# Negai-98/LDT

Hardware: AMD Instinct MI355X
Metric: shapes/sec (2048-pt, 1000-step SDE sample) (higher is better)
Workload: dtype bf16; 1 GPU; BASELINE configs[1]: ShapeNet-airplane sampling, batch 64/GPU, 256 latent tokens x 120, 1000 ancestral SDE steps (24-block d=1024 Score) + decode to 2048 points; global_batch=64, batch_per_gpu=64, sde_steps=1000, points=2048, parallelism=dp1 batch slices, one all-gather, collective=none (single process), rccl_ranks_seen=0

## Files before the change

include/ldt_hip.h:

```cpp
#ifndef LDT_HIP_H
#define LDT_HIP_H
#include <stdint.h>
#ifdef __cplusplus
extern "C" {
#endif

#define LDT_ABI_VERSION 25
#define LDT_OK 0
#define LDT_EARG (-1)
#define LDT_ESHAPE (-2)
#define LDT_EALIGN (-3)
#define LDT_MAX_BLOCKS 64

int ldt_abi_version(void);
const char* ldt_last_error(void);

int ldt_cast_pad_bf16(const float* src, int64_t ld_src, uint16_t* dst, int64_t ld_dst,
                      int64_t rows, int32_t cols, int32_t cols_pad, void* stream);

enum ldt_epilogue {
    LDT_EPI_F32 = 0,
    LDT_EPI_BF16 = 1,
    LDT_EPI_GELU_BF16 = 2,
    LDT_EPI_RELU_BF16 = 3,
// ... 91 lines not shown
                   int64_t mod_sample_stride, int32_t rows_per_sample, void* stream);

int ldt_fold_mean_ratio(const float* stats, int32_t parts, int64_t M, int32_t K, float* out, void* stream);

int ldt_fps(const float* xyz, int32_t B, int32_t n, int32_t m, int32_t skip_near_origin, int32_t* idx_out, void* stream);
int ldt_norm_points(const float* xyz, int32_t B, int32_t n, float* out, void* stream);
int ldt_mixture_seed(const float* eps, const float* sig, const float* mu, const float* logits, int32_t n_mix, int32_t D, int64_t rows,
                     float* out, void* stream);
int ldt_knn(const float* xyz, const float* centers, int32_t B, int32_t n, int32_t S, int32_t k,
            int32_t* idx_out, float* dist_out, void* stream);
int ldt_group_normalize(const float* feat, const float* xyz, const int32_t* fps_idx, const int32_t* knn_idx,
                        const float* alpha, const float* beta, double* stats, int32_t B, int32_t n, int32_t S,
                        int32_t k, int32_t D, uint16_t* U, int32_t ldu, int32_t center_mode, float* group_mean,
                        void* stream);
int ldt_gather_rows(const float* src, const int32_t* idx, int32_t B, int32_t n, int32_t S, int32_t C, float* out, void* stream);
int ldt_grouper_mlp(const float* feat, const float* xyz, const int32_t* fps_idx, const int32_t* knn_idx, const float* alpha,
                    const float* beta, double* stats, int32_t B, int32_t n, int32_t S, int32_t k, int32_t D,
                    const uint16_t* wimg, const float* b1, const float* b2, const float* b3, float* out, void* stream);
int ldt_maxpool(const void* in, int32_t in_bf16, int64_t ld, int64_t G, int32_t n, int32_t C, float* out, void* stream);
int ldt_actnorm(float* x, const float* shift, const float* log_scale, int64_t B, int64_t per_sample, void* stream);
int ldt_reparam(const float* post, const float* noise, float* out, int64_t ldo, float* mu_out, float* logvar_out,
                int64_t rows, int32_t z, float lo, float hi, void* stream);
int ldt_chamfer(const float* a, const float* b, int32_t B, int32_t na, int32_t nb, float* dl, float* dr, void* stream);

int ldt_reparam_kl(const float* post, const float* noise, float* out, int64_t ldo, float* mu_out, float* logvar_out,
                   float* kl_out, float* logqz_out, float* kl_sample_sum, int64_t rows, int64_t rows_per_sample, int32_t z,
                   float lo, float hi, void* stream);
int ldt_diffuse_q(const float* x0, const float* eta_in, const float* m, const float* var, float* xt, float* eta_out,
                  int64_t B, int64_t per_sample, uint64_t seed, int32_t step, void* stream);
int ldt_dsm_loss(const float* eta, const float* params, const float* weight, int64_t B, int64_t per_sample, int32_t l1,
                 float* sample_loss, float* mean_loss, void* stream);

int ldt_nelbo_terms(const float* eta, const float* params, const float* logqz, const float* weight, int64_t B, int64_t per_sample,
                    float* sample_sums, float* batch_sums, void* stream);
int ldt_occupancy_grid(const float* pts, int32_t S, int32_t n, const float* cells, int32_t G, uint32_t* counters, uint32_t* bernoulli,
                       void* stream);

int ldt_transpose_cast_bf16(const void* src, int32_t src_bf16, int64_t ld_src, uint16_t* dst, int64_t ld_dst, int64_t R, int32_t C,
                            int64_t R_pad, void* stream);
int ldt_colsum(const void* dy, int32_t dy_bf16, int64_t ld, int64_t M, int32_t C, float* out, void* stream);
int ldt_layernorm_modulate_bwd(const float* x, int64_t ldx, const float* dy, int64_t lddy, const float* scale, int64_t mod_sample_stride,
                               int32_t rows_per_sample, float* dx, int64_t lddx, float* dshift, float* dscale,
                               int64_t dmod_sample_stride, float* stats, int64_t M, int32_t C, void* stream);
int ldt_gelu_bwd(const uint16_t* u, int64_t ldu, const void* dh, int32_t dh_bf16, int64_t lddh, uint16_t* du, int64_t lddu, int64_t M,
                 int32_t C, void* stream);
int ldt_gate_residual_bwd(const float* dy, int64_t lddy, const void* a, int32_t a_bf16, int64_t lda, const float* gate,
                          int64_t gate_sample_stride, int32_t rows_per_sample, uint16_t* da, int64_t ldda, float* dgate,
                          int64_t dgate_sample_stride, int64_t M, int32_t C, void* stream);
int ldt_silu_bwd(const float* c, const float* dy, float* dc, float* act, int64_t n, void* stream);
int ldt_dsm_loss_bwd(const float* eta, const float* params, const float* weight, int64_t B, int64_t per_sample, int32_t l1, float* dparams,
                     void* stream);
int ldt_embedding_grad(const float* dc, int64_t ld, const int32_t* label, int32_t B, int32_t D, int32_t n_classes, float* dE, void* stream);
int ldt_attention_bwd(const uint16_t* Q, int64_t ldq, int64_t q_batch_stride, const uint16_t* K, int64_t ldk, const uint16_t* V,
                      int64_t ldv, int64_t kv_batch_stride, const uint16_t* O, const uint16_t* dO, float* stats, uint16_t* dQ,
                      int64_t lddq, int64_t dq_batch_stride, uint16_t* dK, int64_t lddk, uint16_t* dV, int64_t lddv,
                      int64_t dkv_batch_stride, int32_t B, int32_t H, int32_t N, int32_t head_dim, void* stream);
int ldt_attention_bwd_narrow(const uint16_t* Q, int64_t ldq, int64_t q_batch_stride, const uint16_t* K, int64_t ldk, const uint16_t* V,
                             int64_t ldv, int64_t kv_batch_stride, const uint16_t* O, const uint16_t* dO, float* stats, uint16_t* dQ,
                             int64_t lddq, int64_t dq_batch_stride, uint16_t* dK, int64_t lddk, uint16_t* dV, int64_t lddv,
                             int64_t dkv_batch_stride, int32_t B, int32_t H, int32_t N, int32_t head_dim, void* stream);
int ldt_attention_bwd_cross(const uint16_t* Q, int64_t ldq, int64_t q_batch_stride, const uint16_t* K, int64_t ldk, const uint16_t* V,
                            int64_t ldv, int64_t kv_batch_stride, const uint16_t* O, const uint16_t* dO, float* stats, uint16_t* dQ,
                            int64_t lddq, int64_t dq_batch_stride, uint16_t* dK, int64_t lddk, uint16_t* dV, int64_t lddv,
                            int64_t dkv_batch_stride, int32_t B, int32_t H, int32_t Nq, int32_t Nk, int32_t head_dim, void* stream);
int ldt_sumsq(const float* x, int64_t n, double* scratch, int32_t scratch_len, float max_norm, float* out, void* stream);
int ldt_adam_ema_step(float* param, float* grad, float* exp_avg, float* exp_avg_sq, float* ema, int64_t n, double lr, double beta1,
                      double beta2, double eps, double weight_decay, int32_t step, double ema_decay, int32_t ema_init,
                      const float* clip_factor, void* stream);

int ldt_ln_mlp_resid(float* x, int64_t ldx, int64_t M, int32_t C, const float* ln_w, const float* ln_b,
                     const float* shift, const float* scale, const float* gate, int64_t mod_sample_stride,
                     int32_t rows_per_sample, const uint16_t* w_up, const float* b_up, const uint16_t* w_dn,
                     const float* b_dn, uint16_t* x_bf16, int64_t ldxb, void* stream);

int ldt_ln_mlp_resid_next(float* x, int64_t ldx, int64_t M, int32_t C, const float* ln_w, const float* ln_b,
                          const float* shift, const float* scale, const float* gate, int64_t mod_sample_stride,
                          int32_t rows_per_sample, const uint16_t* w_up, const float* b_up, const uint16_t* w_dn,
                          const float* b_dn, uint16_t* x_bf16, int64_t ldxb,
                          const float* nx_ln_w, const float* nx_ln_b, const float* nx_shift, const float* nx_scale,
                          int64_t nx_mod_sample_stride, int32_t nx_rows_per_sample, const uint16_t* nx_w, const float* nx_bias,
                          int32_t nx_N, uint16_t* nx_out, int64_t nx_ldo, void* stream);

int ldt_ln_linear(const float* x, int64_t ldx, int64_t M, int32_t C, const float* ln_w, const float* ln_b,
                  const float* shift, const float* scale, int64_t mod_sample_stride, int32_t rows_per_sample,
                  const uint16_t* w, const float* bias, int32_t N, uint16_t* out, int64_t ldo, void* stream);

int ldt_chamfer_pairwise(const float* x, const float* y, int32_t S, int32_t R, int32_t n, int32_t m, float* cd, void* stream);
int ldt_emd_approx(const float* x, const float* y, int32_t S, int32_t R, int32_t n, int32_t m, int32_t pairwise,
                   float* out, void* stream);

typedef struct ldt_score_plan {
    int32_t hidden, heads, blocks, z_dim, z_pad, mlp_hidden, tokens, batch;
    const uint16_t* w_in;  const float* b_in;
    const uint16_t* w_qkv[LDT_MAX_BLOCKS]; const float* b_qkv[LDT_MAX_BLOCKS];
    const uint16_t* w_o[LDT_MAX_BLOCKS];   const float* b_o[LDT_MAX_BLOCKS];
    const uint16_t* w_up[LDT_MAX_BLOCKS];  const float* b_up[LDT_MAX_BLOCKS];
    const uint16_t* w_dn[LDT_MAX_BLOCKS];  const float* b_dn[LDT_MAX_BLOCKS];
    const uint16_t* w_out; const float* b_out;
    const uint16_t* w_q[LDT_MAX_BLOCKS];   const float* b_q[LDT_MAX_BLOCKS];
    const uint16_t* kv_cond[LDT_MAX_BLOCKS];
    int32_t cond_tokens; int32_t _pad0;
    const float* mod; int64_t mod_step_stride; int64_t mod_sample_stride;
    uint16_t* xin;
    float*    X;
    uint16_t* Hb;
    uint16_t* QKV;
    uint16_t* Ob;
    uint16_t* U;
    const float* fold; int64_t fold_step_stride; float* stats;
    int32_t gemm_wgs;
    int32_t fold_monitor_every;
    float* fold_monitor;
} ldt_score_plan;

int ldt_score_lnfold_route(int32_t M, int32_t D, int32_t F, int32_t gemm_wgs);

int ldt_score_forward(const ldt_score_plan* plan, const float* x, float* eps_out,
                      const int32_t* step_ptr, void* stream);

enum ldt_prof_class {
    LDT_PROF_OTHER = 0,
    LDT_PROF_GEMM_IO = 1,
    LDT_PROF_LN = 2,
    LDT_PROF_GEMM_QKV = 3,
    LDT_PROF_ATTN = 4,
    LDT_PROF_GEMM_O = 5,
    LDT_PROF_GEMM_GELU = 6,
    LDT_PROF_GEMM_DN = 7,
    LDT_PROF_NCLASS = 8
};
int ldt_score_forward_profile(const ldt_score_plan* plan, const float* x, float* eps_out, const int32_t* step_ptr,
                              float* ms_by_class, int32_t* launches_by_class, void* stream);

typedef struct ldt_cond_args {
    const float* temb;
    const float* extra;
    const float* w_ada;
    const float* b_ada;
    float* c_buf;
    float* mod_buf;
    int32_t t_dim, n_mod;
    const void* w_ada_bf16;
    void* c_buf_bf16;
} ldt_cond_args;

int ldt_sample_loop(const ldt_score_plan* plan, float* x, float* x_mean, float* eps_tmp,
                    const float* coef, int32_t mode, const float* noise, int64_t noise_step_stride,
                    int64_t elem_offset, uint64_t seed, int32_t* step_counter, int32_t n_steps,
                    const ldt_cond_args* cond, float* x_traj, int32_t use_graph, void* stream);

int ldt_dbg_gemm_group_m(int32_t rows_per_group);
int ldt_dbg_gemm_epi(int32_t bits);
int ldt_dbg_gemm_wreg(int32_t on);

#ifdef __cplusplus
}
#endif
#endif
```

ldt_amd/_lib.py:

```python
import ctypes as C
import os

_HERE = os.path.dirname(os.path.abspath(__file__))
LIB_PATH = os.environ.get("LDT_HIP_LIB", os.path.join(_HERE, "libldt_hip.so"))
ABI_VERSION = 25
MAX_BLOCKS = 64
ODE_SUMSQ_SCRATCH = 1024

EPI_F32, EPI_BF16, EPI_GELU_BF16, EPI_RELU_BF16, EPI_RESID_F32 = range(5)
ACT_NONE, ACT_SILU, ACT_RELU, ACT_GELU = range(4)
BLOCK_ACTS = {"gelu": 1, "silu": 2, "swish": 2, "relu": 3, "leakyrelu": 4, "leakyrelu0.2": 5, "rrelu": 6, "hardswish": 7, "selu": 8}


def block_act_id(name):
    return 0 if name is None else BLOCK_ACTS.get(str(name).lower(), 3)
PROF_CLASSES = ("other", "gemm_io", "ln_modulate", "gemm_qkv", "attention", "gemm_o", "gemm_gelu", "gemm_dn")

_vp, _i32, _i64, _u64 = C.c_void_p, C.c_int32, C.c_int64, C.c_uint64


class ScorePlan(C.Structure):
    _fields_ = (
        [(n, _i32) for n in ("hidden", "heads", "blocks", "z_dim", "z_pad", "mlp_hidden", "tokens", "batch")]
        + [("w_in", _vp), ("b_in", _vp)]
        + [("w_qkv", _vp * MAX_BLOCKS), ("b_qkv", _vp * MAX_BLOCKS),
           ("w_o", _vp * MAX_BLOCKS), ("b_o", _vp * MAX_BLOCKS),
           ("w_up", _vp * MAX_BLOCKS), ("b_up", _vp * MAX_BLOCKS),
           ("w_dn", _vp * MAX_BLOCKS), ("b_dn", _vp * MAX_BLOCKS)]
        + [("w_out", _vp), ("b_out", _vp)]
        + [("w_q", _vp * MAX_BLOCKS), ("b_q", _vp * MAX_BLOCKS), ("kv_cond", _vp * MAX_BLOCKS), ("cond_tokens", _i32), ("_pad0", _i32)]
        + [("mod", _vp), ("mod_step_stride", _i64), ("mod_sample_stride", _i64)]
        + [(n, _vp) for n in ("xin", "X", "Hb", "QKV", "Ob", "U")]
        + [("fold", _vp), ("fold_step_stride", _i64), ("stats", _vp), ("gemm_wgs", _i32), ("fold_monitor_every", _i32), ("fold_monitor", _vp)]
    )


class CondArgs(C.Structure):
    _fields_ = ([(n, _vp) for n in ("temb", "extra", "w_ada", "b_ada", "c_buf", "mod_buf")] + [("t_dim", _i32), ("n_mod", _i32)] +
                [("w_ada_bf16", _vp), ("c_buf_bf16", _vp)])


SIGNATURES = {
    "ldt_abi_version": [],
    "ldt_last_error": [],
    "ldt_cast_pad_bf16": [_vp, _i64, _vp, _i64, _i64, _i32, _i32, _vp],
    "ldt_gemm_bf16": [_i32, _vp, _i64, _vp, _i64, _vp, _vp, _i64, _vp, _i64, _vp, _i64, _vp, _i64, _i32, _vp, _i64,
                      _i32, _i32, _i32, _vp],
    "ldt_gemm_resid_lnstats": [_vp, _i64, _vp, _i64, _vp, _vp, _i64, _vp, _i64, _i32, _vp, _vp, _i64, _vp, _vp, _i64, _i64,
                               _i32, _i32, _i32, _i32, _vp],
    "ldt_gemm_lnfold": [_i32, _vp, _i64, _vp, _i64, _vp, _vp, _vp, _vp, _i64, _vp, _i64, _i32, _i32, _i32, _i32, _vp],
    "ldt_score_lnfold_route": [_i32, _i32, _i32, _i32],
    "ldt_layernorm_modulate": [_vp, _i64, _vp, _i64, _vp, _vp, _vp, _vp, _i64, _i32, _vp, _i64, _i64, _i32, _vp],
    "ldt_attention_fwd": [_vp, _i64, _i64, _vp, _i64, _vp, _i64, _i64, _vp, _i32, _i32, _i32, _i32, _i32, _vp],
    "ldt_attention_route": [_i32, _i32, _i32, _i32, _i32],
    "ldt_gemm_route": [_i32, _i32, _i32, _i32, _i64, _i32, _i32],
    "ldt_qkv_attention": [_vp, _i64, _vp, _i64, _vp, _vp, _i32, _vp, _vp, _i64, _vp, _i64, _i64, _vp, _vp,
                          _i32, _i32, _i32, _i32, _i32, _i32, _i32, _vp, _vp],
    "ldt_qkv_attention_route": [_i32, _i32, _i32, _i32, _i32, _i32, _i32, _i32],
    "ldt_attention_oproj_resid": [_vp, _i64, _i64, _vp, _i64, _vp, _i64, _i64, _i32, _i32, _i32, _i32, _i32, _vp, _vp, _vp, _i64, _vp, _i64, _vp],
    "ldt_sgemm": [_vp, _i64, _vp, _i64, _vp, _vp, _i64, _i32, _i32, _i32, _i32, _i32, _i32, _vp],
    "ldt_sinusoid": [_vp, _vp, _vp, _i32, _i32, _vp],
    "ldt_sampler_step": [_vp, _vp, _vp, _i64, _vp, _vp, _vp, _vp, _i32, _i32, _i64, _i64, _u64, _i32, _i32, _vp],
    "ldt_sampler_step_traj": [_vp, _vp, _vp, _i64, _vp, _vp, _vp, _vp, _vp, _i32, _i32, _i64, _i64, _u64, _i32, _i32, _vp],
    "ldt_philox_normal": [_vp, _i64, _i64, _i32, _u64, _vp],
    "ldt_batch_norm_sum": [_vp, _i32, _i64, _vp, _vp, _vp],
    "ldt_langevin_coef": [_vp, _i32, C.c_float, C.c_float, _vp, _vp],
    "ldt_pndm_transfer": [_vp, _vp, C.c_float, C.c_float, C.c_float, _vp, _i64, _vp],
    "ldt_lincomb4": [_vp, _vp, _vp, _vp, C.c_float, C.c_float, C.c_float, C.c_float, C.c_float, _vp, _i64, _vp],
    "ldt_vpsde_score": [_vp, _vp, C.c_float, C.c_float, C.c_float, _vp, _i32, _i64, _vp],
    "ldt_sde_score": [_vp, _vp, _i32, C.c_float, C.c_float, C.c_float, _vp, _i32, _i64, _vp],
    "ldt_add_f32": [_vp, _vp, _vp, _i64, _vp],
    "ldt_ode_stage": [_vp] * 7 + [C.c_double] * 6 + [_i32, C.c_double, _vp, _vp, _i64, _vp],
    "ldt_ode_rhs": [_vp, _vp, _i32, C.c_float, C.c_float, C.c_float, _vp, _i64, _vp],
    "ldt_ode_scaled_sumsq": [_vp] * 7 + [C.c_double] * 7 + [_i32, _vp, _vp, C.c_double, C.c_double, _vp, _i32, _vp, _i64, _vp],
    "ldt_block_activation": [_vp, _i64, _i64, _i32, _i32, _vp],
    "ldt_group_stats": [_vp, _i64, _i32, _i32, _i32, _i32, C.c_float, _vp, _vp],
    "ldt_norm_apply": [_vp, _i64, _vp, _i64, _i64, _i32, _vp, _i32, _i32, _vp, _vp, _vp, _vp, _i64, _i32, _vp],
    "ldt_widen_bf16": [_vp, _vp, _i64, _vp],
    "ldt_fold_mean_ratio": [_vp, _i32, _i64, _i32, _vp, _vp],
    "ldt_fps": [_vp, _i32, _i32, _i32, _i32, _vp, _vp],
    "ldt_norm_points": [_vp, _i32, _i32, _vp, _vp],
    "ldt_mixture_seed": [_vp, _vp, _vp, _vp, _i32, _i32, _i64, _vp, _vp],
    "ldt_knn": [_vp, _vp, _i32, _i32, _i32, _i32, _vp, _vp, _vp],
    "ldt_group_normalize": [_vp, _vp, _vp, _vp, _vp, _vp, _vp, _i32, _i32, _i32, _i32, _i32, _vp, _i32, _i32, _vp, _vp],
    "ldt_gather_rows": [_vp, _vp, _i32, _i32, _i32, _i32, _vp, _vp],
    "ldt_maxpool": [_vp, _i32, _i64, _i64, _i32, _i32, _vp, _vp],
    "ldt_actnorm": [_vp, _vp, _vp, _i64, _i64, _vp],
    "ldt_reparam": [_vp, _vp, _vp, _i64, _vp, _vp, _i64, _i32, C.c_float, C.c_float, _vp],
    "ldt_chamfer": [_vp, _vp, _i32, _i32, _i32, _vp, _vp, _vp],
    "ldt_reparam_kl": [_vp, _vp, _vp, _i64, _vp, _vp, _vp, _vp, _vp, _i64, _i64, _i32, C.c_float, C.c_float, _vp],
    "ldt_diffuse_q": [_vp, _vp, _vp, _vp, _vp, _vp, _i64, _i64, _u64, _i32, _vp],
    "ldt_dsm_loss": [_vp, _vp, _vp, _i64, _i64, _i32, _vp, _vp, _vp],
    "ldt_nelbo_terms": [_vp, _vp, _vp, _vp, _i64, _i64, _vp, _vp, _vp],
    "ldt_occupancy_grid": [_vp, _i32, _i32, _vp, _i32, _vp, _vp, _vp],
    "ldt_transpose_cast_bf16": [_vp, _i32, _i64, _vp, _i64, _i64, _i32, _i64, _vp],
    "ldt_colsum": [_vp, _i32, _i64, _i64, _i32, _vp, _vp],
    "ldt_layernorm_modulate_bwd": [_vp, _i64, _vp, _i64, _vp, _i64, _i32, _vp, _i64, _vp, _vp, _i64, _vp, _i64, _i32, _vp],
    "ldt_gelu_bwd": [_vp, _i64, _vp, _i32, _i64, _vp, _i64, _i64, _i32, _vp],
    "ldt_gate_residual_bwd": [_vp, _i64, _vp, _i32, _i64, _vp, _i64, _i32, _vp, _i64, _vp, _i64, _i64, _i32, _vp],
    "ldt_silu_bwd": [_vp, _vp, _vp, _vp, _i64, _vp],
    "ldt_dsm_loss_bwd": [_vp, _vp, _vp, _i64, _i64, _i32, _vp, _vp],
    "ldt_embedding_grad": [_vp, _i64, _vp, _i32, _i32, _i32, _vp, _vp],
    "ldt_attention_bwd": [_vp, _i64, _i64, _vp, _i64, _vp, _i64, _i64, _vp, _vp, _vp, _vp, _i64, _i64, _vp, _i64, _vp, _i64, _i64,
                          _i32, _i32, _i32, _i32, _vp],
    "ldt_attention_bwd_narrow": [_vp, _i64, _i64, _vp, _i64, _vp, _i64, _i64, _vp, _vp, _vp, _vp, _i64, _i64, _vp, _i64, _vp, _i64, _i64,
                                 _i32, _i32, _i32, _i32, _vp],
    "ldt_attention_bwd_cross": [_vp, _i64, _i64, _vp, _i64, _vp, _i64, _i64, _vp, _vp, _vp, _vp, _i64, _i64, _vp, _i64, _vp, _i64, _i64,
                                _i32, _i32, _i32, _i32, _i32, _vp],
    "ldt_sumsq": [_vp, _i64, _vp, _i32, C.c_float, _vp, _vp],
    "ldt_adam_ema_step": [_vp, _vp, _vp, _vp, _vp, _i64, C.c_double, C.c_double, C.c_double, C.c_double, C.c_double, _i32, C.c_double, _i32,
                          _vp, _vp],
    "ldt_grouper_mlp": [_vp, _vp, _vp, _vp, _vp, _vp, _vp, _i32, _i32, _i32, _i32, _i32, _vp, _vp, _vp, _vp, _vp, _vp],
    "ldt_ln_mlp_resid": [_vp, _i64, _i64, _i32, _vp, _vp, _vp, _vp, _vp, _i64, _i32, _vp, _vp, _vp, _vp, _vp, _i64, _vp],
    "ldt_ln_mlp_resid_next": [_vp, _i64, _i64, _i32, _vp, _vp, _vp, _vp, _vp, _i64, _i32, _vp, _vp, _vp, _vp, _vp, _i64,
                              _vp, _vp, _vp, _vp, _i64, _i32, _vp, _vp, _i32, _vp, _i64, _vp],
    "ldt_ln_linear": [_vp, _i64, _i64, _i32, _vp, _vp, _vp, _vp, _i64, _i32, _vp, _vp, _i32, _vp, _i64, _vp],
    "ldt_chamfer_pairwise": [_vp, _vp, _i32, _i32, _i32, _i32, _vp, _vp],
    "ldt_emd_approx": [_vp, _vp, _i32, _i32, _i32, _i32, _i32, _vp, _vp],
    "ldt_score_forward": [C.POINTER(ScorePlan), _vp, _vp, _vp, _vp],
    "ldt_score_forward_profile": [C.POINTER(ScorePlan), _vp, _vp, _vp, C.POINTER(C.c_float), C.POINTER(C.c_int32), _vp],
    "ldt_dbg_gemm_group_m": [_i32],
    "ldt_dbg_gemm_epi": [_i32],
    "ldt_dbg_gemm_wreg": [_i32],
    "ldt_sample_loop": [C.POINTER(ScorePlan), _vp, _vp, _vp, _vp, _i32, _vp, _i64, _i64, _u64, _vp, _i32, C.POINTER(CondArgs), _vp, _i32, _vp],
}

_lib = None


class LdtHipError(RuntimeError):
    pass


def lib():
    global _lib
    if _lib is not None:
        return _lib
    if not os.path.exists(LIB_PATH):
        raise LdtHipError(
            "HIP extension %s not found: run `python -c 'import __graft_entry__ as g; g.build()'` "
            "(or ldt_amd/csrc/build.sh).  There is no CPU fallback." % LIB_PATH)
    h = C.CDLL(LIB_PATH)
    for name, argtypes in SIGNATURES.items():
        fn = getattr(h, name)
        fn.argtypes = argtypes
        fn.restype = C.c_char_p if name == "ldt_last_error" else C.c_int
    if h.ldt_abi_version() != ABI_VERSION:
        raise LdtHipError("libldt_hip.so ABI %d != binding ABI %d: rebuild" % (h.ldt_abi_version(), ABI_VERSION))
    _lib = h
    return h


def check(rc, what=""):
    if rc != 0:
        msg = lib().ldt_last_error()
        raise LdtHipError("%s failed (status %d): %s" % (what or "libldt_hip", rc, (msg or b"").decode()))
```

ldt_amd/csrc/api.hip:

```cpp
#include <stdarg.h>
#include <stdio.h>
#include <stdlib.h>
#include <string.h>

#include <vector>

#include "../../include/ldt_hip.h"
#include "kernels.h"

static thread_local char g_err[512] = "";

void ldt_set_error(const char* fmt, ...) {
    va_list ap;
    va_start(ap, fmt);
    vsnprintf(g_err, sizeof(g_err), fmt, ap);
    va_end(ap);
}
int ldt_check_launch(const char* what) {
    const hipError_t e = hipGetLastError();
    if (e != hipSuccess) {
        ldt_set_error("%s: %s", what, hipGetErrorString(e));
        return (int)e;
    }
    return LDT_OK;
}
extern "C" const char* ldt_last_error(void) { return g_err; }
extern "C" int ldt_abi_version(void) { return LDT_ABI_VERSION; }

#define BF(p) reinterpret_cast<const bf16_t*>(p)
#define BFM(p) reinterpret_cast<bf16_t*>(p)
#define ST(s) reinterpret_cast<hipStream_t>(s)
#define TRY(expr)                   \
    do {                            \
        const int _rc = (expr);     \
        if (_rc != LDT_OK) return _rc; \
    } while (0)

extern "C" int ldt_cast_pad_bf16(const float* src, int64_t ld_src, uint16_t* dst, int64_t ld_dst, int64_t rows,
                                 int32_t cols, int32_t cols_pad, void* stream) {
    LDT_REQUIRE(src && dst, LDT_EARG, "cast_pad: null pointer");
    return ldt_cast_pad_launch(src, ld_src, BFM(dst), ld_dst, rows, cols, cols_pad, ST(stream));
}

extern "C" int ldt_gemm_bf16(int32_t epilogue, const uint16_t* X, int64_t ldx, const uint16_t* W, int64_t ldw,
                             const float* bias, void* out, int64_t ldo, const float* resid, int64_t ldr,
                             const uint16_t* skip, int64_t ldskip, const float* gate, int64_t gate_sample_stride,
                             int32_t rows_per_sample, const int32_t* step_ptr, int64_t gate_step_stride,
                             int32_t M, int32_t N, int32_t K, void* stream) {
    LDT_REQUIRE(X && W && out, LDT_EARG, "gemm: null pointer");
    GemmArgs a{BF(X), ldx, BF(W), ldw, bias, out, ldo, resid, ldr, BF(skip), ldskip, gate, gate_sample_stride,
               rows_per_sample, step_ptr, gate_step_stride, M, N, K};
    return ldt_gemm_launch(epilogue, &a, ST(stream));
}

extern "C" int ldt_gemm_resid_lnstats(const uint16_t* X, int64_t ldx, const uint16_t* W, int64_t ldw, const float* bias,
                                      float* out, int64_t ldo, const float* gate, int64_t gate_sample_stride,
                                      int32_t rows_per_sample, const float* ln_scale, uint16_t* xs, int64_t ldxs,
                                      float* stats_out, const int32_t* step_ptr, int64_t gate_step_stride,
                                      int64_t ln_step_stride, int32_t M, int32_t N, int32_t K, int32_t stats_parts, void* stream) {
    LDT_REQUIRE(X && W && out && xs && ln_scale && stats_out, LDT_EARG, "gemm_resid_lnstats: null pointer");
    LDT_REQUIRE(stats_parts == N / 256 || stats_parts == N / 32, LDT_EARG, "gemm_resid_lnstats: stats_parts=%d is neither N/256 nor N/32 (N=%d)", stats_parts, N);
    GemmArgs a{BF(X), ldx, BF(W), ldw, bias, out, ldo, out, ldo, nullptr, 0, gate, gate_sample_stride, rows_per_sample, step_ptr,
               gate_step_stride, M, N, K, BFM(xs), ldxs, ln_scale, ln_step_stride, stats_out};
    a.stats_parts = stats_parts;
    return ldt_gemm_lnfold_launch(EPI_RESID_F32, &a, ST(stream));
}

extern "C" int ldt_gemm_lnfold(int32_t epilogue, const uint16_t* Xs, int64_t ldx, const uint16_t* W, int64_t ldw,
                               const float* stats_in, const float* fold_S, const float* fold_C, uint16_t* out, int64_t ldo,
                               const int32_t* step_ptr, int64_t fold_step_stride, int32_t M, int32_t N, int32_t K, int32_t stats_parts,
                               void* stream) {
    LDT_REQUIRE(Xs && W && out && stats_in && fold_S && fold_C, LDT_EARG, "gemm_lnfold: null pointer");
    LDT_REQUIRE(stats_parts == K / 256 || stats_parts == K / 32, LDT_EARG, "gemm_lnfold: stats_parts=%d is neither K/256 nor K/32 (K=%d)", stats_parts, K);
    GemmArgs a{BF(Xs), ldx, BF(W), ldw, nullptr, out, ldo, nullptr, 0, nullptr, 0, nullptr, 0, 0, step_ptr, 0, M, N, K,
               nullptr, 0, nullptr, 0, nullptr, stats_in, stats_parts, fold_S, fold_C, fold_step_stride};
    return ldt_gemm_lnfold_launch(epilogue, &a, ST(stream));
}

extern "C" int ldt_layernorm_modulate(const float* x, int64_t ldx, uint16_t* y, int64_t ldy, const float* w,
                                      const float* b, const float* shift, const float* scale,
                                      int64_t mod_sample_stride, int32_t rows_per_sample, const int32_t* step_ptr,
                                      int64_t mod_step_stride, int64_t M, int32_t C, void* stream) {
    LDT_REQUIRE(x && y, LDT_EARG, "ln: null pointer");
    LnArgs a{x, ldx, BFM(y), ldy, w, b, shift, scale, mod_sample_stride, rows_per_sample, step_ptr, mod_step_stride, M, C};
    return ldt_ln_launch(&a, ST(stream));
}

extern "C" int ldt_attention_fwd(const uint16_t* Q, int64_t ldq, int64_t q_batch_stride, const uint16_t* K,
                                 int64_t ldk, const uint16_t* V, int64_t ldv, int64_t kv_batch_stride, uint16_t* O,
                                 int32_t B, int32_t H, int32_t Nq, int32_t Nk, int32_t head_dim, void* stream) {
    LDT_REQUIRE(Q && K && V && O, LDT_EARG, "attention: null pointer");
    AttnArgs a{BF(Q), ldq, q_batch_stride, BF(K), ldk, kv_batch_stride, BF(V), ldv, BFM(O), B, H, Nq, Nk,
               1.4426950408889634f / sqrtf((float)head_dim), nullptr, nullptr, nullptr, 0, nullptr, 0};
    return ldt_attn_launch(&a, head_dim, ST(stream));
}
extern "C" int ldt_attention_route(int32_t B, int32_t H, int32_t Nq, int32_t Nk, int32_t head_dim) { return ldt_attn_route(B, H, Nq, Nk, head_dim); }
extern "C" int ldt_gemm_route(int32_t epilogue, int32_t M, int32_t N, int32_t K, int64_t ldo, int32_t fold, int32_t max_wgs) {
    GemmArgs a{};
    a.M = M; a.N = N; a.K = K; a.ldo = ldo; a.ldr = ldo; a.max_wgs = max_wgs;
    if (fold != 0 && fold != 32 && fold != 256) return 0;
    const GemmRoute r = ldt_gemm_decide(epilogue, &a, fold);
    return (r.family << 28) | ((r.tiles_per_wg < 255 ? r.tiles_per_wg : 255) << 20) | (r.bm << 10) | r.bn;
}
extern "C" int ldt_attention_oproj_resid(const uint16_t* Q, int64_t ldq, int64_t q_batch_stride, const uint16_t* K,
                                         int64_t ldk, const uint16_t* V, int64_t ldv, int64_t kv_batch_stride,
                                         int32_t B, int32_t H, int32_t Nq, int32_t Nk, int32_t head_dim,
                                         const uint16_t* Wo, const float* bo, float* X, int64_t ldx, const float* gate,
                                         int64_t gate_sample_stride, void* stream) {
    LDT_REQUIRE(Q && K && V && Wo && bo && X, LDT_EARG, "attention_oproj: null pointer");
    AttnArgs a{BF(Q), ldq, q_batch_stride, BF(K), ldk, kv_batch_stride, BF(V), ldv, nullptr, B, H, Nq, Nk,
               1.4426950408889634f / sqrtf((float)head_dim), BF(Wo), bo, X, ldx, gate, gate_sample_stride};
    return ldt_attn_oproj_launch(&a, head_dim, ST(stream));
}

extern "C" int ldt_sgemm(const float* A, int64_t lda, const float* Bw, int64_t ldb, const float* bias, void* C,
                         int64_t ldc, int32_t out_bf16, int32_t act_in, int32_t act_out, int32_t M, int32_t N,
                         int32_t K, void* stream) {
    SgemmArgs a{A, lda, Bw, ldb, bias, C, ldc, out_bf16, act_in, act_out, M, N, K};
    return ldt_sgemm_launch(&a, ST(stream));
}

extern "C" int ldt_sinusoid(const float* t, const float* freq, float* e, int32_t n, int32_t half, void* stream) {
    LDT_REQUIRE(t && freq && e, LDT_EARG, "sinusoid: null pointer");
    return ldt_sinusoid_launch(t, freq, e, n, half, ST(stream));
}

extern "C" int ldt_sampler_step(const float* x, const float* params, const float* noise, int64_t noise_step_stride,
                                float* x_out, float* x_mean_out, const float* coef, const int32_t* step_ptr,
                                int32_t step_host, int32_t mode, int64_t n, int64_t elem_offset, uint64_t seed,
                                int32_t philox_mul, int32_t philox_add, void* stream) {
    StepArgs a{x, params, noise, x_out, x_mean_out, coef, step_ptr, step_host, mode, n, elem_offset, noise_step_stride,
               (uint32_t)seed, (uint32_t)(seed >> 32), philox_mul, philox_add};
    return ldt_sampler_step_launch(&a, ST(stream));
}
extern "C" int ldt_sampler_step_traj(const float* x, const float* params, const float* noise, int64_t noise_step_stride,
                                     float* x_out, float* x_mean_out, float* traj, const float* coef, const int32_t* step_ptr,
                                     int32_t step_host, int32_t mode, int64_t n, int64_t elem_offset, uint64_t seed,
                                     int32_t philox_mul, int32_t philox_add, void* stream) {
    LDT_REQUIRE(!traj || ldt_aligned16(traj), LDT_EALIGN, "sampler_step_traj: traj must be 16-byte aligned");
    StepArgs a{x, params, noise, x_out, x_mean_out, coef, step_ptr, step_host, mode, n, elem_offset, noise_step_stride,
               (uint32_t)seed, (uint32_t)(seed >> 32), philox_mul, philox_add, traj};
    return ldt_sampler_step_launch(&a, ST(stream));
}

extern "C" int ldt_philox_normal(float* out, int64_t n, int64_t elem_offset, int32_t step, uint64_t seed, void* stream) {
    LDT_REQUIRE(out, LDT_EARG, "philox_normal: null pointer");
    return ldt_philox_normal_launch(out, n, elem_offset, step, (uint32_t)seed, (uint32_t)(seed >> 32), ST(stream));
}

extern "C" int ldt_fps(const float* xyz, int32_t B, int32_t n, int32_t m, int32_t skip_near_origin, int32_t* idx_out, void* stream) {
    LDT_REQUIRE(xyz && idx_out, LDT_EARG, "fps: null pointer");
    return ldt_fps_launch(xyz, B, n, m, skip_near_origin, idx_out, ST(stream));
}
extern "C" int ldt_knn(const float* xyz, const float* centers, int32_t B, int32_t n, int32_t S, int32_t k,
                       int32_t* idx_out, float* dist_out, void* stream) {
    LDT_REQUIRE(xyz && centers && idx_out, LDT_EARG, "knn: null pointer");
    return ldt_knn_launch(xyz, centers, B, n, S, k, idx_out, dist_out, ST(stream));
// ... 50 lines not shown
extern "C" int ldt_ln_mlp_resid(float* x, int64_t ldx, int64_t M, int32_t C, const float* ln_w, const float* ln_b,
                                const float* shift, const float* scale, const float* gate, int64_t mod_sample_stride,
                                int32_t rows_per_sample, const uint16_t* w_up, const float* b_up, const uint16_t* w_dn,
                                const float* b_dn, uint16_t* x_bf16, int64_t ldxb, void* stream) {
    LDT_REQUIRE(x && w_up && b_up && w_dn && b_dn, LDT_EARG, "ln_mlp: null pointer");
    MlpArgs a{x, ldx, M, ln_w, ln_b, shift, scale, gate, mod_sample_stride, rows_per_sample, BF(w_up), b_up, BF(w_dn), b_dn,
              BFM(x_bf16), ldxb};
    return ldt_ln_mlp_launch(&a, C, ST(stream));
}
extern "C" int ldt_ln_mlp_resid_next(float* x, int64_t ldx, int64_t M, int32_t C, const float* ln_w, const float* ln_b,
                                     const float* shift, const float* scale, const float* gate, int64_t mod_sample_stride,
                                     int32_t rows_per_sample, const uint16_t* w_up, const float* b_up, const uint16_t* w_dn,
                                     const float* b_dn, uint16_t* x_bf16, int64_t ldxb,
                                     const float* nx_ln_w, const float* nx_ln_b, const float* nx_shift, const float* nx_scale,
                                     int64_t nx_mod_sample_stride, int32_t nx_rows_per_sample, const uint16_t* nx_w, const float* nx_bias,
                                     int32_t nx_N, uint16_t* nx_out, int64_t nx_ldo, void* stream) {
    LDT_REQUIRE(x && w_up && b_up && w_dn && b_dn && nx_w && nx_out, LDT_EARG, "ln_mlp_next: null pointer");
    MlpArgs a{x, ldx, M, ln_w, ln_b, shift, scale, gate, mod_sample_stride, rows_per_sample, BF(w_up), b_up, BF(w_dn), b_dn,
              BFM(x_bf16), ldxb,
              LnLinArgs{nullptr, 0, M, nx_ln_w, nx_ln_b, nx_shift, nx_scale, nx_mod_sample_stride, nx_rows_per_sample, BF(nx_w), nx_bias,
                        nx_N, BFM(nx_out), nx_ldo}};
    return ldt_ln_mlp_launch(&a, C, ST(stream));
}
extern "C" int ldt_ln_linear(const float* x, int64_t ldx, int64_t M, int32_t C, const float* ln_w, const float* ln_b,
                             const float* shift, const float* scale, int64_t mod_sample_stride, int32_t rows_per_sample,
                             const uint16_t* w, const float* bias, int32_t N, uint16_t* out, int64_t ldo, void* stream) {
    LDT_REQUIRE(x && w && out, LDT_EARG, "ln_linear: null pointer");
    LnLinArgs a{x, ldx, M, ln_w, ln_b, shift, scale, mod_sample_stride, rows_per_sample, BF(w), bias, N, BFM(out), ldo};
    return ldt_ln_linear_launch(&a, C, ST(stream));
}
extern "C" int ldt_chamfer_pairwise(const float* x, const float* y, int32_t S, int32_t R, int32_t n, int32_t m, float* cd, void* stream) {
    LDT_REQUIRE(x && y && cd, LDT_EARG, "chamfer_pairwise: null pointer");
    return ldt_chamfer_pairwise_launch(x, y, S, R, n, m, cd, ST(stream));
}
extern "C" int ldt_emd_approx(const float* x, const float* y, int32_t S, int32_t R, int32_t n, int32_t m, int32_t pairwise,
                              float* out, void* stream) {
    LDT_REQUIRE(x && y && out, LDT_EARG, "emd_approx: null pointer");
    return ldt_emd_approx_launch(x, y, S, R, n, m, pairwise, out, ST(stream));
}

extern "C" int ldt_score_lnfold_route(int32_t M, int32_t D, int32_t F, int32_t gemm_wgs) {
    if (M <= 0 || D <= 0 || F <= 0 || D % 256 != 0 || D > 1024 || F % 256 != 0) return 0;
    if (ldt_gemm_lnfold_v1_route(M, D, F, gemm_wgs)) return 2;
    const int lim = ldt_wg_limit(gemm_wgs);
    return (M % 256 == 0 && (long)(M / 256) * (D / 256) * 8 >= (long)lim * 5) ? 1 : 0;
}

static int check_plan(const ldt_score_plan* p) {
    LDT_REQUIRE(p, LDT_EARG, "score: null plan");
    LDT_REQUIRE(p->blocks > 0 && p->blocks <= LDT_MAX_BLOCKS, LDT_ESHAPE, "score: blocks=%d out of range", p->blocks);
    LDT_REQUIRE(p->hidden > 0 && p->heads > 0 && p->hidden % p->heads == 0, LDT_ESHAPE, "score: hidden %% heads");
    const int dh = p->hidden / p->heads;
    LDT_REQUIRE(dh == 8 || dh == 16 || dh == 32 || dh == 64, LDT_ESHAPE, "score: head dim %d not built (8, 16, 32, 64)", dh);
    LDT_REQUIRE(p->hidden % 64 == 0 && p->mlp_hidden % 64 == 0 && p->z_pad % 64 == 0 && p->z_pad >= p->z_dim, LDT_ESHAPE,
                "score: hidden/mlp_hidden/z_pad must be multiples of 64");
    LDT_REQUIRE(p->z_dim % 4 == 0, LDT_ESHAPE, "score: z_dim %% 4");
    LDT_REQUIRE(p->tokens > 0 && p->batch > 0, LDT_ESHAPE, "score: empty batch");
    LDT_REQUIRE(p->w_in && p->w_out && p->mod && p->xin && p->X && p->Hb && p->QKV && p->Ob && p->U, LDT_EARG, "score: null buffer in plan");
    for (int l = 0; l < p->blocks; ++l) {
        LDT_REQUIRE(p->w_qkv[l] && p->w_o[l] && p->w_up[l] && p->w_dn[l], LDT_EARG, "score: block %d weights missing", l);
        LDT_REQUIRE(!p->kv_cond[l] || (p->w_q[l] && p->cond_tokens > 0), LDT_EARG, "score: block %d cross-attention needs w_q and cond_tokens", l);
    }
    return LDT_OK;
}

struct Prof {
    hipStream_t s;
    std::vector<hipEvent_t> ev;
    std::vector<int> cls;
    void begin(int c) { hipEvent_t a, b; (void)hipEventCreate(&a); (void)hipEventCreate(&b); ev.push_back(a); ev.push_back(b); cls.push_back(c); (void)hipEventRecord(a, s); }
    void end() { (void)hipEventRecord(ev.back(), s); }
    void cancel() { (void)hipEventDestroy(ev.back()); ev.pop_back(); (void)hipEventDestroy(ev.back()); ev.pop_back(); cls.pop_back(); }
};
#define LAUNCH_TRY(cls_, took_, try_expr, st_)      \
    do {                                            \
        if (prof) prof->begin(cls_);                \
        took_ = (try_expr);                         \
        if (prof) { if (took_) prof->end(); else prof->cancel(); } \
        if (took_ && (st_) != LDT_OK) return (st_); \
    } while (0)
#define LAUNCH(cls_, expr)                \
    do {                                  \
        if (prof) prof->begin(cls_);      \
        const int _rc = (expr);           \
        if (prof) prof->end();            \
        if (_rc != LDT_OK) return _rc;    \
    } while (0)

struct QkvAttnStep {
    const bf16_t* X; long ldx; const bf16_t* W; long ldw; const float* bias;
    const float* stats; int stats_parts; const float* fold_S; const float* fold_C; long fold_step_stride;
    const bf16_t* kv; long ldkv; long kv_batch_stride;
    bf16_t* attn_o; bf16_t* QKV;
    int B, tokens, cond_tokens, hidden, heads, K, max_wgs;
    const int* step_ptr;
};
static int qkv_attention_route(const GemmArgs* g, int tokens, int cond_tokens, int head_dim, bool cross, bool folded) {
    if (cross) return ldt_gemm_mid_q_xattn_takes(g, tokens, cond_tokens, head_dim) ? 3 : 0;
    if (ldt_gemm_mid_qkv_attn_takes(g, tokens, head_dim, folded)) return 1;
    return ldt_gemm_qkv_attn256_takes(g, tokens, head_dim, folded) ? 2 : 0;
}
static int qkv_attention_step(const QkvAttnStep& q, hipStream_t s, Prof* prof) {
    const int D = q.hidden, T = q.tokens, dh = D / q.heads;
    const bool cross = q.kv != nullptr, folded = q.stats != nullptr;
    const float scale_log2e = 1.4426950408889634f / sqrtf((float)dh);
    GemmArgs gq{q.X, q.ldx, q.W, q.ldw, q.bias, q.QKV, 3L * D, nullptr, 0, nullptr, 0, nullptr, 0, 0, folded ? q.step_ptr : nullptr, 0,
                q.B * T, cross ? D : 3 * D, q.K};
    if (folded) { gq.stats_in = q.stats; gq.stats_parts = q.stats_parts; gq.fold_S = q.fold_S; gq.fold_C = q.fold_C; gq.fold_step_stride = q.fold_step_stride; }
    gq.max_wgs = q.max_wgs;
    gq.attn_o = q.attn_o; gq.attn_scale_log2e = scale_log2e;
    if (cross) { gq.attn_k = q.kv; gq.attn_v = q.kv + D; gq.attn_ldkv = q.ldkv; gq.attn_kv_batch_stride = q.kv_batch_stride; }
    int fst = LDT_OK;
    bool took = false;
    if (cross) LAUNCH_TRY(LDT_PROF_GEMM_QKV, took, ldt_gemm_mid_q_xattn_try(&gq, T, q.cond_tokens, dh, s, &fst), fst);
    else {
        LAUNCH_TRY(LDT_PROF_GEMM_QKV, took, ldt_gemm_mid_qkv_attn_try(&gq, T, dh, folded, s, &fst), fst);
        if (!took) LAUNCH_TRY(LDT_PROF_GEMM_QKV, took, ldt_gemm_qkv_attn256_try(&gq, T, dh, folded, s, &fst), fst);
    }
    if (took) return LDT_OK;
    if (folded) LAUNCH(LDT_PROF_GEMM_QKV, ldt_gemm_lnfold_launch(LDT_EPI_BF16, &gq, s));
    else LAUNCH(LDT_PROF_GEMM_QKV, ldt_gemm_launch(LDT_EPI_BF16, &gq, s));
    const int S = cross ? q.cond_tokens : T;
    AttnArgs at{q.QKV, 3L * D, (long)T * 3 * D, cross ? q.kv : q.QKV + D, cross ? q.ldkv : 3L * D, cross ? q.kv_batch_stride : (long)T * 3 * D,
                cross ? q.kv + D : q.QKV + 2 * D, cross ? q.ldkv : 3L * D, q.attn_o, q.B, q.heads, T, S, scale_log2e};
    LAUNCH(LDT_PROF_ATTN, ldt_attn_launch(&at, dh, s));
    return LDT_OK;
}

extern "C" int ldt_qkv_attention_route(int32_t B, int32_t tokens, int32_t cond_tokens, int32_t hidden, int32_t heads, int32_t K, int32_t fold,
                                       int32_t max_wgs) {
    if (B <= 0 || tokens <= 0 || hidden <= 0 || heads <= 0 || hidden % heads != 0 || (fold != 0 && fold != 32 && fold != 256) || (fold && cond_tokens > 0)) return 0;
    GemmArgs g{};
    g.M = B * tokens; g.N = cond_tokens > 0 ? hidden : 3 * hidden; g.K = K; g.max_wgs = max_wgs;
    g.stats_parts = fold ? K / fold : 0;
    return qkv_attention_route(&g, tokens, cond_tokens, hidden / heads, cond_tokens > 0, fold != 0);
}
extern "C" int ldt_qkv_attention(const uint16_t* X, int64_t ldx, const uint16_t* W, int64_t ldw, const float* bias,
                                 const float* stats, int32_t stats_parts, const float* fold_S, const float* fold_C, int64_t fold_step_stride,
                                 const uint16_t* kv_cond, int64_t ldkv, int64_t kv_batch_stride, uint16_t* O, uint16_t* QKV,
                                 int32_t B, int32_t tokens, int32_t cond_tokens, int32_t hidden, int32_t heads, int32_t K, int32_t max_wgs,
                                 const int32_t* step_ptr, void* stream) {
    LDT_REQUIRE(X && W && O && QKV, LDT_EARG, "qkv_attention: null pointer");
    LDT_REQUIRE(B > 0 && tokens > 0 && hidden > 0 && heads > 0 && hidden % heads == 0 && hidden % 64 == 0 && K > 0, LDT_ESHAPE,
                "qkv_attention: B=%d tokens=%d hidden=%d heads=%d K=%d", B, tokens, hidden, heads, K);
    const int dh = hidden / heads;
    LDT_REQUIRE(dh == 8 || dh == 16 || dh == 32 || dh == 64, LDT_ESHAPE, "qkv_attention: head dim %d not built (8, 16, 32, 64)", dh);
    LDT_REQUIRE(!kv_cond || (cond_tokens > 0 && !stats), LDT_EARG, "qkv_attention: cross-attention needs cond_tokens and has no folded form");
    LDT_REQUIRE(!stats || (fold_S && fold_C && stats_parts > 0 && !bias), LDT_EARG, "qkv_attention: the folded form needs fold_S, fold_C, stats_parts and takes no bias (it is part of fold_C)");
    QkvAttnStep q{BF(X), ldx, BF(W), ldw, bias, stats, stats_parts, fold_S, fold_C, fold_step_stride, BF(kv_cond), ldkv, kv_batch_stride,
                  BFM(O), BFM(QKV), B, tokens, cond_tokens, hidden, heads, K, max_wgs, step_ptr};
    return qkv_attention_step(q, ST(stream), nullptr);
}

static int score_forward_impl(const ldt_score_plan* p, const float* x, float* eps_out, const int32_t* step_ptr,
                              hipStream_t s, Prof* prof) {
    TRY(check_plan(p));
    LDT_REQUIRE(x && eps_out, LDT_EARG, "score: null x/out");
    const int D = p->hidden, T = p->tokens, M = p->batch * p->tokens, F = p->mlp_hidden;
    const long sstr = p->mod_sample_stride, tstr = p->mod_step_stride;
    const bool fold_v1 = ldt_gemm_lnfold_v1_route(M, D, F, p->gemm_wgs);
    bool fold = p->fold && p->stats && sstr == 0 && (M % 256 == 0 || fold_v1) && D % 256 == 0 && D <= 1024 && F % 256 == 0;
    for (int l = 0; l < p->blocks && fold; ++l) fold = !p->kv_cond[l];
    const int sparts = fold_v1 ? D / 32 : D / 256;
    const long fstep = p->fold_step_stride, fblk = 6L * D + 2L * F;
    LAUNCH(LDT_PROF_OTHER, ldt_cast_pad_launch(x, p->z_dim, BFM(p->xin), p->z_pad, M, p->z_dim, p->z_pad, s));
    {
        GemmArgs g{BF(p->xin), p->z_pad, BF(p->w_in), p->z_pad, p->b_in, p->X, D, nullptr, 0, nullptr, 0, nullptr, 0, 0, nullptr, 0, M, D, p->z_pad};
        g.max_wgs = p->gemm_wgs; LAUNCH(LDT_PROF_GEMM_IO, ldt_gemm_launch(LDT_EPI_F32, &g, s));
    }
    for (int l = 0; l < p->blocks; ++l) {
        const float* m = p->mod + (long)l * 6 * D;
        const float* fl = fold ? p->fold + (long)l * fblk : nullptr;
        QkvAttnStep qa{BF(p->Hb), D, nullptr, D, nullptr, nullptr, 0, nullptr, nullptr, 0, nullptr, 0, 0, BFM(p->Ob), BFM(p->QKV),
                       p->batch, T, p->cond_tokens, D, p->heads, D, p->gemm_wgs, step_ptr};
        if (fold && l > 0) {
            qa.W = BF(p->w_qkv[l]);
            qa.stats = p->stats; qa.stats_parts = sparts; qa.fold_S = fl; qa.fold_C = fl + 3L * D; qa.fold_step_stride = fstep;
        } else {
            LnArgs n1{p->X, D, BFM(p->Hb), D, nullptr, nullptr, m, m + D, sstr, T, step_ptr, tstr, M, D};
            LAUNCH(LDT_PROF_LN, ldt_ln_launch(&n1, s));
            if (p->kv_cond[l]) {
                qa.W = BF(p->w_q[l]); qa.bias = p->b_q[l];
                qa.kv = BF(p->kv_cond[l]); qa.ldkv = 2L * D; qa.kv_batch_stride = (long)p->cond_tokens * 2 * D;
            } else {
                qa.W = BF(p->w_qkv[l]); qa.bias = p->b_qkv[l];
            }
        }
        TRY(qkv_attention_step(qa, s, prof));
        if (fold) {
            GemmArgs go{BF(p->Ob), D, BF(p->w_o[l]), D, p->b_o[l], p->X, D, p->X, D, nullptr, 0, m + 2 * D, sstr, T, step_ptr, tstr, M, D, D,
                        BFM(p->Hb), D, m + 4 * D, tstr, p->stats};
            go.max_wgs = p->gemm_wgs; go.stats_parts = sparts; LAUNCH(LDT_PROF_GEMM_O, ldt_gemm_lnfold_launch(LDT_EPI_RESID_F32, &go, s));
            if (p->fold_monitor) TRY(ldt_fold_monitor_launch(p->stats, sparts, M, D, p->fold_monitor, s));
            GemmArgs gu{BF(p->Hb), D, BF(p->w_up[l]), D, nullptr, p->U, F, nullptr, 0, nullptr, 0, nullptr, 0, 0, step_ptr, 0, M, F, D,
                        nullptr, 0, nullptr, 0, nullptr, p->stats, sparts, fl + 6L * D, fl + 6L * D + F, fstep};
            gu.max_wgs = p->gemm_wgs; LAUNCH(LDT_PROF_GEMM_GELU, ldt_gemm_lnfold_launch(LDT_EPI_GELU_BF16, &gu, s));
            GemmArgs gd{BF(p->U), F, BF(p->w_dn[l]), F, p->b_dn[l], p->X, D, p->X, D, nullptr, 0, m + 5 * D, sstr, T, step_ptr, tstr, M, D, F,
                        BFM(p->Hb), D, m + 6 * D + D, tstr, p->stats};
            gd.max_wgs = p->gemm_wgs; gd.stats_parts = sparts;
            if (l + 1 < p->blocks) {
                LAUNCH(LDT_PROF_GEMM_DN, ldt_gemm_lnfold_launch(LDT_EPI_RESID_F32, &gd, s));
                if (p->fold_monitor) TRY(ldt_fold_monitor_launch(p->stats, sparts, M, D, p->fold_monitor, s));
            }
            else LAUNCH(LDT_PROF_GEMM_DN, ldt_gemm_launch(LDT_EPI_RESID_F32, &gd, s));
            continue;
        }
        LnArgs n2{p->X, D, BFM(p->Hb), D, nullptr, nullptr, m + 3 * D, m + 4 * D, sstr, T, step_ptr, tstr, M, D};
        {
            GemmArgs go{BF(p->Ob), D, BF(p->w_o[l]), D, p->b_o[l], p->X, D, p->X, D, nullptr, 0, m + 2 * D, sstr, T, step_ptr, tstr, M, D, D};
            go.max_wgs = p->gemm_wgs; LAUNCH(LDT_PROF_GEMM_O, ldt_gemm_launch(LDT_EPI_RESID_F32, &go, s));
        }
        LAUNCH(LDT_PROF_LN, ldt_ln_launch(&n2, s));
        GemmArgs gu{BF(p->Hb), D, BF(p->w_up[l]), D, p->b_up[l], p->U, F, nullptr, 0, nullptr, 0, nullptr, 0, 0, nullptr, 0, M, F, D};
        gu.max_wgs = p->gemm_wgs; LAUNCH(LDT_PROF_GEMM_GELU, ldt_gemm_launch(LDT_EPI_GELU_BF16, &gu, s));
        {
            GemmArgs gd{BF(p->U), F, BF(p->w_dn[l]), F, p->b_dn[l], p->X, D, p->X, D, nullptr, 0, m + 5 * D, sstr, T, step_ptr, tstr, M, D, F};
            gd.max_wgs = p->gemm_wgs; LAUNCH(LDT_PROF_GEMM_DN, ldt_gemm_launch(LDT_EPI_RESID_F32, &gd, s));
        }
    }
    {
        const float* m = p->mod + (long)p->blocks * 6 * D;
        LnArgs nf{p->X, D, BFM(p->Hb), D, nullptr, nullptr, m, m + D, sstr, T, step_ptr, tstr, M, D};
        LAUNCH(LDT_PROF_LN, ldt_ln_launch(&nf, s));
        GemmArgs gf{BF(p->Hb), D, BF(p->w_out), D, p->b_out, eps_out, p->z_dim, nullptr, 0, nullptr, 0, nullptr, 0, 0, nullptr, 0, M, p->z_dim, D};
        gf.max_wgs = p->gemm_wgs; LAUNCH(LDT_PROF_GEMM_IO, ldt_gemm_launch(LDT_EPI_F32, &gf, s));
    }
    return LDT_OK;
}

extern "C" int ldt_score_forward(const ldt_score_plan* p, const float* x, float* eps_out, const int32_t* step_ptr, void* stream) {
    return score_forward_impl(p, x, eps_out, step_ptr, ST(stream), nullptr);
}

extern "C" int ldt_score_forward_profile(const ldt_score_plan* p, const float* x, float* eps_out, const int32_t* step_ptr,
                                         float* ms_by_class, int32_t* launches_by_class, void* stream) {
    LDT_REQUIRE(ms_by_class && launches_by_class, LDT_EARG, "score_profile: null output");
    Prof prof{ST(stream), {}, {}};
    const int rc = score_forward_impl(p, x, eps_out, step_ptr, ST(stream), &prof);
    (void)hipStreamSynchronize(ST(stream));
    for (int c = 0; c < LDT_PROF_NCLASS; ++c) { ms_by_class[c] = 0.f; launches_by_class[c] = 0; }
    for (size_t i = 0; i < prof.cls.size(); ++i) {
        float ms = 0.f;
        if (rc == LDT_OK && hipEventElapsedTime(&ms, prof.ev[2 * i], prof.ev[2 * i + 1]) == hipSuccess) {
            ms_by_class[prof.cls[i]] += ms;
            launches_by_class[prof.cls[i]] += 1;
        }
        (void)hipEventDestroy(prof.ev[2 * i]);
        (void)hipEventDestroy(prof.ev[2 * i + 1]);
    }
    return rc;
}

static int enqueue_step(const ldt_score_plan* p, float* x, float* x_mean, float* eps_tmp, const float* coef, int mode,
                        const float* noise, long noise_step_stride, long elem_offset, uint64_t seed, int* step_counter,
                        const ldt_cond_args* cond, float* x_traj, hipStream_t s) {
    if (cond) {
        TRY(ldt_cond_rows_launch(cond->temb, cond->extra, cond->c_buf, cond->c_buf_bf16, step_counter, p->batch, cond->t_dim, 1, s));
        if (cond->w_ada_bf16 && (cond->t_dim % 64 == 0 || !cond->w_ada)) {
            GemmArgs g{};
            g.X = BF(cond->c_buf_bf16); g.ldx = cond->t_dim;
            g.W = BF(cond->w_ada_bf16); g.ldw = cond->t_dim;
            g.bias = cond->b_ada; g.out = cond->mod_buf; g.ldo = cond->n_mod;
            g.M = p->batch; g.N = cond->n_mod; g.K = cond->t_dim;
            g.max_wgs = p->gemm_wgs;
            TRY(ldt_gemm_launch(EPI_F32, &g, s));
        } else {
            SgemmArgs g{cond->c_buf, cond->t_dim, cond->w_ada, cond->t_dim, cond->b_ada, cond->mod_buf, cond->n_mod, 0, LDT_ACT_NONE,
                        LDT_ACT_NONE, p->batch, cond->n_mod, cond->t_dim};
            TRY(ldt_sgemm_launch(&g, s));
        }
    }
    TRY(score_forward_impl(p, x, eps_tmp, cond ? nullptr : step_counter, s, nullptr));
    const long n = (long)p->batch * p->tokens * p->z_dim;
    StepArgs st{x, eps_tmp, noise, x, x_mean, coef, step_counter, 0, mode, n, elem_offset, noise_step_stride,
                (uint32_t)seed, (uint32_t)(seed >> 32), 1, 0, x_traj};
    TRY(ldt_sampler_step_launch(&st, s));
    return ldt_advance_step_launch(step_counter, s);
}

extern "C" int ldt_sample_loop(const ldt_score_plan* p, float* x, float* x_mean, float* eps_tmp, const float* coef,
                               int32_t mode, const float* noise, int64_t noise_step_stride, int64_t elem_offset,
                               uint64_t seed, int32_t* step_counter, int32_t n_steps, const ldt_cond_args* cond,
                               float* x_traj, int32_t use_graph, void* stream) {
    TRY(check_plan(p));
    LDT_REQUIRE(x && x_mean && eps_tmp && coef && step_counter && n_steps > 0, LDT_EARG, "sample_loop: null pointer / n_steps");
    LDT_REQUIRE(!cond || !cond->w_ada_bf16 == !cond->c_buf_bf16, LDT_EARG, "sample_loop: w_ada_bf16 and c_buf_bf16 go together");
    LDT_REQUIRE(!cond || (cond->temb && (cond->w_ada || cond->w_ada_bf16) && cond->b_ada && cond->c_buf && cond->mod_buf && cond->mod_buf == p->mod &&
                          p->mod_sample_stride == cond->n_mod && cond->t_dim > 0), LDT_EARG,
                "sample_loop: inconsistent conditioning block (plan->mod must be cond->mod_buf with sample stride n_mod)");
    hipStream_t s = ST(stream);
    hipError_t e = hipMemsetAsync(step_counter, 0, sizeof(int), s);
    if (e != hipSuccess) { ldt_set_error("sample_loop: memset: %s", hipGetErrorString(e)); return (int)e; }
    ldt_score_plan plain = *p;
    plain.fold_monitor = nullptr;
    const bool mon = p->fold_monitor != nullptr;
    const int every = p->fold_monitor_every > 0 ? p->fold_monitor_every : 1;
    auto monitored = [&](int i) { return mon && (i % every == 0 || i == n_steps - 1); };
    if (!use_graph) {
        for (int i = 0; i < n_steps; ++i)
            TRY(enqueue_step(monitored(i) ? p : &plain, x, x_mean, eps_tmp, coef, mode, noise, noise_step_stride, elem_offset, seed, step_counter, cond, x_traj, s));
        return LDT_OK;
    }
    hipStream_t gs = nullptr;
    hipEvent_t ev_in = nullptr, ev_out = nullptr;
    hipGraph_t graph = nullptr, graph_m = nullptr;
    hipGraphExec_t exec = nullptr, exec_m = nullptr;
    int status = LDT_OK;
#define HIPTRY(call, what)                                                                   \
    do {                                                                                     \
        const hipError_t _e = (call);                                                        \
        if (_e != hipSuccess && status == LDT_OK) {                                          \
            ldt_set_error("sample_loop: %s: %s", what, hipGetErrorString(_e));               \
            status = (int)_e;                                                                \
        }                                                                                    \
    } while (0)
    HIPTRY(hipStreamCreateWithFlags(&gs, hipStreamNonBlocking), "stream create");
    HIPTRY(hipEventCreateWithFlags(&ev_in, hipEventDisableTiming), "event create");
    HIPTRY(hipEventCreateWithFlags(&ev_out, hipEventDisableTiming), "event create");
    if (status == LDT_OK) {
        HIPTRY(hipEventRecord(ev_in, s), "event record");
        HIPTRY(hipStreamWaitEvent(gs, ev_in, 0), "stream wait");
    }
    if (status == LDT_OK) {
        for (int pass = 0; pass < (mon ? 2 : 1) && status == LDT_OK; ++pass) {
            HIPTRY(hipStreamBeginCapture(gs, hipStreamCaptureModeThreadLocal), "begin capture");
            if (status == LDT_OK) {
                const int rc = enqueue_step(pass ? p : &plain, x, x_mean, eps_tmp, coef, mode, noise, noise_step_stride, elem_offset, seed, step_counter, cond, x_traj, gs);
                const hipError_t ee = hipStreamEndCapture(gs, pass ? &graph_m : &graph);
                if (rc != LDT_OK) status = rc;
                else if (ee != hipSuccess) { ldt_set_error("sample_loop: end capture: %s", hipGetErrorString(ee)); status = (int)ee; }
            }
        }
    }
    if (status == LDT_OK) HIPTRY(hipGraphInstantiate(&exec, graph, nullptr, nullptr, 0), "graph instantiate");
    if (status == LDT_OK && mon) HIPTRY(hipGraphInstantiate(&exec_m, graph_m, nullptr, nullptr, 0), "graph instantiate");
    for (int i = 0; i < n_steps && status == LDT_OK; ++i) HIPTRY(hipGraphLaunch(monitored(i) ? exec_m : exec, gs), "graph launch");
    if (gs) {
        if (status == LDT_OK) {
            HIPTRY(hipEventRecord(ev_out, gs), "event record");
            HIPTRY(hipStreamWaitEvent(s, ev_out, 0), "stream wait");
        }
        (void)hipStreamSynchronize(gs);
    }
    if (exec) (void)hipGraphExecDestroy(exec);
    if (exec_m) (void)hipGraphExecDestroy(exec_m);
    if (graph) (void)hipGraphDestroy(graph);
    if (graph_m) (void)hipGraphDestroy(graph_m);
    if (ev_in) (void)hipEventDestroy(ev_in);
    if (ev_out) (void)hipEventDestroy(ev_out);
    if (gs) (void)hipStreamDestroy(gs);
#undef HIPTRY
    return status;
}
```

ldt_amd/csrc/elementwise.hip:

```cpp
#include <stdlib.h>

#include "kernels.h"

__global__ void cast_pad_kernel(const float* __restrict__ src, long lds, bf16_t* __restrict__ dst, long ldd,
                                long rows, int cols, int cols_pad) {
    const long total = rows * (long)(cols_pad / 4);
    for (long i = blockIdx.x * (long)blockDim.x + threadIdx.x; i < total; i += (long)gridDim.x * blockDim.x) {
        const long r = i / (cols_pad / 4);
        const int c = (int)(i % (cols_pad / 4)) * 4;
        float v[4];
#pragma unroll
        for (int j = 0; j < 4; ++j) v[j] = (c + j < cols) ? src[r * lds + c + j] : 0.f;
        bf16x4 pk = {(bf16_t)v[0], (bf16_t)v[1], (bf16_t)v[2], (bf16_t)v[3]};
        *reinterpret_cast<bf16x4*>(dst + r * ldd + c) = pk;
    }
}

int ldt_cast_pad_launch(const float* src, long lds, bf16_t* dst, long ldd, long rows, int cols,
                                   int cols_pad, hipStream_t s) {
    LDT_REQUIRE(rows > 0 && cols > 0 && cols_pad >= cols && cols_pad % 4 == 0 && ldd % 4 == 0, LDT_ESHAPE,
                "cast_pad: bad shape rows=%ld cols=%d cols_pad=%d ldd=%ld", rows, cols, cols_pad, ldd);
    LDT_REQUIRE((reinterpret_cast<uintptr_t>(dst) & 7) == 0, LDT_EALIGN, "cast_pad: dst must be 8-byte aligned");
    const long total = rows * (long)(cols_pad / 4);
    int blocks = (int)((total + 255) / 256);
    if (blocks > 2048) blocks = 2048;
    hipLaunchKernelGGL(cast_pad_kernel, dim3(blocks), dim3(256), 0, s, src, lds, dst, ldd, rows, cols, cols_pad);
    return ldt_check_launch("cast_pad");
}

template <int NV>
__global__ __launch_bounds__(256) void ln_mod_vec_kernel(const LnArgs a) {
    const int lane = threadIdx.x & 63;
    const long row = blockIdx.x * 4L + (threadIdx.x >> 6);
    if (row >= a.M) return;
    const float* xr = a.x + row * a.ldx;
    const long modoff = a.shift ? (a.step_ptr ? (long)(*a.step_ptr) * a.mod_step_stride : 0) + (row / a.rows_per_sample) * a.mod_sample_stride : 0;
    f32x4 v[NV];
    float s = 0.f;
#pragma unroll
    for (int i = 0; i < NV; ++i) {
        const int c = i * 256 + lane * 4;
        v[i] = *reinterpret_cast<const f32x4*>(xr + c);
        s += (v[i][0] + v[i][1]) + (v[i][2] + v[i][3]);
    }
    const float mean = wave_sum(s) / (float)a.C;
    float q = 0.f;
#pragma unroll
    for (int i = 0; i < NV; ++i)
#pragma unroll
        for (int j = 0; j < 4; ++j) { const float d = v[i][j] - mean; q += d * d; }
    const float rstd = rsqrtf(wave_sum(q) / (float)a.C + 1e-6f);
    const float* sh = a.shift; const float* sc = a.scale;
    if (sh) { sh += modoff; sc += modoff; }
    bf16_t* yr = a.y + row * a.ldy;
#pragma unroll
    for (int i = 0; i < NV; ++i) {
        const int c = i * 256 + lane * 4;
        f32x4 o;
#pragma unroll
        for (int j = 0; j < 4; ++j) o[j] = (v[i][j] - mean) * rstd;
        if (a.w) { const f32x4 w = *reinterpret_cast<const f32x4*>(a.w + c); const f32x4 b = *reinterpret_cast<const f32x4*>(a.b + c);
#pragma unroll
            for (int j = 0; j < 4; ++j) o[j] = o[j] * w[j] + b[j]; }
        if (sh) { const f32x4 h = *reinterpret_cast<const f32x4*>(sh + c); const f32x4 g = *reinterpret_cast<const f32x4*>(sc + c);
#pragma unroll
            for (int j = 0; j < 4; ++j) o[j] = o[j] * (1.f + g[j]) + h[j]; }
        bf16x4 pk = {(bf16_t)o[0], (bf16_t)o[1], (bf16_t)o[2], (bf16_t)o[3]};
        *reinterpret_cast<bf16x4*>(yr + c) = pk;
    }
}

__global__ __launch_bounds__(256) void ln_mod_generic_kernel(const LnArgs a) {
    const int lane = threadIdx.x & 63;
    const long row = blockIdx.x * 4L + (threadIdx.x >> 6);
    if (row >= a.M) return;
    const float* xr = a.x + row * a.ldx;
    float s = 0.f;
    for (int c = lane; c < a.C; c += 64) s += xr[c];
    const float mean = wave_sum(s) / (float)a.C;
    float q = 0.f;
    for (int c = lane; c < a.C; c += 64) { const float d = xr[c] - mean; q += d * d; }
    const float rstd = rsqrtf(wave_sum(q) / (float)a.C + 1e-6f);
    const float* sh = a.shift; const float* sc = a.scale;
    if (sh) {
        const long off = (a.step_ptr ? (long)(*a.step_ptr) * a.mod_step_stride : 0) +
                         (row / a.rows_per_sample) * a.mod_sample_stride;
        sh += off; sc += off;
    }
    bf16_t* yr = a.y + row * a.ldy;
    for (int c = lane; c < a.C; c += 64) {
        float o = (xr[c] - mean) * rstd;
        if (a.w) o = o * a.w[c] + a.b[c];
        if (sh) o = o * (1.f + sc[c]) + sh[c];
        yr[c] = (bf16_t)o;
    }
}

int ldt_ln_launch(const LnArgs* a, hipStream_t s) {
    LDT_REQUIRE(a->M > 0 && a->C > 0, LDT_ESHAPE, "ln: empty problem");
    LDT_REQUIRE((a->shift == nullptr) == (a->scale == nullptr), LDT_EARG, "ln: shift and scale go together");
    LDT_REQUIRE((a->w == nullptr) == (a->b == nullptr), LDT_EARG, "ln: affine weight and bias go together");
    LDT_REQUIRE(!a->shift || a->rows_per_sample > 0, LDT_EARG, "ln: rows_per_sample must be > 0 with modulation");
    dim3 grid((unsigned)((a->M + 3) / 4)), block(256);
    const bool vec = (a->C % 256 == 0) && a->C <= 1024 && a->ldx % 4 == 0 && a->ldy % 4 == 0 && ldt_aligned16(a->x) &&
                     (reinterpret_cast<uintptr_t>(a->y) & 7) == 0 && (!a->shift || (ldt_aligned16(a->shift) && ldt_aligned16(a->scale) &&
                     a->mod_sample_stride % 4 == 0 && a->mod_step_stride % 4 == 0)) && (!a->w || (ldt_aligned16(a->w) && ldt_aligned16(a->b)));
    if (vec) {
        switch (a->C / 256) {
            case 1: hipLaunchKernelGGL(ln_mod_vec_kernel<1>, grid, block, 0, s, *a); break;
            case 2: hipLaunchKernelGGL(ln_mod_vec_kernel<2>, grid, block, 0, s, *a); break;
            case 3: hipLaunchKernelGGL(ln_mod_vec_kernel<3>, grid, block, 0, s, *a); break;
            default: hipLaunchKernelGGL(ln_mod_vec_kernel<4>, grid, block, 0, s, *a); break;
        }
    } else {
        hipLaunchKernelGGL(ln_mod_generic_kernel, grid, block, 0, s, *a);
    }
    return ldt_check_launch("ln_modulate");
}


__global__ __launch_bounds__(256) void sampler_step_kernel(const StepArgs a) {
    const int step = a.step_ptr ? *a.step_ptr : a.step_host;
    const f32x4 cf = *reinterpret_cast<const f32x4*>(a.coef + 4L * step);
    const float* nz = a.noise ? a.noise + (long)step * a.noise_step_stride : nullptr;
    const long nvec = a.n / 4;
    for (long i = blockIdx.x * (long)blockDim.x + threadIdx.x; i < nvec; i += (long)gridDim.x * blockDim.x) {
        const f32x4 x = *reinterpret_cast<const f32x4*>(a.x + 4 * i);
        const f32x4 p = *reinterpret_cast<const f32x4*>(a.params + 4 * i);
        f32x4 z;
        if (nz) {
            z = *reinterpret_cast<const f32x4*>(nz + 4 * i);
        } else {
            const uint64_t e = (uint64_t)(a.elem_offset / 4 + i);
            uint32_t c[4] = {(uint32_t)e, (uint32_t)(e >> 32), (uint32_t)(step * a.philox_mul + a.philox_add), 0x4C445421u};
            philox4x32_10(c, a.seed_lo, a.seed_hi);
            float z0, z1, z2, z3;
            box_muller(c[0], c[1], z0, z1);
            box_muller(c[2], c[3], z2, z3);
            z = (f32x4){z0, z1, z2, z3};
        }
        f32x4 xm, xn;
        {
#pragma clang fp contract(off)
#pragma unroll
            for (int j = 0; j < 4; ++j) {
                if (a.mode == 0) {
                    const float score = -p[j] / cf[1];
                    const float bs = cf[0] * score;
                    const float num = x[j] + bs;
                    xm[j] = num / cf[2];
                } else {
                    const float ax = cf[0] * x[j];
                    const float bp = cf[1] * p[j];
                    xm[j] = ax + bp;
                }
                const float cz = (a.mode == 0) ? cf[3] : cf[2];
                const float nz_ = cz * z[j];
                xn[j] = xm[j] + nz_;
            }
        }
        *reinterpret_cast<f32x4*>(a.x_out + 4 * i) = xn;
        if (a.traj) *reinterpret_cast<f32x4*>(a.traj + (long)step * a.n + 4 * i) = xn;
        if (a.x_mean_out) *reinterpret_cast<f32x4*>(a.x_mean_out + 4 * i) = xm;
    }
}

__global__ void advance_step_kernel(int* step_ptr) { if (threadIdx.x == 0 && blockIdx.x == 0) *step_ptr += 1; }

int ldt_sampler_step_launch(const StepArgs* a, hipStream_t s) {
    LDT_REQUIRE(a->n > 0 && a->n % 4 == 0 && a->elem_offset % 4 == 0, LDT_ESHAPE, "sampler_step: n and elem_offset must be multiples of 4 (n=%ld)", a->n);
    LDT_REQUIRE(a->x && a->params && a->x_out && a->coef, LDT_EARG, "sampler_step: null pointer");
    LDT_REQUIRE(ldt_aligned16(a->x) && ldt_aligned16(a->params) && ldt_aligned16(a->x_out) && ldt_aligned16(a->coef) &&
                (!a->noise || ldt_aligned16(a->noise)) && (!a->x_mean_out || ldt_aligned16(a->x_mean_out)) && a->noise_step_stride % 4 == 0,
                LDT_EALIGN, "sampler_step: buffers must be 16-byte aligned");
    LDT_REQUIRE(a->mode == 0 || a->mode == 1, LDT_EARG, "sampler_step: mode %d", a->mode);
    long blocks = (a->n / 4 + 255) / 256;
    if (blocks > 2048) blocks = 2048;
    hipLaunchKernelGGL(sampler_step_kernel, dim3((unsigned)blocks), dim3(256), 0, s, *a);
    return ldt_check_launch("sampler_step");
}
int ldt_advance_step_launch(int* step_ptr, hipStream_t s) {
    hipLaunchKernelGGL(advance_step_kernel, dim3(1), dim3(64), 0, s, step_ptr);
    return ldt_check_launch("advance_step");
}

__global__ void philox_normal_kernel(float* out, long n, long elem_offset, int step, uint32_t k0, uint32_t k1) {
    const long nvec = n / 4;
    for (long i = blockIdx.x * (long)blockDim.x + threadIdx.x; i < nvec; i += (long)gridDim.x * blockDim.x) {
        const uint64_t e = (uint64_t)(elem_offset / 4 + i);
        uint32_t c[4] = {(uint32_t)e, (uint32_t)(e >> 32), (uint32_t)step, 0x4C445421u};
        philox4x32_10(c, k0, k1);
        float z0, z1, z2, z3;
        box_muller(c[0], c[1], z0, z1);
        box_muller(c[2], c[3], z2, z3);
        *reinterpret_cast<f32x4*>(out + 4 * i) = (f32x4){z0, z1, z2, z3};
    }
}
int ldt_philox_normal_launch(float* out, long n, long elem_offset, int step, uint32_t k0, uint32_t k1, hipStream_t s) {
    LDT_REQUIRE(n > 0 && n % 4 == 0 && elem_offset % 4 == 0 && ldt_aligned16(out), LDT_ESHAPE, "philox_normal: n/offset %% 4, 16-byte aligned");
    long blocks = (n / 4 + 255) / 256;
    if (blocks > 2048) blocks = 2048;
    hipLaunchKernelGGL(philox_normal_kernel, dim3((unsigned)blocks), dim3(256), 0, s, out, n, elem_offset, step, k0, k1);
    return ldt_check_launch("philox_normal");
}

__global__ void sinusoid_kernel(const float* __restrict__ t, const float* __restrict__ freq, float* __restrict__ e, int n, int half) {
    const int i = blockIdx.x;
    for (int k = threadIdx.x; k < half; k += blockDim.x) {
        const float a = __fmul_rn(t[i], freq[k]);
        e[(long)i * 2 * half + k] = sinf(a);
        e[(long)i * 2 * half + half + k] = cosf(a);
    }
}
int ldt_sinusoid_launch(const float* t, const float* freq, float* e, int n, int half, hipStream_t s) {
    LDT_REQUIRE(n > 0 && half > 0, LDT_ESHAPE, "sinusoid: empty");
    hipLaunchKernelGGL(sinusoid_kernel, dim3(n), dim3(128), 0, s, t, freq, e, n, half);
    return ldt_check_launch("sinusoid");
}

__device__ __forceinline__ float apply_act(float v, int act) {
    switch (act) {
        case ACT_SILU: return v / (1.0f + expf(-v));
        case ACT_RELU: return fmaxf(v, 0.f);
        case ACT_GELU: return gelu_erf(v);
        default: return v;
    }
}
__global__ __launch_bounds__(256) void sgemm_nt_kernel(const SgemmArgs a) {
    __shared__ float As[16][68];
    __shared__ float Bs[16][68];
    const int tid = threadIdx.x;
    const int tx = tid & 15, ty = tid >> 4;
    const int m0 = blockIdx.y * 64, n0 = blockIdx.x * 64;
    float acc[4][4] = {};
    const int lr = tid >> 2, lk = (tid & 3) * 4;
    const bool vec = (a.lda % 4 == 0) && (a.ldb % 4 == 0) && (a.K % 4 == 0) && ldt_aligned16(a.A) && ldt_aligned16(a.B);
    for (int k0 = 0; k0 < a.K; k0 += 16) {
        const int m = m0 + lr, n = n0 + lr, kk = k0 + lk;
        f32x4 va4 = {0.f, 0.f, 0.f, 0.f}, vb4 = {0.f, 0.f, 0.f, 0.f};
        if (vec) {
            if (m < a.M && kk < a.K) va4 = *reinterpret_cast<const f32x4*>(a.A + (long)m * a.lda + kk);
            if (n < a.N && kk < a.K) vb4 = *reinterpret_cast<const f32x4*>(a.B + (long)n * a.ldb + kk);
        } else {
#pragma unroll
            for (int j = 0; j < 4; ++j) {
                if (m < a.M && kk + j < a.K) va4[j] = a.A[(long)m * a.lda + kk + j];
                if (n < a.N && kk + j < a.K) vb4[j] = a.B[(long)n * a.ldb + kk + j];
            }
        }
#pragma unroll
        for (int j = 0; j < 4; ++j) {
            As[lk + j][lr] = a.act_in ? apply_act(va4[j], a.act_in) : va4[j];
            Bs[lk + j][lr] = vb4[j];
        }
        __syncthreads();
#pragma unroll
        for (int k = 0; k < 16; ++k) {
            const f32x4 av = *reinterpret_cast<const f32x4*>(&As[k][ty * 4]);
            const f32x4 bv = *reinterpret_cast<const f32x4*>(&Bs[k][tx * 4]);
#pragma unroll
            for (int i = 0; i < 4; ++i)
#pragma unroll
                for (int j = 0; j < 4; ++j) acc[i][j] = fmaf(av[i], bv[j], acc[i][j]);
        }
        __syncthreads();
    }
#pragma unroll
    for (int i = 0; i < 4; ++i) {
        const int m = m0 + ty * 4 + i;
        if (m >= a.M) continue;
#pragma unroll
        for (int j = 0; j < 4; ++j) {
            const int n = n0 + tx * 4 + j;
            if (n >= a.N) continue;
            float v = acc[i][j] + (a.bias ? a.bias[n] : 0.f);
            v = apply_act(v, a.act_out);
            if (a.out_bf16) reinterpret_cast<bf16_t*>(a.C)[(long)m * a.ldc + n] = (bf16_t)v;
            else reinterpret_cast<float*>(a.C)[(long)m * a.ldc + n] = v;
        }
    }
}
int ldt_sgemm_launch(const SgemmArgs* a, hipStream_t s) {
    LDT_REQUIRE(a->M > 0 && a->N > 0 && a->K > 0, LDT_ESHAPE, "sgemm: empty problem");
    LDT_REQUIRE(a->A && a->B && a->C, LDT_EARG, "sgemm: null pointer");
    static const bool no_mfma = getenv("LDT_SGEMM_VALU") != nullptr;
    static const bool no_skinny = getenv("LDT_SGEMM_SKINNY") && atoi(getenv("LDT_SGEMM_SKINNY")) == 0;
    int st = LDT_OK;
    if (!no_skinny && ldt_skinny_linear_try(a, s, &st)) return st;
    if (!no_mfma && ldt_sgemm_mfma_try(a, s, &st)) return st;
    dim3 grid((a->N + 63) / 64, (a->M + 63) / 64), block(256);
    LDT_REQUIRE(grid.y < 65536, LDT_ESHAPE, "sgemm: M too large for this kernel (M=%d)", a->M);
    hipLaunchKernelGGL(sgemm_nt_kernel, grid, block, 0, s, *a);
    return ldt_check_launch("sgemm_nt");
}

__global__ void cond_rows_kernel(const float* __restrict__ temb, const float* __restrict__ extra, float* __restrict__ c, bf16_t* __restrict__ cb,
                                 const int* __restrict__ step_ptr, int batch, int t_dim, int silu_out) {
    const int step = step_ptr ? *step_ptr : 0;
    for (int i = blockIdx.x * blockDim.x + threadIdx.x; i < batch * t_dim; i += gridDim.x * blockDim.x) {
        const int k = i % t_dim;
        const float v = temb[(long)step * t_dim + k] + (extra ? extra[i] : 0.f);
        const float o = silu_out ? silu(v) : v;
        c[i] = o;
        if (cb) cb[i] = (bf16_t)o;
    }
}
int ldt_cond_rows_launch(const float* temb, const float* extra, float* c, void* c_bf16, const int* step_ptr, int batch, int t_dim, int silu_out, hipStream_t s) {
    LDT_REQUIRE(temb && c && batch > 0 && t_dim > 0, LDT_EARG, "cond_rows: bad arguments");
    int blocks = (batch * t_dim + 255) / 256; if (blocks > 1024) blocks = 1024;
    hipLaunchKernelGGL(cond_rows_kernel, dim3(blocks), dim3(256), 0, s, temb, extra, c, reinterpret_cast<bf16_t*>(c_bf16), step_ptr, batch, t_dim, silu_out);
    return ldt_check_launch("cond_rows");
}
```

ldt_amd/csrc/gemm256_tile.h:

```cpp
#pragma once
#include <type_traits>

#include "kernels.h"

enum { FOLD_NONE = 0, FOLD_PRODUCER = 1, FOLD_CONSUMER = 2 };

#define G256_BUF_BYTES 65536
#define G256_W_OFF 32768
#define G256_RING_BYTES (2 * G256_BUF_BYTES)
#define G256_LDS_BYTES (G256_RING_BYTES + 8 * 4096)
#define G256_STATS_OFF 2304
#define G256_SC_OFF (G256_STATS_OFF + 1024)

#define G256_BARRIER()                        \
    do {                                      \
        __builtin_amdgcn_sched_barrier(0);    \
        __builtin_amdgcn_s_barrier();         \
        __builtin_amdgcn_sched_barrier(0);    \
    } while (0)

struct Tile256List {
    int tiles_m, tiles_n, gm;
    int c_lo, j, stride, count;
    __host__ __device__ Tile256List(int tiles_m_, int tiles_n_, int group_m, int G, int bid) : tiles_m(tiles_m_), tiles_n(tiles_n_), gm(group_m) {
        const int tiles = tiles_m * tiles_n;
        const int nx = G < 8 ? G : 8;
        const int xcd = bid % nx;
        j = bid / nx;
        stride = (G - xcd + nx - 1) / nx;
        const int c_hi = (int)((long)tiles * (xcd + 1) / nx);
        c_lo = (int)((long)tiles * xcd / nx);
        count = (c_hi - c_lo - j + stride - 1) / stride > 0 ? (c_hi - c_lo - j + stride - 1) / stride : 0;
    }
    __host__ __device__ void tile(int i, int& tm, int& tn) const {
        const int id = c_lo + j + i * stride;
        if (gm <= 1) { tm = id / tiles_n; tn = id % tiles_n; return; }
        const int per = gm * tiles_n, g = id / per, r = id - g * per;
        const int rows = gm < tiles_m - g * gm ? gm : tiles_m - g * gm;
        tm = g * gm + r % rows; tn = r / rows;
    }
    static int max_count(int tiles_m, int tiles_n, int G) {
        int mx = 0;
        for (int b = 0; b < G && b < 8; ++b) { const int c = Tile256List(tiles_m, tiles_n, 1, G, b).count; mx = c > mx ? c : mx; }
        return mx;
    }
};

static inline int gemm256_default_group_m(int tiles_m, int tiles_n) { return (tiles_n >= 8 && tiles_m >= 8) ? 4 : 1; }
bool ldt_gemm256_takes(int epi, const GemmArgs* a);
int ldt_gemm256_launch(int epi, int fold, const GemmArgs* a, const GemmRoute& route, hipStream_t stream);
int ldt_gemm_variant_env();

__device__ __forceinline__ float row16_sum(float v) {
    v += __builtin_bit_cast(float, __builtin_amdgcn_update_dpp(0, __builtin_bit_cast(int, v), 0xB1, 0xF, 0xF, true));
    v += __builtin_bit_cast(float, __builtin_amdgcn_update_dpp(0, __builtin_bit_cast(int, v), 0x4E, 0xF, 0xF, true));
    v += __builtin_bit_cast(float, __builtin_amdgcn_update_dpp(0, __builtin_bit_cast(int, v), 0x141, 0xF, 0xF, true));
    v += __builtin_bit_cast(float, __builtin_amdgcn_update_dpp(0, __builtin_bit_cast(int, v), 0x140, 0xF, 0xF, true));
    return v;
}


__device__ __forceinline__ void g256_fold_finalize(char* stage_base, int R, int parts, int K) {
    char* slot = stage_base + (R >> 7) * 4096 + G256_STATS_OFF + (R & 127) * 8;
    float s1 = 0.f, s2 = 0.f;
    for (int pp = 0; pp < parts; ++pp) {
        const f32x2 t = *reinterpret_cast<const f32x2*>(slot + pp * 2 * 4096);
        s1 += t[0]; s2 += t[1];
    }
    const float invk = 1.0f / (float)K;
    const float mean = s1 * invk;
    const float var = fmaxf(s2 * invk - mean * mean, 0.f);
    const float r = rsqrtf(var + 1e-6f);
    *reinterpret_cast<f32x2*>(slot) = (f32x2){r, -mean * r};
}

template <int EPI, int FOLD, int XRING = 0>
__device__ __forceinline__ void g256_epilogue_staged(const GemmArgs& a, f32x4 (&acc)[4][8], int m0, int n0, int grp, int wn,
                                                   int lane, int lrow, int lchk, const float* gate, char* reg, char* stage_base,
                                                   const float* ln_scale, bool have_pre, f32x4 g4_pre, f32x4 sc4_pre,
                                                   char* xring = nullptr) {
    const int mb = m0 + grp * 128, nb = n0 + wn * 64;
    f32x4 bias4[4];
#pragma unroll
    for (int ni = 0; ni < 4; ++ni)
        bias4[ni] = (a.bias && FOLD != FOLD_CONSUMER) ? *reinterpret_cast<const f32x4*>(a.bias + nb + ni * 16 + lchk * 4) : (f32x4){0.f, 0.f, 0.f, 0.f};
    if (EPI == EPI_BF16 || EPI == EPI_GELU_BF16 || EPI == EPI_RELU_BF16) {
        constexpr int RS = 128 + 16;
        f32x4 s4[4];
        float rr[8], nm[8];
        if (FOLD == FOLD_CONSUMER) {
#pragma unroll
            for (int mi = 0; mi < 8; ++mi) {
                const int R = grp * 128 + mi * 16 + lrow;
                const f32x2 t = *reinterpret_cast<const f32x2*>(stage_base + (R >> 7) * 4096 + G256_STATS_OFF + (R & 127) * 8);
                rr[mi] = t[0]; nm[mi] = t[1];
            }
#pragma unroll
            for (int ni = 0; ni < 4; ++ni) {
                const int c = wn * 64 + ni * 16 + lchk * 4;
                s4[ni] = *reinterpret_cast<const f32x4*>(stage_base + (c >> 7) * 4096 + G256_SC_OFF + (c & 127) * 4);
                bias4[ni] = *reinterpret_cast<const f32x4*>(stage_base + (2 + (c >> 7)) * 4096 + G256_SC_OFF + (c & 127) * 4);
            }
        }
#pragma unroll
        for (int mi = 0; mi < 8; ++mi) {
#pragma unroll
            for (int ni = 0; ni < 4; ++ni) {
                f32x4 v = acc[ni][mi];
                if (FOLD == FOLD_CONSUMER) {
#pragma unroll
                    for (int r = 0; r < 4; ++r) v[r] = v[r] * rr[mi] + (nm[mi] * s4[ni][r] + bias4[ni][r]);
                } else {
#pragma unroll
                    for (int r = 0; r < 4; ++r) v[r] += bias4[ni][r];
                }
                if (EPI == EPI_GELU_BF16) {
#pragma unroll
                    for (int r = 0; r < 4; r += 2) {
                        const f32x2 gg = gelu_erf_fast2((f32x2){v[r], v[r + 1]});
                        v[r] = gg[0]; v[r + 1] = gg[1];
                    }
                }
                if (EPI == EPI_RELU_BF16) {
                    if (a.skip) {
                        const bf16x4 sk = *reinterpret_cast<const bf16x4*>(a.skip + (long)(mb + mi * 16 + lrow) * a.lds_ + nb + ni * 16 + lchk * 4);
#pragma unroll
                        for (int r = 0; r < 4; ++r) v[r] += (float)sk[r];
                    }
#pragma unroll
                    for (int r = 0; r < 4; ++r) v[r] = fmaxf(v[r], 0.f);
                }
                const bf16x4 pk = {(bf16_t)v[0], (bf16_t)v[1], (bf16_t)v[2], (bf16_t)v[3]};
                *reinterpret_cast<bf16x4*>(reg + lrow * RS + (ni * 16 + lchk * 4) * 2) = pk;
            }
            bf16_t* o = reinterpret_cast<bf16_t*>(a.out) + (long)(mb + mi * 16) * a.ldo + nb;
#pragma unroll
            for (int it = 0; it < 2; ++it) {
                const int row = it * 8 + (lane >> 3), ch = lane & 7;
                const bf16x8 d = *reinterpret_cast<const bf16x8*>(reg + row * RS + ch * 16);
                *reinterpret_cast<bf16x8*>(o + (long)row * a.ldo + ch * 8) = d;
            }
        }
    } else {
        const int ch = lane & 15;
        f32x4 g4 = {1.f, 1.f, 1.f, 1.f};
        const bool has_gate = (EPI == EPI_RESID_F32) && gate;
        const bool shared_gate = has_gate && a.gate_sample_stride == 0;
        if (shared_gate) g4 = have_pre ? g4_pre : *reinterpret_cast<const f32x4*>(gate + nb + ch * 4);
        f32x4 sc4 = {1.f, 1.f, 1.f, 1.f};
        constexpr int SP = (FOLD == FOLD_PRODUCER) ? 8 : 4;
        const float* xsrc = XRING ? a.resid + ((long)mb + (lane >> 4)) * a.ldr + nb + ch * 4 : nullptr;
        const long xstep = (long)4 * a.ldr;
        auto request_pass = [&](int p) {
#pragma unroll
            for (int it = 0; it < 4; ++it) {
                __builtin_amdgcn_global_load_lds((const __attribute__((address_space(1))) void*)xsrc,
                                                 (__attribute__((address_space(3))) void*)(xring + (p & 3) * 4096 + it * 1024), 16, 0, 0);
                xsrc += xstep;
                asm volatile("" : "+v"(xsrc));
            }
        };
        if (XRING) { request_pass(0); request_pass(1); request_pass(2); request_pass(3); }
        float rs1[8], rs2[8];
        if (FOLD == FOLD_PRODUCER) {
            const f32x4 t = have_pre ? sc4_pre : *reinterpret_cast<const f32x4*>(ln_scale + nb + ch * 4);
#pragma unroll
            for (int r = 0; r < 4; ++r) sc4[r] = 1.0f + t[r];
        }
#pragma unroll
        for (int mi = 0; mi < 8; ++mi) {
#pragma unroll
            for (int ni = 0; ni < 4; ++ni) {
                f32x4 v = acc[ni][mi];
#pragma unroll
                for (int r = 0; r < 4; ++r) v[r] += bias4[ni][r];
                *reinterpret_cast<f32x4*>(reg + lrow * 256 + (((ni * 4 + lchk) ^ lrow) << 4)) = v;
            }
            const long mrow0 = mb + mi * 16;
            float k1 = 0.f, k2 = 0.f;
            if (XRING) {
                constexpr int NW[8] = {12, 12 + SP, 12 + 2 * SP, 12 + 3 * SP, 12 + 3 * SP, 8 + 3 * SP, 4 + 3 * SP, 3 * SP};
                switch (mi) {
                    case 0: asm volatile("s_waitcnt vmcnt(%0)" ::"n"(NW[0]) : "memory"); break;
                    case 1: asm volatile("s_waitcnt vmcnt(%0)" ::"n"(NW[1]) : "memory"); break;
                    case 2: asm volatile("s_waitcnt vmcnt(%0)" ::"n"(NW[2]) : "memory"); break;
                    case 3: asm volatile("s_waitcnt vmcnt(%0)" ::"n"(NW[3]) : "memory"); break;
                    case 4: asm volatile("s_waitcnt vmcnt(%0)" ::"n"(NW[4]) : "memory"); break;
                    case 5: asm volatile("s_waitcnt vmcnt(%0)" ::"n"(NW[5]) : "memory"); break;
                    case 6: asm volatile("s_waitcnt vmcnt(%0)" ::"n"(NW[6]) : "memory"); break;
                    default: asm volatile("s_waitcnt vmcnt(%0)" ::"n"(NW[7]) : "memory"); break;
                }
            }
#pragma unroll
            for (int it = 0; it < 4; ++it) {
                const int row = it * 4 + (lane >> 4);
                f32x4 v = *reinterpret_cast<const f32x4*>(reg + row * 256 + ((ch ^ row) << 4));
                float* o = reinterpret_cast<float*>(a.out) + (mrow0 + row) * a.ldo + nb + ch * 4;
                if (EPI == EPI_RESID_F32 && XRING) {
                    const f32x4 x = *reinterpret_cast<const f32x4*>(xring + (mi & 3) * 4096 + it * 1024 + lane * 16);
#pragma unroll
                    for (int r = 0; r < 4; ++r) v[r] = x[r] + g4[r] * v[r];
                } else if (EPI == EPI_RESID_F32) {
                    f32x4 x = {0.f, 0.f, 0.f, 0.f};
                    if (!(a.dbg & 1)) x = *reinterpret_cast<const f32x4*>(a.resid + (mrow0 + row) * a.ldr + nb + ch * 4);
                    if (has_gate && !shared_gate)
                        g4 = *reinterpret_cast<const f32x4*>(gate + ((mrow0 + row) / a.rows_per_sample) * a.gate_sample_stride + nb + ch * 4);
#pragma unroll
                    for (int r = 0; r < 4; ++r) v[r] = x[r] + g4[r] * v[r];
                }
                if (XRING || !(a.dbg & 2)) *reinterpret_cast<f32x4*>(o) = v;
                if (FOLD == FOLD_PRODUCER) {
                    const bf16x4 pk = {(bf16_t)(v[0] * sc4[0]), (bf16_t)(v[1] * sc4[1]), (bf16_t)(v[2] * sc4[2]), (bf16_t)(v[3] * sc4[3])};
                    if (XRING || !(a.dbg & 4)) *reinterpret_cast<bf16x4*>(a.xs + (mrow0 + row) * a.ldxs + nb + ch * 4) = pk;
                    const float s1 = row16_sum((v[0] + v[1]) + (v[2] + v[3]));
                    const float s2 = row16_sum((v[0] * v[0] + v[1] * v[1]) + (v[2] * v[2] + v[3] * v[3]));
                    const bool keep = (lane & 15) == it;
                    k1 = keep ? s1 : k1; k2 = keep ? s2 : k2;
                }
            }
            rs1[mi] = k1; rs2[mi] = k2;
            if (XRING && mi < 4) request_pass(mi + 4);
        }
        if (FOLD == FOLD_PRODUCER && !(a.dbg & 8)) {
            if ((lane & 15) < 4) {
#pragma unroll
                for (int mi = 0; mi < 8; ++mi)
                    *reinterpret_cast<f32x2*>(reg + (mi * 16 + (lane & 15) * 4 + (lane >> 4)) * 8) = (f32x2){rs1[mi], rs2[mi]};
            }
            asm volatile("s_waitcnt lgkmcnt(0)" ::: "memory");
            G256_BARRIER();
            const int tid = threadIdx.x;
            if (tid < 256) {
                const char* src = stage_base + (tid >> 7) * 4 * 4096 + (tid & 127) * 8;
                f32x2 t = *reinterpret_cast<const f32x2*>(src);
#pragma unroll
                for (int w = 1; w < 4; ++w) { const f32x2 u = *reinterpret_cast<const f32x2*>(src + w * 4096); t[0] += u[0]; t[1] += u[1]; }
                *reinterpret_cast<f32x2*>(a.stats_out + ((long)(n0 >> 8) * a.M + m0 + tid) * 2) = t;
            }
        }
    }
}

template <int NWP, int W_TILE_ROWS>
struct Stream256 {
    int wvo[NWP], xavo[2], xbvo[2];
    int wds[NWP], xads[2], xbds[2];
    const char* sxb = nullptr;
    const char* swb = nullptr;
    int s_it = 0, s_kt = 0, s_inc = 128;

    __device__ __forceinline__ Stream256(const GemmArgs& a, int wave, int lane) {
#pragma unroll
        for (int q = 0; q < 2; ++q) {
            const int pj = wave * 2 + q;
            const int r0 = pj < 8 ? pj * 8 : 128 + (pj - 8) * 8;
            const int ra = r0 + (lane >> 3), rb = ra + 64;
            xavo[q] = ra * (int)a.ldx * 2 + (((lane & 7) ^ ((ra >> 1) & 7)) << 4);
            xbvo[q] = rb * (int)a.ldx * 2 + (((lane & 7) ^ ((rb >> 1) & 7)) << 4);
            xads[q] = r0 * 128;
            xbds[q] = (r0 + 64) * 128;
        }
    }
    __device__ __forceinline__ void seek(const GemmArgs& a, const Tile256List& tl, int it) {
        int tm, tn;
        tl.tile(it, tm, tn);
        sxb = reinterpret_cast<const char*>(a.X + (long)(tm * 256) * a.ldx);
        swb = reinterpret_cast<const char*>(a.W + (long)tn * W_TILE_ROWS * a.ldw);
    }
    __device__ __forceinline__ void advance(const GemmArgs& a, const Tile256List& tl) {
        sxb += s_inc; swb += s_inc;
        if (++s_kt == (a.K >> 6)) {
            s_kt = 0;
            if (++s_it < tl.count) seek(a, tl, s_it);
            else { sxb -= s_inc; swb -= s_inc; s_inc = 0; s_kt = -0x40000000; }
        }
    }
    static __device__ __forceinline__ void piece(const char* src, char* dst) {
        __builtin_amdgcn_global_load_lds((const __attribute__((address_space(1))) void*)src, (__attribute__((address_space(3))) void*)dst, 16, 0, 0);
    }
    __device__ __forceinline__ void issue_w(char* buf) const {
#pragma unroll
        for (int q = 0; q < NWP; ++q) piece(swb + wvo[q], buf + wds[q]);
    }
    __device__ __forceinline__ void issue_xa(char* buf) const {
#pragma unroll
        for (int q = 0; q < 2; ++q) piece(sxb + xavo[q], buf + xads[q]);
    }
    __device__ __forceinline__ void issue_xb(char* buf) const {
#pragma unroll
        for (int q = 0; q < 2; ++q) piece(sxb + xbvo[q], buf + xbds[q]);
    }
};

struct KTileLanes {
    int xb[2], wb[2];
    __device__ __forceinline__ KTileLanes(int grp, int wcol0, int lrow, int lchk) {
        const int sw = (lrow >> 1) & 7;
        const int xrb = (grp * 128 + lrow) * 128, wrb = G256_W_OFF + (wcol0 + lrow) * 128;
        xb[0] = xrb + ((lchk ^ sw) << 4); xb[1] = xrb + (((4 + lchk) ^ sw) << 4);
        wb[0] = wrb + ((lchk ^ sw) << 4); wb[1] = wrb + (((4 + lchk) ^ sw) << 4);
    }
};

template <int PH> using Phase = std::integral_constant<int, PH>;
template <int NF, bool W_LDS, class Req, class WRegs>
__device__ __forceinline__ void ktile256(const char* st, const KTileLanes& ln, f32x4 (&acc)[NF][8], Req&& request, WRegs&& wregs) {
    bf16x8 wf[NF], xf[4];
    auto phase = [&](auto ph) {
        constexpr int PH = decltype(ph)::value, KH = PH >> 1, MH = PH & 1;
        if constexpr (W_LDS && MH == 0) {
#pragma unroll
            for (int i = 0; i < NF; ++i) wf[i] = *reinterpret_cast<const bf16x8*>(st + ln.wb[KH] + i * 2048);
        }
#pragma unroll
        for (int i = 0; i < 4; ++i) xf[i] = *reinterpret_cast<const bf16x8*>(st + ln.xb[KH] + (MH * 4 + i) * 2048);
        request(ph);
        G256_BARRIER();
        if constexpr (!W_LDS && MH == 0) wregs(ph, wf);
        __builtin_amdgcn_s_setprio(1);
#pragma unroll
        for (int ni = 0; ni < NF; ++ni)
#pragma unroll
            for (int mi = 0; mi < 4; ++mi)
                acc[ni][MH * 4 + mi] = __builtin_amdgcn_mfma_f32_16x16x32_bf16(wf[ni], xf[mi], acc[ni][MH * 4 + mi], 0, 0, 0);
        __builtin_amdgcn_s_setprio(0);
        G256_BARRIER();
    };
    phase(Phase<0>{}); phase(Phase<1>{}); phase(Phase<2>{}); phase(Phase<3>{});
}

__device__ __forceinline__ void g256_fold_stats_dma(const GemmArgs& a, int m0, int wave, int lane, char* stage_reg) {
    if (wave < 2 * a.stats_parts) {
        const float* src = a.stats_in + ((long)(wave >> 1) * a.M + m0 + (wave & 1) * 128) * 2 + lane * 4;
        __builtin_amdgcn_global_load_lds((const __attribute__((address_space(1))) void*)src,
                                         (__attribute__((address_space(3))) void*)(stage_reg + G256_STATS_OFF), 16, 0, 0);
    }
}
```

ldt_amd/csrc/gemm_256.hip:

```cpp
#include <stdlib.h>

#include <map>
#include <mutex>
#include <tuple>

#include "gemm256_tile.h"
#include "attn_tile.h"

template <int EPI, int FOLD = FOLD_NONE, int XRING = 0, int WREG = 0, int KLONG = 0>
__global__ __launch_bounds__(512) void gemm_bf16_nt_256f_kernel(const GemmArgs a) {
    static_assert(!WREG || XRING == 1, "WREG: one tile per workgroup");
    extern __shared__ __attribute__((aligned(16))) char smem2[];
    const int tid = threadIdx.x;
    const int lane = tid & 63;
    const int wave = __builtin_amdgcn_readfirstlane(tid >> 6);
    const int grp = wave >> 2, wn = wave & 3;
    const int lrow = lane & 15, lchk = lane >> 4;
    const int nkt = a.K >> 6;

    const Tile256List tl(a.M / 256, a.N / 256, a.group_m, gridDim.x, blockIdx.x);
    if (tl.count == 0) return;
    auto tile_of = [&](int it, int& m0, int& n0) {
        int tm, tn;
        tl.tile(it, tm, tn);
        m0 = tm * 256; n0 = tn * 256;
    };

    Stream256<4, 256> S(a, wave, lane);
#pragma unroll
    for (int q = 0; q < 4; ++q) {
        const int r = (wave * 4 + q) * 8 + (lane >> 3);
        S.wvo[q] = r * (int)a.ldw * 2 + (((lane & 7) ^ ((r >> 1) & 7)) << 4);
        S.wds[q] = G256_W_OFF + (wave * 4 + q) * 1024;
    }
    int gk = 0;
    S.seek(a, tl, 0);
    const char* wrp = nullptr;
    const char* wnext = nullptr;
    int w_kt = 0;
    const int wlane = lane * 16, wlane2 = lane * 16 + 4096;
    typedef int i32x4 __attribute__((ext_vector_type(4)));
    i32x4 w0[4], w1[4];
    auto wbase = [&](int it) {
        int m0, n0;
        tile_of(it, m0, n0);
        return reinterpret_cast<const char*>(a.Wp) + (long)((n0 >> 6) + wn) * nkt * 8192;
    };
    auto wload_h0 = [&]() {
        const unsigned long wb = ((unsigned long)(unsigned)__builtin_amdgcn_readfirstlane((int)((unsigned long)wrp >> 32)) << 32) |
                                 (unsigned long)(unsigned)__builtin_amdgcn_readfirstlane((int)(unsigned long)wrp);
#define WLD(dst, voff, imm) asm volatile("global_load_dwordx4 %0, %1, %2 offset:" #imm : "=v"(dst) : "v"(voff), "s"(wb) : "memory")
        WLD(w0[0], wlane, 0); WLD(w0[1], wlane, 1024); WLD(w0[2], wlane, 2048); WLD(w0[3], wlane, 3072);
    };
    auto wload_h1 = [&]() {
        const unsigned long wb = ((unsigned long)(unsigned)__builtin_amdgcn_readfirstlane((int)((unsigned long)wrp >> 32)) << 32) |
                                 (unsigned long)(unsigned)__builtin_amdgcn_readfirstlane((int)(unsigned long)wrp);
        WLD(w1[0], wlane2, 0); WLD(w1[1], wlane2, 1024); WLD(w1[2], wlane2, 2048); WLD(w1[3], wlane2, 3072);
#undef WLD
        wrp += 8192;
        if (++w_kt == nkt) { w_kt = 0; wrp = wnext; }
    };
    if (WREG) wrp = wbase(0);

    const float* gate = a.gate;
    if (EPI == EPI_RESID_F32 && gate && a.step_ptr) gate += (long)(*a.step_ptr) * a.gate_step_stride;
    const int step = ((FOLD != FOLD_NONE) && a.step_ptr) ? *a.step_ptr : 0;
    const float* ln_scale = (FOLD == FOLD_PRODUCER) ? a.ln_scale + (long)step * a.ln_step_stride : nullptr;
    const float* fold_S = (FOLD == FOLD_CONSUMER) ? a.fold_S + (long)step * a.fold_step_stride : nullptr;
    const float* fold_C = (FOLD == FOLD_CONSUMER) ? a.fold_C + (long)step * a.fold_step_stride : nullptr;
    f32x4 g4_pre = {1.f, 1.f, 1.f, 1.f}, sc4_pre = {0.f, 0.f, 0.f, 0.f};
    const bool pre_ok = (EPI == EPI_RESID_F32) && gate && a.gate_sample_stride == 0;
    if (EPI == EPI_RESID_F32) {
        int m0, n0;
        tile_of(0, m0, n0);
        if (pre_ok) g4_pre = *reinterpret_cast<const f32x4*>(gate + n0 + wn * 64 + (lane & 15) * 4);
        if (FOLD == FOLD_PRODUCER) sc4_pre = *reinterpret_cast<const f32x4*>(ln_scale + n0 + wn * 64 + (lane & 15) * 4);
    }

    if (WREG) {
        wload_h0();
        __builtin_amdgcn_sched_barrier(0);
        S.issue_xa(smem2); S.issue_xb(smem2); S.advance(a, tl);
        S.issue_xa(smem2 + G256_BUF_BYTES); S.issue_xb(smem2 + G256_BUF_BYTES); S.advance(a, tl);
        asm volatile("s_waitcnt vmcnt(6)" ::: "memory");
    } else {
        S.issue_w(smem2); S.issue_xa(smem2); S.issue_xb(smem2); S.advance(a, tl);
        S.issue_w(smem2 + G256_BUF_BYTES); S.issue_xa(smem2 + G256_BUF_BYTES); S.issue_xb(smem2 + G256_BUF_BYTES); S.advance(a, tl);
        asm volatile("s_waitcnt vmcnt(10)" ::: "memory");
    }
    G256_BARRIER();
    if (EPI == EPI_RESID_F32) asm volatile("" : "+v"(g4_pre), "+v"(sc4_pre));

    const KTileLanes ln(grp, wn * 64, lrow, lchk);
    constexpr int EPI_VMEM = (EPI == EPI_BF16 || EPI == EPI_GELU_BF16 || EPI == EPI_RELU_BF16) ? 16
                             : (FOLD == FOLD_PRODUCER) ? 57 : 32;
    char* stage_reg = smem2 + G256_RING_BYTES + wave * 4096;
    bool prev_staged = false;

    for (int it = 0; it < tl.count; ++it) {
        int m0, n0;
        tile_of(it, m0, n0);
        f32x4 acc[4][8];
#pragma unroll
        for (int i = 0; i < 4; ++i)
#pragma unroll
            for (int jj = 0; jj < 8; ++jj) acc[i][jj] = (f32x4){0.f, 0.f, 0.f, 0.f};
        if (WREG) wnext = wbase(it);
        if (grp == 1) G256_BARRIER();

        enum { KT_PLAIN = 0, KT_FIRST = 1 , KT_SECOND = 2, KT_FOLD_DMA = 4, KT_FOLD_FINAL = 8 };
        auto ktile = [&](auto flags_c) {
            constexpr int FL = decltype(flags_c)::value;
            constexpr bool SKIP = (FL & KT_FIRST) != 0;
            char* nb = smem2 + ((gk + 1) & 1) * G256_BUF_BYTES;
            auto request = [&](auto ph) {
                constexpr int PH = decltype(ph)::value;
                if constexpr (PH == 0) {
                    if (WREG) wload_h1();
                    else if (!SKIP) S.issue_w(nb);
                    if (FL & KT_FOLD_DMA) {
                        g256_fold_stats_dma(a, m0, wave, lane, stage_reg);
                        if (wave < 4 && lane < 32) {
                            const float* src = (wave < 2 ? fold_S : fold_C) + n0 + (wave & 1) * 128 + lane * 4;
                            __builtin_amdgcn_global_load_lds((const __attribute__((address_space(1))) void*)src,
                                                             (__attribute__((address_space(3))) void*)(stage_reg + G256_SC_OFF), 16, 0, 0);
                        }
                    }
                    if ((FL & KT_FOLD_FINAL) && wave < 4) g256_fold_finalize(smem2 + G256_RING_BYTES, tid, a.stats_parts, a.K);
                    constexpr int P0W = SKIP ? 8 : 4;
                    constexpr bool AFTER_EPI = (FL & KT_FIRST) || (!WREG && (FL & KT_SECOND));
                    if (AFTER_EPI && prev_staged) asm volatile("s_waitcnt vmcnt(%0)" ::"n"(P0W + EPI_VMEM > 63 ? 63 : P0W + EPI_VMEM) : "memory");
                    else asm volatile("s_waitcnt vmcnt(%0)" ::"n"(P0W) : "memory");
                } else if constexpr (PH == 1) {
                    if (!SKIP) S.issue_xa(nb);
                } else if constexpr (PH == 2) {
                    if (!SKIP) { S.issue_xb(nb); S.advance(a, tl); }
                    if (WREG) {
                        wload_h0();
                        if (SKIP) asm volatile("s_waitcnt vmcnt(4)" ::: "memory");
                        else asm volatile("s_waitcnt vmcnt(8)" ::: "memory");
                    }
                } else {
                    constexpr int P3W = WREG ? (SKIP ? 4 : 6) : 2;
                    if (!WREG && SKIP && prev_staged) asm volatile("s_waitcnt vmcnt(%0)" ::"n"(2 + EPI_VMEM > 63 ? 63 : 2 + EPI_VMEM) : "memory");
                    else asm volatile("s_waitcnt vmcnt(%0)" ::"n"(P3W) : "memory");
                }
            };
            auto wregs = [&](auto ph, bf16x8 (&wf)[4]) {
                if constexpr (decltype(ph)::value == 0) {
                    asm volatile("" : "+v"(w0[0]), "+v"(w0[1]), "+v"(w0[2]), "+v"(w0[3]));
#pragma unroll
                    for (int i = 0; i < 4; ++i) wf[i] = __builtin_bit_cast(bf16x8, w0[i]);
                } else {
                    asm volatile("" : "+v"(w1[0]), "+v"(w1[1]), "+v"(w1[2]), "+v"(w1[3]));
#pragma unroll
                    for (int i = 0; i < 4; ++i) wf[i] = __builtin_bit_cast(bf16x8, w1[i]);
                }
            };
            ktile256<4, !WREG>(smem2 + (gk & 1) * G256_BUF_BYTES, ln, acc, request, wregs);
            ++gk;
        };
#define KTL(f) std::integral_constant<int, (f)>{}
        if (FOLD == FOLD_CONSUMER) {
            ktile(KTL(KT_FIRST)); ktile(KTL(KT_FOLD_DMA | KT_SECOND)); ktile(KTL(KT_PLAIN)); ktile(KTL(KT_FOLD_FINAL));
            for (int kt = 4; kt < nkt; ++kt) ktile(KTL(KT_PLAIN));
        } else {
            ktile(KTL(KT_FIRST)); ktile(KTL(KT_SECOND));
            for (int kt = 2; kt < nkt; ++kt) ktile(KTL(KT_PLAIN));
        }
#undef KTL
        if (grp == 0) G256_BARRIER();

        prev_staged = true;
        if (!XRING) {
            char* pb = smem2 + ((gk + 1) & 1) * G256_BUF_BYTES;
            if (!WREG) S.issue_w(pb);
            S.issue_xa(pb); S.issue_xb(pb); S.advance(a, tl);
        }
        if (XRING) {
            asm volatile("s_waitcnt vmcnt(0)" ::: "memory");
            G256_BARRIER();
            g256_epilogue_staged<EPI, FOLD, 1>(a, acc, m0, n0, grp, wn, lane, lrow, lchk, gate, stage_reg, smem2 + G256_RING_BYTES, ln_scale,
                                               true, g4_pre, sc4_pre, smem2 + wave * 16384);
            break;
        } else
            g256_epilogue_staged<EPI, FOLD>(a, acc, m0, n0, grp, wn, lane, lrow, lchk, gate, stage_reg, smem2 + G256_RING_BYTES, ln_scale,
                                            it == 0 && (pre_ok || FOLD == FOLD_PRODUCER), g4_pre, sc4_pre);
    }
    asm volatile("s_waitcnt vmcnt(0)" ::: "memory");
}

template <int FOLD>
__global__ __launch_bounds__(512) void gemm_qkv_attn256_kernel(const GemmArgs a) {
    static_assert(FOLD == FOLD_NONE || FOLD == FOLD_CONSUMER, "qkv+attention: plain or LN-folded consumer");
    extern __shared__ __attribute__((aligned(16))) char smem2[];
    const int tid = threadIdx.x;
    const int lane = tid & 63;
    const int wave = __builtin_amdgcn_readfirstlane(tid >> 6);
    const int grp = wave >> 2, wn = wave & 3;
    const int lrow = lane & 15, lchk = lane >> 4;
    const int nkt = a.K >> 6;
    const int hidden = a.N / 3, heads = hidden / 64;

    const Tile256List tl(a.M / 256, heads, a.group_m, gridDim.x, blockIdx.x);
    if (tl.count == 0) return;
    auto tile_of = [&](int it, int& m0, int& hd) {
        int tm;
        tl.tile(it, tm, hd);
        m0 = tm * 256;
    };

    Stream256<3, 64> S(a, wave, lane);
#pragma unroll
    for (int q = 0; q < 3; ++q) {
        const int pj = wave * 3 + q;
        const int r = pj * 8 + (lane >> 3);
        const int gr = (pj >> 3) * hidden + (r & 63);
        S.wvo[q] = gr * (int)a.ldw * 2 + (((lane & 7) ^ ((r >> 1) & 7)) << 4);
        S.wds[q] = G256_W_OFF + pj * 1024;
    }
    int gk = 0;
    S.seek(a, tl, 0);
    const int step = ((FOLD != FOLD_NONE) && a.step_ptr) ? *a.step_ptr : 0;
    const float* fold_S = (FOLD == FOLD_CONSUMER) ? a.fold_S + (long)step * a.fold_step_stride : nullptr;
    const float* fold_C = (FOLD == FOLD_CONSUMER) ? a.fold_C + (long)step * a.fold_step_stride : nullptr;

    S.issue_w(smem2); S.issue_xa(smem2); S.issue_xb(smem2); S.advance(a, tl);
    asm volatile("s_waitcnt vmcnt(2)" ::: "memory");
    G256_BARRIER();

    const KTileLanes ln(grp, wn * 48, lrow, lchk);
    constexpr int EPI_VMEM = 4;
    bool prev_staged = false;
    const int r32 = lane & 31, hh = lane >> 5;
    AttnLaneOffs<64> lo;
    lo.init(lane);

    for (int it = 0; it < tl.count; ++it) {
        int m0, hd;
        tile_of(it, m0, hd);
        f32x4 acc[3][8];
#pragma unroll
        for (int i = 0; i < 3; ++i)
#pragma unroll
            for (int jj = 0; jj < 8; ++jj) acc[i][jj] = (f32x4){0.f, 0.f, 0.f, 0.f};
        f32x4 add4[3];
#pragma unroll
        for (int ni = 0; ni < 3; ++ni) {
            const int c = wn * 48 + ni * 16 + lchk * 4;
            add4[ni] = (FOLD == FOLD_NONE && a.bias) ? *reinterpret_cast<const f32x4*>(a.bias + (c >> 6) * hidden + hd * 64 + (c & 63)) : (f32x4){0.f, 0.f, 0.f, 0.f};
        }
        if (grp == 1) G256_BARRIER();

        enum { KT_PLAIN = 0, KT_FIRST = 1, KT_FOLD_DMA = 4, KT_FOLD_FINAL = 8 };
        auto ktile = [&](auto flags_c) {
            constexpr int FL = decltype(flags_c)::value;
            char* nb = smem2 + ((gk + 1) & 1) * G256_BUF_BYTES;
            auto request = [&](auto ph) {
                constexpr int PH = decltype(ph)::value;
                if constexpr (PH == 0) {
                    S.issue_w(nb);
                    if (FL & KT_FOLD_DMA) {
                        char* stage_reg = smem2 + G256_RING_BYTES + wave * 4096;
                        g256_fold_stats_dma(a, m0, wave, lane, stage_reg);
                        if (wave < 6 && lane < 16) {
                            const int seg = wave < 3 ? wave : wave - 3;
                            const float* src = (wave < 3 ? fold_S : fold_C) + seg * hidden + hd * 64 + lane * 4;
                            __builtin_amdgcn_global_load_lds((const __attribute__((address_space(1))) void*)src,
                                                             (__attribute__((address_space(3))) void*)(stage_reg + G256_SC_OFF), 16, 0, 0);
                        }
                    }
                    if ((FL & KT_FOLD_FINAL) && wave < 4) g256_fold_finalize(smem2 + G256_RING_BYTES, tid, a.stats_parts, a.K);
                    constexpr int P0W = 3;
                    if ((FL & KT_FIRST) && prev_staged) asm volatile("s_waitcnt vmcnt(%0)" ::"n"(P0W + EPI_VMEM) : "memory");
                    else asm volatile("s_waitcnt vmcnt(%0)" ::"n"(P0W) : "memory");
                } else if constexpr (PH == 1) {
                    S.issue_xa(nb);
                } else if constexpr (PH == 2) {
                    S.issue_xb(nb); S.advance(a, tl);
                } else {
                    asm volatile("s_waitcnt vmcnt(2)" ::: "memory");
                }
            };
            ktile256<3, true>(smem2 + (gk & 1) * G256_BUF_BYTES, ln, acc, request, [](auto, auto&) {});
            ++gk;
        };
#define KTL(f) std::integral_constant<int, (f)>{}
        if (FOLD == FOLD_CONSUMER) {
            ktile(KTL(KT_FIRST)); ktile(KTL(KT_FOLD_DMA)); ktile(KTL(KT_PLAIN)); ktile(KTL(KT_FOLD_FINAL));
            for (int kt = 4; kt < nkt; ++kt) ktile(KTL(KT_PLAIN));
        } else {
            ktile(KTL(KT_FIRST));
            for (int kt = 1; kt < nkt; ++kt) ktile(KTL(KT_PLAIN));
        }
#undef KTL
        if (grp == 0) G256_BARRIER();
        prev_staged = true;

        char* stage_base = smem2 + G256_RING_BYTES;
        char* kvb = smem2 + ((gk + 1) & 1) * G256_BUF_BYTES;
        f32x4 s4[3];
        float rr[8], nm[8];
        if (FOLD == FOLD_CONSUMER) {
#pragma unroll
            for (int mi = 0; mi < 8; ++mi) {
                const int R = grp * 128 + mi * 16 + lrow;
                const f32x2 t = *reinterpret_cast<const f32x2*>(stage_base + (R >> 7) * 4096 + G256_STATS_OFF + (R & 127) * 8);
                rr[mi] = t[0]; nm[mi] = t[1];
            }
#pragma unroll
            for (int ni = 0; ni < 3; ++ni) {
                const int c = wn * 48 + ni * 16 + lchk * 4;
                s4[ni] = *reinterpret_cast<const f32x4*>(stage_base + (c >> 6) * 4096 + G256_SC_OFF + (c & 63) * 4);
                add4[ni] = *reinterpret_cast<const f32x4*>(stage_base + (3 + (c >> 6)) * 4096 + G256_SC_OFF + (c & 63) * 4);
            }
            asm volatile("s_waitcnt lgkmcnt(0)" ::: "memory");
            G256_BARRIER();
        }
#pragma unroll
        for (int mi = 0; mi < 8; ++mi) {
            const int R = grp * 128 + mi * 16 + lrow;
            const int swr = (R >> 1) & 7;
#pragma unroll
            for (int ni = 0; ni < 3; ++ni) {
                f32x4 v = acc[ni][mi];
                if (FOLD == FOLD_CONSUMER) {
#pragma unroll
                    for (int r = 0; r < 4; ++r) v[r] = v[r] * rr[mi] + (nm[mi] * s4[ni][r] + add4[ni][r]);
                } else {
#pragma unroll
                    for (int r = 0; r < 4; ++r) v[r] += add4[ni][r];
                }
                const bf16x4 pk = {(bf16_t)v[0], (bf16_t)v[1], (bf16_t)v[2], (bf16_t)v[3]};
                const int c = wn * 48 + ni * 16 + lchk * 4, seg = c >> 6, cc = c & 63;
                const int sz = seg == 2 ? ((R >> 1) & 1) << 2 : swr;
                char* dst = (seg == 0 ? stage_base : kvb + (seg - 1) * 32768) + R * 128 + (((cc >> 3) ^ sz) << 4) + (cc & 7) * 2;
                *reinterpret_cast<bf16x4*>(dst) = pk;
            }
        }
        asm volatile("s_waitcnt lgkmcnt(0)" ::: "memory");
        G256_BARRIER();

        {
            const int q0 = wave * 32;
            bf16x8 qf[4];
#pragma unroll
            for (int sI = 0; sI < 4; ++sI)
                qf[sI] = *reinterpret_cast<const bf16x8*>(stage_base + (q0 + r32) * 128 + (((hh + 2 * sI) ^ ((r32 >> 1) & 7)) << 4));
            f32x16 oacc[2];
#pragma unroll
            for (int d = 0; d < 2; ++d)
#pragma unroll
                for (int i = 0; i < 16; ++i) oacc[d][i] = 0.f;
            float m_run = -INFINITY, l_run = 0.f;
            f32x16 sa0, sa1, sb0, sb1;
            const char* Kt = kvb;
            const char* Vt = kvb + 32768;
            const float csc = a.attn_scale_log2e;
            attn_scores<64>(Kt, qf, sa0, sa1, lo);
            __builtin_amdgcn_sched_barrier(0);
            attn_scores<64>(Kt + 8192, qf, sb0, sb1, lo);
            __builtin_amdgcn_sched_barrier(0);
            attn_softmax_pv<64>(Vt, sa0, sa1, oacc, m_run, l_run, 0, 256, hh, csc, lo);
            __builtin_amdgcn_sched_barrier(0);
            attn_scores<64>(Kt + 2 * 8192, qf, sa0, sa1, lo);
            __builtin_amdgcn_sched_barrier(0);
            attn_softmax_pv<64>(Vt + 8192, sb0, sb1, oacc, m_run, l_run, 64, 256, hh, csc, lo);
            __builtin_amdgcn_sched_barrier(0);
            attn_scores<64>(Kt + 3 * 8192, qf, sb0, sb1, lo);
            __builtin_amdgcn_sched_barrier(0);
            attn_softmax_pv<64>(Vt + 2 * 8192, sa0, sa1, oacc, m_run, l_run, 128, 256, hh, csc, lo);
            __builtin_amdgcn_sched_barrier(0);
            attn_softmax_pv<64>(Vt + 3 * 8192, sb0, sb1, oacc, m_run, l_run, 192, 256, hh, csc, lo);
            char* ost = stage_base + q0 * 128;
            const float inv = 1.0f / (l_run + __shfl_xor(l_run, 32, 64));
#pragma unroll
            for (int d = 0; d < 2; ++d)
#pragma unroll
                for (int g = 0; g < 4; ++g) {
                    const int chn = d * 4 + g;
                    const bf16x4 pk = {(bf16_t)(oacc[d][4 * g + 0] * inv), (bf16_t)(oacc[d][4 * g + 1] * inv),
                                       (bf16_t)(oacc[d][4 * g + 2] * inv), (bf16_t)(oacc[d][4 * g + 3] * inv)};
                    *reinterpret_cast<bf16x4*>(ost + r32 * 128 + ((chn ^ (r32 & 7)) << 4) + hh * 8) = pk;
                }
            asm volatile("s_waitcnt lgkmcnt(0)" ::: "memory");
            bf16_t* ob = a.attn_o + (((long)(m0 >> 8) * heads + hd) * 256 + q0) * 64;
#pragma unroll
            for (int p4 = 0; p4 < 4; ++p4) {
                const int row = p4 * 8 + (lane >> 3), ch = lane & 7;
                const bf16x8 v = *reinterpret_cast<const bf16x8*>(ost + row * 128 + ((ch ^ (row & 7)) << 4));
                *reinterpret_cast<bf16x8*>(ob + (long)row * 64 + ch * 8) = v;
            }
        }
        asm volatile("s_waitcnt lgkmcnt(0)" ::: "memory");
        G256_BARRIER();
    }
    asm volatile("s_waitcnt vmcnt(0)" ::: "memory");
}

__global__ __launch_bounds__(256) void pack_wfrag_kernel(const bf16_t* __restrict__ W, long ldw, int N, int K, bf16_t* __restrict__ Wp) {
    const long c = (long)blockIdx.x * 256 + threadIdx.x;
    const int nkt = K >> 6;
    if (c >= (long)N * K / 8) return;
    const int lane = (int)(c & 63), f = (int)((c >> 6) & 7);
    const long t = c >> 9;
    const int kt = (int)(t % nkt), n64 = (int)(t / nkt);
    const int n = n64 * 64 + (f & 3) * 16 + (lane & 15), k = kt * 64 + (f >> 2) * 32 + (lane >> 4) * 8;
    *reinterpret_cast<bf16x8*>(Wp + c * 8) = *reinterpret_cast<const bf16x8*>(W + (long)n * ldw + k);
}
int ldt_gemm_pack_wfrag_launch(const bf16_t* W, long ldw, int N, int K, bf16_t* Wp, hipStream_t stream) {
    LDT_REQUIRE(W && Wp && N > 0 && K > 0 && N % 64 == 0 && K % 64 == 0 && ldw >= K && ldw % 8 == 0 && ldt_aligned16(W) && ldt_aligned16(Wp), LDT_ESHAPE,
                "pack_wfrag: N=%d and K=%d must be multiples of 64, rows 16-byte aligned (ldw=%ld)", N, K, ldw);
    const long chunks = (long)N * K / 8;
    hipLaunchKernelGGL(pack_wfrag_kernel, dim3((unsigned)((chunks + 255) / 256)), dim3(256), 0, stream, W, ldw, N, K, Wp);
    return ldt_check_launch("pack_wfrag");
}
static std::atomic<int> g_dbg_wreg{-1};
extern "C" int ldt_dbg_gemm_wreg(int32_t on) { g_dbg_wreg.store(on); return LDT_OK; }
static const bf16_t* dbg_wfrag_cached(const bf16_t* W, long ldw, int N, int K, hipStream_t stream) {
    static std::mutex mu;
    static std::map<std::tuple<const void*, long, int, int>, bf16_t*> cache;
    std::lock_guard<std::mutex> lk(mu);
    auto key = std::make_tuple((const void*)W, ldw, N, K);
    auto itc = cache.find(key);
    if (itc != cache.end()) return itc->second;
    bf16_t* wp = nullptr;
    if (hipMalloc((void**)&wp, (size_t)N * K * 2) != hipSuccess) return nullptr;
    if (ldt_gemm_pack_wfrag_launch(W, ldw, N, K, wp, stream) != LDT_OK) { (void)hipFree(wp); return nullptr; }
    cache[key] = wp;
    return wp;
}

static std::atomic<int> g_group_m{-1};
extern "C" int ldt_dbg_gemm_group_m(int32_t gm) { g_group_m.store(gm); return LDT_OK; }
static std::atomic<int> g_dbg_epi{-1};
extern "C" int ldt_dbg_gemm_epi(int32_t bits) { g_dbg_epi.store(bits); return LDT_OK; }

bool ldt_gemm256_takes(int epi, const GemmArgs* a) {
    return a->K % 64 == 0 && a->K >= 128 && a->M % 256 == 0 && a->N % 256 == 0 && a->ldo % 8 == 0 &&
           (epi != EPI_RESID_F32 || (a->ldr % 4 == 0 && (!a->gate || a->gate_sample_stride % 4 == 0))) &&
           (epi != EPI_RELU_BF16 || !a->skip || a->lds_ % 4 == 0);
}

template <int EPI, int FOLD = FOLD_NONE>
static int launch_256(const GemmArgs* a_in, const GemmRoute& route, hipStream_t stream) {
    static const int gm_env = getenv("LDT_GEMM_GM") ? atoi(getenv("LDT_GEMM_GM")) : -1;
    const int gm_dbg = g_group_m.load();
    GemmArgs a_copy = *a_in;
    a_copy.group_m = gm_dbg >= 0 ? gm_dbg : gm_env >= 0 ? gm_env : gemm256_default_group_m(a_in->M / 256, a_in->N / 256);
    static const bool xring_on = !(getenv("LDT_RESID_RING") && atoi(getenv("LDT_RESID_RING")) == 0);
    const bool xring = (EPI == EPI_RESID_F32 && xring_on && a_in->resid && ldt_aligned16(a_in->resid) && (!a_in->gate || a_in->gate_sample_stride == 0));
    static const int dbg_env = getenv("LDT_DBG_EPI") ? atoi(getenv("LDT_DBG_EPI")) : 0;
    a_copy.dbg = g_dbg_epi.load() >= 0 ? g_dbg_epi.load() : dbg_env;
    const GemmArgs* a = &a_copy;
    LDT_REQUIRE(ldt_gemm256_takes(EPI, a), LDT_ESHAPE, "gemm256: M=%d N=%d must be multiples of 256, K=%d of 64 (>= 128), rows 16-byte aligned", a->M, a->N, a->K);
    static const int wreg_env = getenv("LDT_GEMM_WREG") ? atoi(getenv("LDT_GEMM_WREG")) : -1;
    const int wreg_dbg = g_dbg_wreg.load() >= 0 ? g_dbg_wreg.load() : wreg_env;
    const int grid = route.grid;
    if constexpr (EPI == EPI_RESID_F32) {
        if (xring && route.family == GEMM_ROUTE_256_ONE && a->dbg == 0) {
            if (wreg_dbg == 1 && !a_copy.Wp) a_copy.Wp = dbg_wfrag_cached(a->W, a->ldw, a->N, a->K, stream);
            const bool wreg = a_copy.Wp && wreg_dbg != 0 && ldt_aligned16(a_copy.Wp);
            const bool klong = a->K >= 2048;
#define LAUNCH_XR(W, KL)                                                                                                          \
    do {                                                                                                                          \
        LDT_ENSURE_LDS((&gemm_bf16_nt_256f_kernel<EPI, FOLD, 1, W, KL>), G256_LDS_BYTES, "gemm256f");                              \
        hipLaunchKernelGGL((gemm_bf16_nt_256f_kernel<EPI, FOLD, 1, W, KL>), dim3(grid), dim3(512), G256_LDS_BYTES, stream, *a);   \
    } while (0)
            if (wreg) { if (klong) LAUNCH_XR(1, 1); else LAUNCH_XR(1, 0); }
            else if (klong) LAUNCH_XR(0, 1);
            else LAUNCH_XR(0, 0);
#undef LAUNCH_XR
            return ldt_check_launch("gemm_bf16_nt_256f");
        }
    }
    LDT_ENSURE_LDS((&gemm_bf16_nt_256f_kernel<EPI, FOLD>), G256_LDS_BYTES, "gemm256f");
    hipLaunchKernelGGL((gemm_bf16_nt_256f_kernel<EPI, FOLD>), dim3(grid), dim3(512), G256_LDS_BYTES, stream, *a);
    return ldt_check_launch("gemm_bf16_nt_256f");
}

int ldt_gemm256_launch(int epi, int fold, const GemmArgs* a, const GemmRoute& r, hipStream_t stream) {
    if (fold == FOLD_PRODUCER && epi == EPI_RESID_F32) return launch_256<EPI_RESID_F32, FOLD_PRODUCER>(a, r, stream);
    if (fold == FOLD_CONSUMER && epi == EPI_BF16) return launch_256<EPI_BF16, FOLD_CONSUMER>(a, r, stream);
    if (fold == FOLD_CONSUMER && epi == EPI_GELU_BF16) return launch_256<EPI_GELU_BF16, FOLD_CONSUMER>(a, r, stream);
    if (fold == FOLD_NONE) switch (epi) {
        case EPI_F32: return launch_256<EPI_F32>(a, r, stream);
        case EPI_BF16: return launch_256<EPI_BF16>(a, r, stream);
        case EPI_GELU_BF16: return launch_256<EPI_GELU_BF16>(a, r, stream);
        case EPI_RELU_BF16: return launch_256<EPI_RELU_BF16>(a, r, stream);
        case EPI_RESID_F32: return launch_256<EPI_RESID_F32>(a, r, stream);
    }
    ldt_set_error("gemm: unknown epilogue %d", epi);
    return LDT_EARG;
}

bool ldt_gemm_qkv_attn256_takes(const GemmArgs* a_in, int tokens, int head_dim, bool folded) {
    static const bool on = !(getenv("LDT_QKV_ATTN256") && atoi(getenv("LDT_QKV_ATTN256")) == 0);
    const GemmArgs& g = *a_in;
    if (!on || ldt_gemm_variant_env() != 0 || tokens != 256 || head_dim != 64) return false;
    if (g.M <= 0 || g.N <= 0 || g.N % 192 != 0 || (g.N / 3) % 64 != 0 || g.M % 256 != 0 || g.K % 64 != 0 || g.K < (folded ? 256 : 128)) return false;
    if (folded && (g.stats_parts <= 0 || g.stats_parts > 4 || g.stats_parts * 256 != g.K)) return false;
    const long tiles = (long)(g.M / 256) * ((g.N / 3) / 64);
    return tiles * 8 >= (long)ldt_wg_limit(g.max_wgs) * 5;
}
bool ldt_gemm_qkv_attn256_try(const GemmArgs* a_in, int tokens, int head_dim, bool folded, hipStream_t stream, int* status) {
    const GemmArgs& g = *a_in;
    if (!g.attn_o || !ldt_gemm_qkv_attn256_takes(a_in, tokens, head_dim, folded)) return false;
    if (folded && (!g.stats_in || !g.fold_S || !g.fold_C ||
                   !ldt_aligned16(g.stats_in) || !ldt_aligned16(g.fold_S) || !ldt_aligned16(g.fold_C) || g.fold_step_stride % 4 != 0))
        return false;
    if (!ldt_aligned16(g.X) || !ldt_aligned16(g.W) || !ldt_aligned16(g.attn_o) || (g.bias && !ldt_aligned16(g.bias)) || g.ldx % 8 != 0 || g.ldw % 8 != 0 ||
        g.ldx < g.K || g.ldw < g.K)
        return false;
    const int tm = g.M / 256, tn = (g.N / 3) / 64;
    const long tiles = (long)tm * tn;
    const int lim = ldt_wg_limit(g.max_wgs);
    GemmArgs a = g;
    static const int gm_env = getenv("LDT_QKV_GM") ? atoi(getenv("LDT_QKV_GM")) : getenv("LDT_GEMM_GM") ? atoi(getenv("LDT_GEMM_GM")) : -1;
    a.group_m = gm_env >= 0 ? gm_env : gemm256_default_group_m(tm, tn);
    const int grid = tiles < lim ? (int)tiles : lim;
    auto launch = [&]() -> int {
        if (folded) {
            LDT_ENSURE_LDS((&gemm_qkv_attn256_kernel<FOLD_CONSUMER>), G256_LDS_BYTES, "gemm_qkv_attn256");
            hipLaunchKernelGGL((gemm_qkv_attn256_kernel<FOLD_CONSUMER>), dim3(grid), dim3(512), G256_LDS_BYTES, stream, a);
        } else {
            LDT_ENSURE_LDS((&gemm_qkv_attn256_kernel<FOLD_NONE>), G256_LDS_BYTES, "gemm_qkv_attn256");
            hipLaunchKernelGGL((gemm_qkv_attn256_kernel<FOLD_NONE>), dim3(grid), dim3(512), G256_LDS_BYTES, stream, a);
        }
        return ldt_check_launch("gemm_qkv_attn256");
    };
    *status = launch();
    return true;
}
```

ldt_amd/csrc/gemm_bf16.hip:

```cpp
#include <stdlib.h>

#include "gemm256_tile.h"

#define BK 64

template <int ROWS, int NW = 4>
__device__ __forceinline__ void stage_tile(const bf16_t* __restrict__ g, long ld, int row0, int nrows_total,
                                           int k0, char* lds_tile, int wave, int lane) {
#pragma unroll
    for (int p = 0; p < ROWS / (8 * NW); ++p) {
        const int piece = wave * (ROWS / (8 * NW)) + p;
        const int r = piece * 8 + (lane >> 3);
        const int cdst = lane & 7;
        const int csrc = cdst ^ ((r >> 1) & 7);
        int grow = row0 + r;
        grow = grow < nrows_total ? grow : nrows_total - 1;
        const bf16_t* src = g + (long)grow * ld + k0 + csrc * 8;
        char* dst = lds_tile + piece * 1024;
        __builtin_amdgcn_global_load_lds((const __attribute__((address_space(1))) void*)src,
                                         (__attribute__((address_space(3))) void*)dst, 16, 0, 0);
    }
}

template <int EPI, int TBM, int TBN, int NST = 2, int NW = 4>
__global__ __launch_bounds__(NW * 64) void gemm_bf16_nt_kernel(const GemmArgs a) {
    constexpr int BM = TBM, BN = TBN;
    constexpr int XB = TBM * BK * 2, WB = TBN * BK * 2;
    constexpr int WGM = NW / 2;
    constexpr int MT = TBM / (16 * WGM), NT = TBN / 32;
    constexpr int OPS = (TBM + TBN) / (8 * NW);
    __shared__ __attribute__((aligned(16))) char smem[NST * (XB + WB)];
    const int tid = threadIdx.x;
    const int lane = tid & 63;
    const int wave = __builtin_amdgcn_readfirstlane(tid >> 6);
    const int wm = wave >> 1, wn = wave & 1;

    const int tiles_n = (a.N + BN - 1) / BN;
    const int nwg = gridDim.x;
    const int bid = blockIdx.x;
    const int q = nwg >> 3, r8 = nwg & 7, xcd = bid & 7;
    const int wgid = (xcd < r8 ? xcd * (q + 1) : r8 * (q + 1) + (xcd - r8) * q) + (bid >> 3);
    const int tiles_m = (a.M + BM - 1) / BM;
    const int tile_m = a.col_major ? wgid % tiles_m : wgid / tiles_n, tile_n = a.col_major ? wgid / tiles_m : wgid % tiles_n;
    const int m0 = tile_m * BM, n0 = tile_n * BN;

    f32x4 acc[NT][MT];
#pragma unroll
    for (int i = 0; i < NT; ++i)
#pragma unroll
        for (int j = 0; j < MT; ++j) acc[i][j] = (f32x4){0.f, 0.f, 0.f, 0.f};

    const bf16_t* Xk = a.X;
    const bf16_t* Wk = a.W;
    const int nk = a.K / BK;
    stage_tile<TBM, NW>(Xk, a.ldx, m0, a.M, 0, smem, wave, lane);
    stage_tile<TBN, NW>(Wk, a.ldw, n0, a.N, 0, smem + XB, wave, lane);
    int ahead = 0;
#pragma unroll
    for (int st = 1; st < NST - 1; ++st)
        if (st < nk) {
            stage_tile<TBM, NW>(Xk, a.ldx, m0, a.M, st * BK, smem + st * (XB + WB), wave, lane);
            stage_tile<TBN, NW>(Wk, a.ldw, n0, a.N, st * BK, smem + st * (XB + WB) + XB, wave, lane);
            ++ahead;
        }
    if (NST >= 3 && ahead == 1) asm volatile("s_waitcnt vmcnt(%0)" ::"n"(OPS) : "memory");
    else asm volatile("s_waitcnt vmcnt(0)" ::: "memory");
    __builtin_amdgcn_s_barrier();

    const int lrow = lane & 15;
    const int lchk = lane >> 4;
    int cur = 0;
    for (int kt = 0; kt < nk; ++kt) {
        char* sx = smem + cur * (XB + WB);
        char* sw = sx + XB;
        if (kt + NST - 1 < nk) {
            int nb = cur + NST - 1; nb = nb >= NST ? nb - NST : nb;
            char* nx = smem + nb * (XB + WB);
            stage_tile<TBM, NW>(Xk, a.ldx, m0, a.M, (kt + NST - 1) * BK, nx, wave, lane);
            stage_tile<TBN, NW>(Wk, a.ldw, n0, a.N, (kt + NST - 1) * BK, nx + XB, wave, lane);
        }
#pragma unroll
        for (int ks = 0; ks < 2; ++ks) {
            bf16x8 wf[NT], xf[MT];
            const int c = ks * 4 + lchk;
#pragma unroll
            for (int i = 0; i < NT; ++i) {
                const int rw = wn * (TBN / 2) + i * 16 + lrow;
                wf[i] = *reinterpret_cast<const bf16x8*>(sw + rw * 128 + ((c ^ ((rw >> 1) & 7)) << 4));
            }
#pragma unroll
            for (int i = 0; i < MT; ++i) {
                const int rx = wm * (TBM / WGM) + i * 16 + lrow;
                xf[i] = *reinterpret_cast<const bf16x8*>(sx + rx * 128 + ((c ^ ((rx >> 1) & 7)) << 4));
            }
#pragma unroll
            for (int ni = 0; ni < NT; ++ni)
#pragma unroll
                for (int mi = 0; mi < MT; ++mi)
                    acc[ni][mi] = __builtin_amdgcn_mfma_f32_16x16x32_bf16(wf[ni], xf[mi], acc[ni][mi], 0, 0, 0);
        }
        const int left = nk - 2 - kt;
        if (NST >= 3 && left >= 1) asm volatile("s_waitcnt vmcnt(%0)" ::"n"(OPS) : "memory");
        else asm volatile("s_waitcnt vmcnt(0)" ::: "memory");
        __builtin_amdgcn_s_barrier();
        cur = cur + 1 == NST ? 0 : cur + 1;
    }

    const float* gate = a.gate;
    if (EPI == EPI_RESID_F32 && gate && a.step_ptr) gate += (long)(*a.step_ptr) * a.gate_step_stride;
#pragma unroll
    for (int mi = 0; mi < MT; ++mi) {
        const int m = m0 + wm * (TBM / WGM) + mi * 16 + lrow;
        if (m >= a.M) continue;
        const float* grow = nullptr;
        if (EPI == EPI_RESID_F32 && gate) grow = gate + (long)(m / a.rows_per_sample) * a.gate_sample_stride;
#pragma unroll
        for (int ni = 0; ni < NT; ++ni) {
            const int n = n0 + wn * (TBN / 2) + ni * 16 + lchk * 4;
            if (n >= a.N) continue;
            f32x4 v = acc[ni][mi];
            const bool full = (n + 3 < a.N);
            float b[4] = {0.f, 0.f, 0.f, 0.f};
            if (a.bias) {
                if (full) { const f32x4 t = *reinterpret_cast<const f32x4*>(a.bias + n); b[0] = t[0]; b[1] = t[1]; b[2] = t[2]; b[3] = t[3]; }
                else for (int r = 0; r < 4; ++r) if (n + r < a.N) b[r] = a.bias[n + r];
            }
#pragma unroll
            for (int r = 0; r < 4; ++r) v[r] += b[r];
            if (EPI == EPI_F32) {
                float* o = reinterpret_cast<float*>(a.out) + (long)m * a.ldo + n;
                if (full) *reinterpret_cast<f32x4*>(o) = v;
                else for (int r = 0; r < 4; ++r) if (n + r < a.N) o[r] = v[r];
            } else if (EPI == EPI_RESID_F32) {
                float* o = reinterpret_cast<float*>(a.out) + (long)m * a.ldo + n;
                const float* rs = a.resid + (long)m * a.ldr + n;
                if (full) {
                    f32x4 x = *reinterpret_cast<const f32x4*>(rs);
                    if (grow) { const f32x4 g = *reinterpret_cast<const f32x4*>(grow + n);
#pragma unroll
                        for (int r = 0; r < 4; ++r) x[r] = x[r] + g[r] * v[r];
                    } else {
#pragma unroll
                        for (int r = 0; r < 4; ++r) x[r] = x[r] + v[r];
                    }
                    *reinterpret_cast<f32x4*>(o) = x;
                } else {
                    for (int r = 0; r < 4; ++r) if (n + r < a.N) o[r] = rs[r] + (grow ? grow[n + r] : 1.f) * v[r];
                }
            } else {
                if (EPI == EPI_GELU_BF16) {
#pragma unroll
                    for (int r = 0; r < 4; r += 2) {
                        const f32x2 gg = gelu_erf_fast2((f32x2){v[r], v[r + 1]});
                        v[r] = gg[0]; v[r + 1] = gg[1];
                    }
                }
                if (EPI == EPI_RELU_BF16) {
                    if (a.skip) {
                        const bf16_t* sk = a.skip + (long)m * a.lds_ + n;
                        for (int r = 0; r < 4; ++r) if (n + r < a.N) v[r] += (float)sk[r];
                    }
#pragma unroll
                    for (int r = 0; r < 4; ++r) v[r] = fmaxf(v[r], 0.f);
                }
                bf16_t* o = reinterpret_cast<bf16_t*>(a.out) + (long)m * a.ldo + n;
                if (full) {
                    bf16x4 pk = {(bf16_t)v[0], (bf16_t)v[1], (bf16_t)v[2], (bf16_t)v[3]};
                    *reinterpret_cast<bf16x4*>(o) = pk;
                } else for (int r = 0; r < 4; ++r) if (n + r < a.N) o[r] = (bf16_t)v[r];
            }
        }
    }
}

int ldt_gemm_variant_env() {
    static int v = -1;
    if (v < 0) { const char* e = getenv("LDT_GEMM_FORCE"); v = e ? atoi(e) : 0; }
    return v;
}
bool ldt_gemm_lnfold_v1_route(int M, int D, int F, int max_wgs) {
    const int lim = ldt_wg_limit(max_wgs);
    auto small = [&](int N) { return (long)((M + 255) / 256) * ((N + 255) / 256) * 8 < (long)lim * 5; };
    if (!(ldt_gemm_variant_env() == 0 && M % 128 == 0 && D % 64 == 0 && F % 64 == 0 && D <= 1024 && small(D) && small(3 * D) && small(F))) return false;
    if ((long)(M / 64) * (D / 128) * 8 < (long)lim * 5) return false;
    return ldt_gemm_mid_lnfold_takes(EPI_RESID_F32, M, D, D) && ldt_gemm_mid_lnfold_takes(EPI_RESID_F32, M, D, F) &&
           ldt_gemm_mid_lnfold_takes(EPI_BF16, M, 3 * D, D) && ldt_gemm_mid_lnfold_takes(EPI_GELU_BF16, M, F, D);
}

GemmRoute ldt_gemm_decide(int epi, const GemmArgs* a, int granule) {
    GemmRoute r{};
    if (!(a->M > 0 && a->N > 0 && a->K > 0) || a->K % BK != 0 || a->ldo % 4 != 0) return r;
    const int lim = ldt_wg_limit(a->max_wgs);
    auto take_256 = [&]() {
        const int tm = a->M / 256, tn = a->N / 256, tiles = tm * tn;
        r.grid = tiles < lim ? tiles : lim;
        r.bm = r.bn = 256;
        r.tiles_per_wg = Tile256List::max_count(tm, tn, r.grid);
        r.family = r.tiles_per_wg == 1 ? GEMM_ROUTE_256_ONE : GEMM_ROUTE_256_MULTI;
    };
    if (granule) {
        const bool producer = epi == EPI_RESID_F32;
        if (!producer && epi != EPI_BF16 && epi != EPI_GELU_BF16) return r;
        if (granule == 32) {
            if (a->M % 128 != 0 || a->N % 64 != 0 || a->K < 128) return r;
            ldt_gemm_mid_route(epi, producer ? FOLD_PRODUCER : FOLD_CONSUMER, a, &r);
        } else if (granule == 256) {
            if (a->M % 256 != 0 || a->N % 256 != 0 || a->K < 256 || !ldt_gemm256_takes(epi, a)) return r;
            if (!producer && (a->K % 256 != 0 || a->K > 1024)) return r;
            take_256();
        }
        return r;
    }
    const int force = ldt_gemm_variant_env();
    const int tiles256 = ((a->M + 255) / 256) * ((a->N + 255) / 256);
    const bool big = tiles256 * 8 >= lim * 5 && a->N > 128;
    if (force == 0 && !big) {
        if (ldt_gemm_mid_route(epi, FOLD_NONE, a, &r)) return r;
    }
    if ((force == 256 || (force == 0 && big)) && ldt_gemm256_takes(epi, a)) { take_256(); return r; }
    auto ntiles = [&](int bm, int bn) { return (long)((a->M + bm - 1) / bm) * ((a->N + bn - 1) / bn); };
    const int shape = (force == 128 || ntiles(128, 128) >= 2 * LDT_NUM_CUS) ? 0 : (ntiles(128, 64) >= 2 * LDT_NUM_CUS ? 1 : 2);
    r.family = GEMM_ROUTE_V1;
    r.v1_shape = shape;
    r.v1_stages = shape == 2 ? 3 : 2;
    r.bm = shape == 2 ? 64 : 128;
    r.bn = shape == 0 ? 128 : 64;
    r.tiles_per_wg = 1;
    r.grid = (int)ntiles(r.bm, r.bn);
    return r;
}

static int gemm_check_epilogue_operands(const char* who, int epi, const GemmArgs* a) {
    if (epi == EPI_RESID_F32) {
        LDT_REQUIRE(a->resid && a->ldr % 4 == 0 && ldt_aligned16(a->resid), LDT_EALIGN, "%s: resid missing/misaligned", who);
        LDT_REQUIRE(!a->gate || (a->rows_per_sample > 0 && ldt_aligned16(a->gate) && a->gate_sample_stride % 4 == 0 && a->gate_step_stride % 4 == 0),
                    LDT_EARG, "%s: gate needs rows_per_sample>0 and 16-byte aligned strides", who);
    }
    LDT_REQUIRE(!a->bias || ldt_aligned16(a->bias), LDT_EALIGN, "%s: bias must be 16-byte aligned", who);
    return LDT_OK;
}

int ldt_gemm_lnfold_launch(int epi, const GemmArgs* a, hipStream_t stream) {
    const int width = epi == EPI_RESID_F32 ? a->N : a->K;
    const bool v1 = a->stats_parts > 0 && a->stats_parts * 32 == width && a->stats_parts * 256 != width;
    if (v1) LDT_REQUIRE(a->M > 0 && a->M % 128 == 0 && a->N % 64 == 0 && a->K >= 128 && a->K % BK == 0, LDT_ESHAPE,
                        "gemm_lnfold (v1 route): M=%d must be a multiple of 128, N=%d of 64, K=%d >= 128, K %% 64 == 0", a->M, a->N, a->K);
    else LDT_REQUIRE(a->M > 0 && a->N > 0 && a->K >= 256 && a->M % 256 == 0 && a->N % 256 == 0 && a->K % BK == 0, LDT_ESHAPE,
                     "gemm_lnfold: M=%d N=%d must be multiples of 256 and K=%d >= 256, K %% 64 == 0", a->M, a->N, a->K);
    LDT_REQUIRE(a->ldx % 8 == 0 && a->ldw % 8 == 0 && a->ldx >= a->K && a->ldw >= a->K && a->ldo % 8 == 0 && ldt_aligned16(a->X) &&
                ldt_aligned16(a->W) && ldt_aligned16(a->out), LDT_EALIGN, "gemm_lnfold: operands must be 16-byte aligned (ldx=%ld ldw=%ld ldo=%ld)",
                a->ldx, a->ldw, a->ldo);
    if (epi == EPI_RESID_F32) {
        if (const int rc = gemm_check_epilogue_operands("gemm_lnfold", epi, a)) return rc;
        LDT_REQUIRE(a->xs && a->ln_scale && a->stats_out && a->ldxs % 4 == 0 && a->ldxs >= a->N && ldt_aligned16(a->xs) &&
                    ldt_aligned16(a->ln_scale) && a->ln_step_stride % 4 == 0 && ldt_aligned16(a->stats_out), LDT_EARG,
                    "gemm_lnfold: producer needs xs / ln_scale / stats_out (16-byte aligned)");
        const GemmRoute r = ldt_gemm_decide(epi, a, v1 ? 32 : 256);
        if (v1) {
            if (r.family == GEMM_ROUTE_MID) return ldt_gemm_mid_launch(epi, FOLD_PRODUCER, a, r, stream);
            ldt_set_error("gemm_lnfold: statistics per 32 columns are the mid-size tile kernel's; it does not take M=%d N=%d K=%d as a producer", a->M, a->N, a->K);
            return LDT_ESHAPE;
        }
        LDT_REQUIRE(r.family == GEMM_ROUTE_256_ONE || r.family == GEMM_ROUTE_256_MULTI, LDT_ESHAPE,
                    "gemm256: M=%d N=%d must be multiples of 256, K=%d of 64 (>= 128), rows 16-byte aligned", a->M, a->N, a->K);
        return ldt_gemm256_launch(epi, FOLD_PRODUCER, a, r, stream);
    }
    LDT_REQUIRE(epi == EPI_BF16 || epi == EPI_GELU_BF16, LDT_EARG, "gemm_lnfold: epilogue %d has no folded form", epi);
    LDT_REQUIRE(a->stats_in && a->fold_S && a->fold_C && ldt_aligned16(a->stats_in) && ldt_aligned16(a->fold_S) && ldt_aligned16(a->fold_C) &&
                a->fold_step_stride % 4 == 0, LDT_EARG, "gemm_lnfold: consumer needs stats_in, fold_S, fold_C (16-byte aligned)");
    const GemmRoute r = ldt_gemm_decide(epi, a, v1 ? 32 : 256);
    if (v1) {
        LDT_REQUIRE(a->stats_parts <= 32, LDT_ESHAPE, "gemm_lnfold (v1 route): K=%d > 1024 input channels", a->K);
        if (r.family == GEMM_ROUTE_MID) return ldt_gemm_mid_launch(epi, FOLD_CONSUMER, a, r, stream);
        ldt_set_error("gemm_lnfold: statistics per 32 columns are the mid-size tile kernel's; it does not take M=%d N=%d K=%d as a consumer", a->M, a->N, a->K);
        return LDT_ESHAPE;
    }
    LDT_REQUIRE(a->stats_parts >= 1 && a->stats_parts <= 4 && a->stats_parts * 256 == a->K, LDT_EARG,
                "gemm_lnfold: consumer needs stats_in[K/256 <= 4][M][2] (or [K/32][M][2] for the small-batch kernels); K=%d parts=%d", a->K, a->stats_parts);
    LDT_REQUIRE(r.family == GEMM_ROUTE_256_ONE || r.family == GEMM_ROUTE_256_MULTI, LDT_ESHAPE,
                "gemm256: M=%d N=%d must be multiples of 256, K=%d of 64 (>= 128), rows 16-byte aligned", a->M, a->N, a->K);
    return ldt_gemm256_launch(epi, FOLD_CONSUMER, a, r, stream);
}


int ldt_gemm_launch(int epi, const GemmArgs* a, hipStream_t stream) {
    LDT_REQUIRE(a->M > 0 && a->N > 0 && a->K > 0, LDT_ESHAPE, "gemm: empty problem M=%d N=%d K=%d", a->M, a->N, a->K);
    LDT_REQUIRE(a->K % BK == 0, LDT_ESHAPE, "gemm: K=%d must be a multiple of %d (pad activations/weights)", a->K, BK);
    LDT_REQUIRE(a->ldx % 8 == 0 && a->ldw % 8 == 0 && ldt_aligned16(a->X) && ldt_aligned16(a->W), LDT_EALIGN,
                "gemm: X/W rows must be 16-byte aligned (ldx=%ld ldw=%ld)", a->ldx, a->ldw);
    LDT_REQUIRE(a->ldx >= a->K && a->ldw >= a->K, LDT_ESHAPE, "gemm: leading dims smaller than K");
    LDT_REQUIRE(a->ldo % 4 == 0 && ldt_aligned16(a->out), LDT_EALIGN, "gemm: out must be 16-byte aligned, ldo%%4==0 (ldo=%ld)", a->ldo);
    if (const int rc = gemm_check_epilogue_operands("gemm", epi, a)) return rc;
    const GemmRoute r = ldt_gemm_decide(epi, a, 0);
    if (r.family == GEMM_ROUTE_MID) return ldt_gemm_mid_launch(epi, FOLD_NONE, a, r, stream);
    if (r.family == GEMM_ROUTE_256_ONE || r.family == GEMM_ROUTE_256_MULTI) return ldt_gemm256_launch(epi, FOLD_NONE, a, r, stream);
    LDT_REQUIRE(r.family == GEMM_ROUTE_V1, LDT_ESHAPE, "gemm: no kernel takes M=%d N=%d K=%d", a->M, a->N, a->K);
    const int shape = r.v1_shape;
    auto ntiles = [&](int bm, int bn) { return (long)((a->M + bm - 1) / bm) * ((a->N + bn - 1) / bn); };
    dim3 block(256);
    static const int v1_map_env = getenv("LDT_GEMM_V1_MAP") ? atoi(getenv("LDT_GEMM_V1_MAP")) : -1;
    GemmArgs a_v1 = *a;
    {
        const long tm = (a->M + r.bm - 1) / r.bm, tn = (a->N + r.bn - 1) / r.bn;
        a_v1.col_major = v1_map_env >= 0 ? v1_map_env : (tn >= 3 * tm ? 1 : 0);
    }
    a = &a_v1;
#define LAUNCH_V1(E)                                                                                                     \
    do {                                                                                                                 \
        if (shape == 0) hipLaunchKernelGGL((gemm_bf16_nt_kernel<E, 128, 128>), dim3((unsigned)ntiles(128, 128)), block, 0, stream, *a); \
        else if (shape == 1) hipLaunchKernelGGL((gemm_bf16_nt_kernel<E, 128, 64>), dim3((unsigned)ntiles(128, 64)), block, 0, stream, *a); \
        else hipLaunchKernelGGL((gemm_bf16_nt_kernel<E, 64, 64, 3>), dim3((unsigned)ntiles(64, 64)), block, 0, stream, *a);  \
    } while (0)
    switch (epi) {
        case EPI_F32: LAUNCH_V1(EPI_F32); break;
        case EPI_BF16: LAUNCH_V1(EPI_BF16); break;
        case EPI_GELU_BF16: LAUNCH_V1(EPI_GELU_BF16); break;
        case EPI_RELU_BF16: LAUNCH_V1(EPI_RELU_BF16); break;
        case EPI_RESID_F32: LAUNCH_V1(EPI_RESID_F32); break;
        default: ldt_set_error("gemm: unknown epilogue %d", epi); return LDT_EARG;
    }
#undef LAUNCH_V1
    return ldt_check_launch("gemm_bf16_nt");
}
```

ldt_amd/csrc/kernels.h:

```cpp
#pragma once
#include "common.h"

enum { EPI_F32 = 0, EPI_BF16 = 1, EPI_GELU_BF16 = 2, EPI_RELU_BF16 = 3, EPI_RESID_F32 = 4 };
#define LDT_NUM_CUS 256
static inline int ldt_wg_limit(int max_wgs) { return (max_wgs > 0 && max_wgs < LDT_NUM_CUS) ? max_wgs : LDT_NUM_CUS; }
enum { ACT_NONE = 0, ACT_SILU = 1, ACT_RELU = 2, ACT_GELU = 3 };

struct GemmArgs {
    const bf16_t* X; long ldx;
    const bf16_t* W; long ldw;
    const float* bias;
    void* out; long ldo;
    const float* resid; long ldr;
    const bf16_t* skip; long lds_;
    const float* gate;
    long gate_sample_stride;
    int rows_per_sample;
    const int* step_ptr; long gate_step_stride;
    int M, N, K;
    bf16_t* xs; long ldxs; const float* ln_scale; long ln_step_stride; float* stats_out;
    const float* stats_in; int stats_parts; const float* fold_S; const float* fold_C; long fold_step_stride;
    int group_m;
    int dbg;
    int max_wgs;
    int col_major;
    bf16_t* attn_o; float attn_scale_log2e;
    const bf16_t* attn_k; const bf16_t* attn_v; long attn_ldkv; long attn_kv_batch_stride;
    const bf16_t* Wp;
};

struct LnArgs {
    const float* x; long ldx;
    bf16_t* y; long ldy;
    const float* w; const float* b;
    const float* shift; const float* scale;
    long mod_sample_stride; int rows_per_sample;
    const int* step_ptr; long mod_step_stride;
    long M; int C;
};

struct AttnArgs {
    const bf16_t* Q; long ldq; long q_batch_stride;
    const bf16_t* K; long ldk; long kv_batch_stride;
    const bf16_t* V; long ldv;
    bf16_t* O;
    int B, H, Nq, Nk;
    float scale_log2e;
    const bf16_t* Wo; const float* bo; float* X; long ldx; const float* gate; long gate_sample_stride;
};

struct StepArgs {
    const float* x; const float* params; const float* noise;
    float* x_out; float* x_mean_out;
    const float* coef; const int* step_ptr; int step_host; int mode;
    long n; long elem_offset; long noise_step_stride;
    uint32_t seed_lo, seed_hi;
    int philox_mul, philox_add;
    float* traj;
};

struct SgemmArgs {
    const float* A; long lda; const float* B; long ldb; const float* bias;
    void* C; long ldc; int out_bf16; int act_in; int act_out;
    int M, N, K;
};

int ldt_gemm_launch(int epi, const GemmArgs* a, hipStream_t stream);
enum { GEMM_ROUTE_NONE = 0, GEMM_ROUTE_256_ONE = 1, GEMM_ROUTE_256_MULTI = 2, GEMM_ROUTE_MID = 3, GEMM_ROUTE_V1 = 4 };
struct GemmRoute {
    int family, bm, bn;
    int tiles_per_wg;
    int grid;
    int v1_shape, v1_stages;
};
GemmRoute ldt_gemm_decide(int epi, const GemmArgs* a, int granule);
bool ldt_gemm_mid_route(int epi, int fold, const GemmArgs* a, GemmRoute* r);
int ldt_gemm_mid_launch(int epi, int fold, const GemmArgs* a, const GemmRoute& route, hipStream_t stream);
bool ldt_gemm_mid_lnfold_takes(int epi, int M, int N, int K);
bool ldt_gemm_mid_qkv_attn_try(const GemmArgs* a, int tokens, int head_dim, bool folded, hipStream_t stream, int* status);
bool ldt_gemm_qkv_attn256_try(const GemmArgs* a, int tokens, int head_dim, bool folded, hipStream_t stream, int* status);
bool ldt_gemm_mid_q_xattn_try(const GemmArgs* a, int tokens, int cond_tokens, int head_dim, hipStream_t stream, int* status);
bool ldt_gemm_mid_qkv_attn_takes(const GemmArgs* a, int tokens, int head_dim, bool folded);
bool ldt_gemm_qkv_attn256_takes(const GemmArgs* a, int tokens, int head_dim, bool folded);
bool ldt_gemm_mid_q_xattn_takes(const GemmArgs* a, int tokens, int cond_tokens, int head_dim);
bool ldt_gemm_lnfold_v1_route(int M, int D, int F, int max_wgs);
int ldt_gemm_lnfold_launch(int epi, const GemmArgs* a, hipStream_t stream);
int ldt_ln_launch(const LnArgs* a, hipStream_t s);
int ldt_attn_launch(const AttnArgs* a, int dh, hipStream_t s);
int ldt_attn_route(int B, int H, int Nq, int Nk, int dh);
int ldt_attn_narrow_launch(const AttnArgs* a, int dh, hipStream_t s);
int ldt_attn_oproj_launch(const AttnArgs* a, int dh, hipStream_t s);
struct AttnBwdArgs {
    const bf16_t* Q; long ldq; long q_bs;
    const bf16_t* K; long ldk; const bf16_t* V; long ldv; long kv_bs;
    const bf16_t* O; const bf16_t* dO;
    float* stats;
    bf16_t* dQ; long lddq; long dq_bs;
    bf16_t* dK; long lddk; bf16_t* dV; long lddv; long dkv_bs;
    int B, H, Nq, Nk;
    float scale;
};
int ldt_attn_bwd_launch(const AttnBwdArgs* a, int dh, hipStream_t s);
int ldt_attn_bwd_narrow_launch(const AttnBwdArgs* a, int dh, hipStream_t s);
template <int N, int M>
__device__ __forceinline__ void narrow_halve(float* v, int lr) {
    const bool up = (lr & M) != 0;
#pragma unroll
    for (int k = 0; k < N / 2; ++k) {
        const float keep = up ? v[k + N / 2] : v[k];
        const float send = up ? v[k] : v[k + N / 2];
        v[k] = keep + __shfl_xor(send, M, 64);
    }
}
int ldt_cast_pad_launch(const float* src, long lds, bf16_t* dst, long ldd, long rows, int cols, int cols_pad, hipStream_t s);
int ldt_sampler_step_launch(const StepArgs* a, hipStream_t s);
int ldt_advance_step_launch(int* step_ptr, hipStream_t s);
int ldt_philox_normal_launch(float* out, long n, long elem_offset, int step, uint32_t k0, uint32_t k1, hipStream_t s);
int ldt_sinusoid_launch(const float* t, const float* freq, float* e, int n, int half, hipStream_t s);
int ldt_sgemm_launch(const SgemmArgs* a, hipStream_t s);
bool ldt_sgemm_mfma_try(const SgemmArgs* a, hipStream_t s, int* status);
bool ldt_skinny_linear_try(const SgemmArgs* a, hipStream_t s, int* status);

int ldt_fps_launch(const float* xyz, int B, int n, int m, int skip_near_origin, int* idx, hipStream_t s);
int ldt_fps_wave_launch(const float* xyz, int B, int n, int m, int skip_near_origin, int* idx, hipStream_t s);
int ldt_knn_launch(const float* xyz, const float* centers, int B, int n, int S, int k, int* out, float* dist_out, hipStream_t s);
int ldt_group_launch(const float* feat, const float* xyz, const int* fps_idx, const int* knn_idx, const float* alpha,
                     const float* beta, double* stats, int B, int n, int S, int k, int D, bf16_t* U, int ldu,
                     int center_mode, float* gmean, hipStream_t s);
int ldt_group_stats_launch(const float* feat, const float* xyz, const int* fps_idx, const int* knn_idx, double* stats,
                           int B, int n, int S, int k, int D, hipStream_t s);
struct GroupMlpArgs {
    const float* feat; const float* xyz;
    const int* fps_idx; const int* knn_idx;
    const float* alpha; const float* beta;
    const double* stats;
    const bf16_t* wimg;
    const float* b1; const float* b2; const float* b3;
    int B, n, S, k, flat;
    float* out;
};
int ldt_grouper_mlp_launch(const GroupMlpArgs* a, hipStream_t s);
int ldt_norm_points_launch(const float* xyz, int B, int n, float* out, hipStream_t s);
int ldt_mixture_seed_launch(const float* eps, const float* sig, const float* mu, const float* logits, int n_mix, int D, long rows, float* out, hipStream_t s);
int ldt_gather_rows_launch(const float* src, const int* idx, int B, int n, int S, int C, float* out, hipStream_t s);
int ldt_maxpool_launch(const void* in, int in_bf16, long ld, long G, int n, int C, float* out, hipStream_t s);
int ldt_actnorm_launch(float* x, const float* shift, const float* log_scale, long B, long per_sample, hipStream_t s);
int ldt_reparam_launch(const float* post, const float* noise, float* out, long ldo, float* mu_out, float* lv_out,
                       long rows, int z, float lo, float hi, hipStream_t s);
int ldt_chamfer_launch(const float* a, const float* b, int B, int na, int nb, float* dl, float* dr, hipStream_t s);
struct LnLinArgs {
    const float* x; long ldx; long M;
    const float* ln_w; const float* ln_b; const float* shift; const float* scale; long mod_sample_stride; int rows_per_sample;
    const bf16_t* w; const float* bias; int N;
    bf16_t* out; long ldo;
};
struct MlpArgs {
    float* x; long ldx; long M;
    const float* ln_w; const float* ln_b;
    const float* shift; const float* scale;
    const float* gate;
    long mod_sample_stride; int rows_per_sample;
    const bf16_t* w_up; const float* b_up;
    const bf16_t* w_dn; const float* b_dn;
    bf16_t* x_bf16; long ldxb;
    LnLinArgs next;
};
int ldt_ln_mlp_launch(const MlpArgs* a, int C, hipStream_t st);
int ldt_ln_linear_launch(const LnLinArgs* a, int C, hipStream_t st);
int ldt_chamfer_pairwise_launch(const float* x, const float* y, int S, int R, int n, int m, float* cd, hipStream_t st);
int ldt_emd_approx_launch(const float* x, const float* y, int S, int R, int n, int m, int pairwise, float* out, hipStream_t st);
int ldt_fold_monitor_launch(const float* stats, int parts, long M, int K, float* out, hipStream_t s);
int ldt_cond_rows_launch(const float* temb, const float* extra, float* c, void* c_bf16, const int* step_ptr, int batch, int t_dim, int silu_out, hipStream_t s);
```

ldt_amd/score.py:

```python
import ctypes
import os

import numpy as np
import torch
import torch.nn as nn

from . import ops
from ._lib import ACT_NONE, ACT_SILU, MAX_BLOCKS, ScorePlan, check, lib
from .layers import FinalLayer, LabelEmbedding, ResidualBlock, TimeEmbedding, conv_w, params_fingerprint


class Score(nn.Module):
    def __init__(self, cfg):
        super().__init__()
        self.cfg = cfg
        self.z_dim = cfg.z_dim
        self.out_dim = self.z_dim
        self.z_scale = cfg.z_scale
        self.hidden_size = cfg.hidden_size
        self.num_heads = cfg.num_heads
        self.condition = cfg.condition
        self.num_steps = cfg.num_steps
        self.norm = cfg.norm
        self.t_dim = cfg.t_dim
# ... 129 lines not shown
        elif torch.is_tensor(img_cond):
            extra = img_cond.to(self._device(), torch.float32).contiguous()
        kv, S = (None, 0)
        if torch.is_tensor(pts_cond):
            kv, S = self.project_condition(pts_cond)
        return extra, kv, S

    def _cross_panels(self, l):
        P = self.packed()
        if ("w_q", l) not in P:
            blk = self.Transformer[l]
            with torch.no_grad():
                wq = conv_w(blk.fc_q).float().contiguous(); wkv = conv_w(blk.fc_kv).float().contiguous()
                P[("w_q", l)] = ops.cast_pad_bf16(wq, wq.shape[1]); P[("b_q", l)] = blk.fc_q.bias.detach().float().contiguous()
                P[("w_kv", l)] = ops.cast_pad_bf16(wkv, wkv.shape[1]); P[("b_kv", l)] = blk.fc_kv.bias.detach().float().contiguous()
        return P[("w_q", l)], P[("b_q", l)], P[("w_kv", l)], P[("b_kv", l)]

    def project_condition(self, pts_cond):
        key = (pts_cond.data_ptr(), pts_cond._version, tuple(pts_cond.shape))
        self.packed()
        if key not in self._cond_cache:
            from ._lib import EPI_BF16
            B, C, S = pts_cond.shape
            y = pts_cond.to(self._device(), torch.float32).transpose(1, 2).contiguous().view(B * S, C)
            yb = ops.cast_pad_bf16(y, C)
            kv = {}
            for l in range(0, self.num_blocks, 2):
                _, _, wkv, bkv = self._cross_panels(l)
                kv[l] = ops.gemm_bf16(yb, wkv, bkv, EPI_BF16)
            self._cond_cache = {key: (kv, S, pts_cond)}
        return self._cond_cache[key][:2]

    def _workspace(self, B, T, slot=0):
        k = (B, T, self._device(), slot)
        if k not in self._ws:
            dev, M, D = self._device(), B * T, self.hidden_size
            bf = dict(dtype=torch.bfloat16, device=dev)
            self._ws = {kk: v for kk, v in self._ws.items() if kk[:3] == k[:3]}
            self._ws[k] = {
                "xin": torch.zeros((M, ops.pad64(self.z_dim)), **bf),
                "X": torch.empty((M, D), dtype=torch.float32, device=dev),
                "Hb": torch.empty((M, D), **bf), "QKV": torch.empty((M, 3 * D), **bf),
                "Ob": torch.empty((M, D), **bf), "U": torch.empty((M, self.Transformer[0].mlp.out.in_channels), **bf),
                "stats": torch.empty((max(D // 32, 1), M, 2), dtype=torch.float32, device=dev),
            }
        return self._ws[k]

    def plan(self, B, T, mod, mod_step_stride, mod_sample_stride, kv_cond=None, cond_tokens=0, fold=None, slot=0, gemm_wgs=0, monitor=None,
             monitor_every=0):
        P, W = self.packed(), self._workspace(B, T, slot)
        p = ScorePlan()
        p.gemm_wgs = gemm_wgs
        p.hidden, p.heads, p.blocks = self.hidden_size, self.num_heads, self.num_blocks
        p.z_dim, p.z_pad, p.mlp_hidden = self.z_dim, ops.pad64(self.z_dim), W["U"].shape[1]
        p.tokens, p.batch = T, B
        p.w_in, p.b_in = P["w_in"].data_ptr(), P["b_in"].data_ptr()
        for l in range(self.num_blocks):
            for nm in ("qkv", "o", "up", "dn"):
                getattr(p, "w_" + nm)[l] = P["w_" + nm][l].data_ptr()
                getattr(p, "b_" + nm)[l] = P["b_" + nm][l].data_ptr()
        p.w_out, p.b_out = P["w_out"].data_ptr(), P["b_out"].data_ptr()
        p.mod, p.mod_step_stride, p.mod_sample_stride = mod.data_ptr(), mod_step_stride, mod_sample_stride
        for nm in ("xin", "X", "Hb", "QKV", "Ob", "U"):
            setattr(p, nm, W[nm].data_ptr())
        if kv_cond:
            p.cond_tokens = cond_tokens
            for l, kv in kv_cond.items():
                wq, bq, _, _ = self._cross_panels(l)
                p.w_q[l], p.b_q[l], p.kv_cond[l] = wq.data_ptr(), bq.data_ptr(), kv.data_ptr()
        if fold is not None:
            if mod_sample_stride != 0:
                raise ValueError("LN folding needs batch-shared modulation (mod_sample_stride == 0)")
            p.fold, p.fold_step_stride, p.stats = fold.data_ptr(), fold.stride(0), W["stats"].data_ptr()
            if monitor is not None:
                p.fold_monitor = monitor.data_ptr()
                p.fold_monitor_every = int(monitor_every)
        p._keep = (P, W, mod, kv_cond, fold, monitor)
        return p

    def _frequencies(self):
        if self._freq is None or self._freq.device != self._device():
            half = self.TimeEmbedding.t_emb_dim // 2
            s = np.log(10000) / (half - 1)
            self._freq = torch.exp(torch.arange(half) * -s).to(self._device())
        return self._freq

    def time_table(self, t, extra_c=None):
        te = self.TimeEmbedding.mlp
        e = ops.sinusoid(t.contiguous(), self._frequencies())
        h = ops.sgemm(e, te[0].weight, te[0].bias, act_out=ACT_SILU)
        c = ops.sgemm(h, te[2].weight, te[2].bias)
        if extra_c is not None:
            c = ops.add_f32(c, extra_c.expand_as(c))
        D = self.hidden_size
        mod = torch.empty((t.numel(), self.n_mod), dtype=torch.float32, device=t.device)
        for l, blk in enumerate(self.Transformer):
            lin = blk.adaLN[1]
            ops.sgemm(c, lin.weight, lin.bias, act_in=ACT_SILU, out=mod[:, l * 6 * D:(l + 1) * 6 * D])
        lin = self.ln_out.adaLN[1]
        ops.sgemm(c, lin.weight, lin.bias, act_in=ACT_SILU, out=mod[:, self.num_blocks * 6 * D:])
        return c, mod

    def can_fold(self, B, T, gemm_wgs=0):
        self.collect_fold_ratio()
        mode = int(os.environ.get("LDT_LN_FOLD", "1"))
        D, M = self.hidden_size, B * T
        F = self.Transformer[0].mlp.out.in_channels if not self.unet else 0
        if (self._fold_disabled and mode != 2) or mode == 0 or self.host_blocks:
            return False
        route = int(lib().ldt_score_lnfold_route(M, D, F, gemm_wgs))
        if route == 2:
            return mode == 2 or bool(int(os.environ.get("LDT_LN_FOLD_SMALL", "1")))
        if route == 1:
            return True
        return mode == 2 and M % 256 == 0 and D % 256 == 0 and D <= 1024 and F % 256 == 0

    FOLD_MAX_MEAN_RATIO = 16.0

    def fold_probe(self, x, step_index, mod, fold):
        B, T, _ = x.shape
        mon = torch.zeros(1, dtype=torch.float32, device=x.device)
        step = torch.full((1,), int(step_index), dtype=torch.int32, device=x.device)
        plan = self.plan(B, T, mod, self.n_mod, 0, fold=fold, slot=0, monitor=mon)
        out = torch.empty_like(x)
        check(lib().ldt_score_forward(ctypes.byref(plan), x.contiguous().data_ptr(), out.data_ptr(), step.data_ptr(), ops.stream_ptr()),
              "ldt_score_forward")
        return self.note_fold_ratio(float(mon.item()))

    def note_fold_ratio(self, ratio):
        self.fold_ratio_seen = max(self.fold_ratio_seen, ratio)
        if ratio > self.FOLD_MAX_MEAN_RATIO and not self._fold_disabled:
            import warnings
            self._fold_disabled = True
            warnings.warn("ldt_amd.Score: a LayerNorm input row has mean^2 / variance = %.1f (> %.0f): the LN-folded GEMM epilogues "
                          "would lose accuracy there; using the LayerNorm kernels from now on (LDT_LN_FOLD=2 forces folding)"
                          % (ratio, self.FOLD_MAX_MEAN_RATIO))
        return ratio

    def defer_fold_ratio(self, monitor):
        self.collect_fold_ratio()
        self._fold_pending = monitor

    def collect_fold_ratio(self):
        if self._fold_pending is not None:
            mon, self._fold_pending = self._fold_pending, None
            self.note_fold_ratio(float(mon.item()))
        return self.fold_ratio_seen

    def fold_table(self, mod):
        P = self.packed()
        D, F = self.hidden_size, self.Transformer[0].mlp.out.in_channels
        n = mod.shape[0]
        fb = 6 * D + 2 * F
        fold = torch.empty((n, self.num_blocks * fb), dtype=torch.float32, device=mod.device)
        ones = torch.ones((1, D), dtype=torch.float32, device=mod.device)
        for l in range(self.num_blocks):
            m0, f0 = l * 6 * D, l * fb
            for (w, b, sh, sc, off) in ((P["w_qkv"][l], P["b_qkv"][l], m0, m0 + D, f0),
                                        (P["w_up"][l], P["b_up"][l], m0 + 3 * D, m0 + 4 * D, f0 + 6 * D)):
                wf = ops.widen_bf16(w)
                N = wf.shape[0]
                ops.sgemm(mod[:, sc:sc + D], wf, ops.sgemm(ones, wf).view(-1), out=fold[:, off:off + N])
                ops.sgemm(mod[:, sh:sh + D], wf, b, out=fold[:, off + N:off + 2 * N])
        return fold

    def label_embedding(self, label):
        if not hasattr(self, "LabelEmbedding"):
            raise ValueError("label given but cfg.score.num_categorys <= 1 (no LabelEmbedding, score.py:103-106)")
        le = self.LabelEmbedding
        e = le.label_emb.weight.detach()[label.to(self._device()).long()].float().contiguous()
        h = ops.sgemm(e, le.mlp[0].weight, le.mlp[0].bias, act_out=ACT_SILU)
        return ops.sgemm(h, le.mlp[2].weight, le.mlp[2].bias)

    @torch.no_grad()
    def forward(self, x, t, label=None, condition=None):
        if not x.is_cuda:
            raise RuntimeError("Score.forward: x is on %s; the HIP path has no CPU fallback" % x.device)
        if self.training and self.dropout > 0:
            raise RuntimeError("Score.forward: dropout=%g needs eval() — the HIP path is the inference (sampling) path" % self.dropout)
        B, T, z = x.shape
        assert z == self.z_dim
        x = x.contiguous().float()
        if self.unet:
            return self._forward_unet(x, t, label, condition)
        if self.host_blocks:
            return self._forward_host_blocks(x, t, label, condition)
        extra, kv, S = self.condition_embedding(label, condition)
        _, mod = self.time_table(t.to(x).float(), extra_c=extra)
        plan = self.plan(B, T, mod, 0, self.n_mod, kv_cond=kv, cond_tokens=S)
        out = torch.empty_like(x)
        check(lib().ldt_score_forward(ctypes.byref(plan), x.data_ptr(), out.data_ptr(), None, ops.stream_ptr()),
              "ldt_score_forward")
        return out

    @torch.no_grad()
    def forward_shared_t(self, x, t, fold=None):
        if not x.is_cuda:
            raise RuntimeError("Score.forward_shared_t: x is on %s; the HIP path has no CPU fallback" % x.device)
        if self.host_blocks:
            raise NotImplementedError("forward_shared_t: the U-Net / non-LayerNorm variants are host-driven (forward)")
        B, T, z = x.shape
        assert z == self.z_dim
        x = x.contiguous().float()
        _, mod = self.time_table(torch.tensor([float(t)], dtype=torch.float32, device=x.device))
        use_fold = self.can_fold(B, T) if fold is None else bool(fold)
        plan = self.plan(B, T, mod, self.n_mod, 0, fold=self.fold_table(mod) if use_fold else None)
        out = torch.empty_like(x)
        check(lib().ldt_score_forward(ctypes.byref(plan), x.data_ptr(), out.data_ptr(), None, ops.stream_ptr()),
              "ldt_score_forward")
        return out

    @torch.no_grad()
    def forward_table_row(self, x, step_index, mod, fold=None):
        if not x.is_cuda:
            raise RuntimeError("Score.forward_table_row: x is on %s; the HIP path has no CPU fallback" % x.device)
        B, T, z = x.shape
        assert z == self.z_dim and mod.shape[1] == self.n_mod and 0 <= int(step_index) < mod.shape[0]
        x = x.contiguous().float()
        step = torch.full((1,), int(step_index), dtype=torch.int32, device=x.device)
        plan = self.plan(B, T, mod, self.n_mod, 0, fold=fold)
        out = torch.empty_like(x)
        check(lib().ldt_score_forward(ctypes.byref(plan), x.data_ptr(), out.data_ptr(), step.data_ptr(), ops.stream_ptr()),
              "ldt_score_forward")
        return out

    def _forward_host_blocks(self, x, t, label, condition):
        from ._lib import EPI_F32
        from .blocks import final_layer, residual_block
        if isinstance(condition, dict):
            if not hasattr(self, "c_net"):
                raise ValueError("a raw condition dict needs cfg.score.condition=True (ConditionNet, score.py:64-65)")
            condition = self.c_net(condition)
        pts_cond, img_cond = (None, 0.) if condition is None else condition
        B, T, _ = x.shape
        P = self.packed()
        c = self.time_embedding(t.to(x).float())
        if label is not None:
            c = ops.add_f32(c, self.label_embedding(label))
        elif torch.is_tensor(img_cond):
            c = ops.add_f32(c, img_cond.to(x).expand_as(c).contiguous())
        y, S = None, None
        if torch.is_tensor(pts_cond):
            S = pts_cond.shape[2]
            yt = pts_cond.to(self._device(), torch.float32).transpose(1, 2).contiguous().view(B * S, self.hidden_size)
            y = ops.cast_pad_bf16(yt, self.hidden_size)
        xin = ops.cast_pad_bf16(x.view(B * T, self.z_dim), ops.pad64(self.z_dim))
        h = ops.gemm_bf16(xin, P["w_in"], P["b_in"], EPI_F32)
        for l, Pb in enumerate(P["blocks"]):
            if y is not None and l % 2 == 0:
                residual_block(Pb, h, B, T, y_bf16=y, Nk=S, c=c)
            else:
                residual_block(Pb, h, B, T, c=c)
        return final_layer(P["final"], h, B, T, c).view(B, T, self.z_dim)

    def _forward_unet(self, x, t, label, condition):
        from ._lib import EPI_F32
        from .blocks import final_layer, residual_block
        pts_cond, img_cond = (None, 0.) if condition is None else (self.c_net(condition) if isinstance(condition, dict) else condition)
        if torch.is_tensor(pts_cond):
            raise NotImplementedError("unet + point condition: the reference passes the (B,hidden,S) condition as K/V source to "
                                      "down blocks whose fc_kv expects 2*hidden channels (score.py:80,146) and fails there")
        B, T, _ = x.shape
        P = self.packed()
        c = self.time_embedding(t.to(x).float())
        if label is not None:
            c = ops.add_f32(c, self.label_embedding(label))
        elif torch.is_tensor(img_cond):
            c = ops.add_f32(c, img_cond.to(x).expand_as(c))
        xin = ops.cast_pad_bf16(x.view(B * T, self.z_dim), ops.pad64(self.z_dim))
        h = ops.gemm_bf16(xin, P["w_in"], P["b_in"], EPI_F32)
        skips = [h.clone()]
        for Pb in P["up"]:
            residual_block(Pb, h, B, T, c=c)
            skips.append(h.clone())
        residual_block(P["mid"], h, B, T, c=c)
        for Pb in P["down"]:
            h = residual_block(Pb, torch.cat((h, skips.pop()), dim=1), B, T, c=c)
        return final_layer(P["final"], h, B, T, c).view(B, T, self.z_dim)
```

Measured before the change: 6.142 shapes/sec.

## Fold final LayerNorm into output GEMM and emit bf16 xin from sampler step

The final block's down-projection GEMM now runs as a fold producer that skips its fp32 residual store and writes only the scaled bf16 activations and LN stats. The output projection then uses a new fp32 LN-fold consumer epilogue with precomputed scale/shift tables appended to the fold table. This removes the separate final LayerNorm pass and the fp32 residual write. Separately, the sampler step kernel writes the next step's padded bf16 input, so the per-step cast/pad launch is skipped. Both paths are on by default via a seam bitmask, with an env var and a debug setter to switch them off.

```diff
diff --git a/include/ldt_hip.h b/include/ldt_hip.h
--- a/include/ldt_hip.h
+++ b/include/ldt_hip.h
@@ -267,6 +267,7 @@
 int ldt_dbg_gemm_group_m(int32_t rows_per_group);
 int ldt_dbg_gemm_epi(int32_t bits);
 int ldt_dbg_gemm_wreg(int32_t on);
+int ldt_dbg_seam(int32_t bits);
 
 #ifdef __cplusplus
 }
diff --git a/ldt_amd/_lib.py b/ldt_amd/_lib.py
--- a/ldt_amd/_lib.py
+++ b/ldt_amd/_lib.py
@@ -122,6 +122,7 @@
     "ldt_dbg_gemm_group_m": [_i32],
     "ldt_dbg_gemm_epi": [_i32],
     "ldt_dbg_gemm_wreg": [_i32],
+    "ldt_dbg_seam": [_i32],
     "ldt_sample_loop": [C.POINTER(ScorePlan), _vp, _vp, _vp, _vp, _i32, _vp, _i64, _i64, _u64, _vp, _i32, C.POINTER(CondArgs), _vp, _i32, _vp],
 }
 
diff --git a/ldt_amd/csrc/api.hip b/ldt_amd/csrc/api.hip
--- a/ldt_amd/csrc/api.hip
+++ b/ldt_amd/csrc/api.hip
@@ -3,6 +3,7 @@
 #include <stdlib.h>
 #include <string.h>
 
+#include <atomic>
 #include <vector>
 
 #include "../../include/ldt_hip.h"
@@ -359,8 +360,18 @@
     return qkv_attention_step(q, ST(stream), nullptr);
 }
 
+enum { SEAM_FOLD = 1 ,
+       SEAM_XIN = 2  };
+static std::atomic<int> g_dbg_seam{-1};
+extern "C" int ldt_dbg_seam(int32_t bits) { g_dbg_seam.store(bits); return LDT_OK; }
+static int seam_bits() {
+    static const int env = getenv("LDT_SEAM") ? atoi(getenv("LDT_SEAM")) & 3 : 3;
+    const int d = g_dbg_seam.load();
+    return d >= 0 ? d & 3 : env;
+}
+
 static int score_forward_impl(const ldt_score_plan* p, const float* x, float* eps_out, const int32_t* step_ptr,
-                              hipStream_t s, Prof* prof) {
+                              hipStream_t s, Prof* prof, bool xin_ready = false) {
     TRY(check_plan(p));
     LDT_REQUIRE(x && eps_out, LDT_EARG, "score: null x/out");
     const int D = p->hidden, T = p->tokens, M = p->batch * p->tokens, F = p->mlp_hidden;
@@ -370,7 +381,8 @@
     for (int l = 0; l < p->blocks && fold; ++l) fold = !p->kv_cond[l];
     const int sparts = fold_v1 ? D / 32 : D / 256;
     const long fstep = p->fold_step_stride, fblk = 6L * D + 2L * F;
-    LAUNCH(LDT_PROF_OTHER, ldt_cast_pad_launch(x, p->z_dim, BFM(p->xin), p->z_pad, M, p->z_dim, p->z_pad, s));
+    const bool fold_final = fold && !fold_v1 && (seam_bits() & SEAM_FOLD) && fstep >= (long)p->blocks * fblk + 2L * p->z_dim;
+    if (!xin_ready) LAUNCH(LDT_PROF_OTHER, ldt_cast_pad_launch(x, p->z_dim, BFM(p->xin), p->z_pad, M, p->z_dim, p->z_pad, s));
     {
         GemmArgs g{BF(p->xin), p->z_pad, BF(p->w_in), p->z_pad, p->b_in, p->X, D, nullptr, 0, nullptr, 0, nullptr, 0, 0, nullptr, 0, M, D, p->z_pad};
         g.max_wgs = p->gemm_wgs; LAUNCH(LDT_PROF_GEMM_IO, ldt_gemm_launch(LDT_EPI_F32, &g, s));
@@ -405,7 +417,8 @@
             GemmArgs gd{BF(p->U), F, BF(p->w_dn[l]), F, p->b_dn[l], p->X, D, p->X, D, nullptr, 0, m + 5 * D, sstr, T, step_ptr, tstr, M, D, F,
                         BFM(p->Hb), D, m + 6 * D + D, tstr, p->stats};
             gd.max_wgs = p->gemm_wgs; gd.stats_parts = sparts;
-            if (l + 1 < p->blocks) {
+            if (l + 1 < p->blocks || fold_final) {
+                if (l + 1 == p->blocks) gd.no_out = 1;
                 LAUNCH(LDT_PROF_GEMM_DN, ldt_gemm_lnfold_launch(LDT_EPI_RESID_F32, &gd, s));
                 if (p->fold_monitor) TRY(ldt_fold_monitor_launch(p->stats, sparts, M, D, p->fold_monitor, s));
             }
@@ -425,7 +438,12 @@
             gd.max_wgs = p->gemm_wgs; LAUNCH(LDT_PROF_GEMM_DN, ldt_gemm_launch(LDT_EPI_RESID_F32, &gd, s));
         }
     }
-    {
+    if (fold_final) {
+        const float* fo = p->fold + (long)p->blocks * fblk;
+        GemmArgs gf{BF(p->Hb), D, BF(p->w_out), D, nullptr, eps_out, p->z_dim, nullptr, 0, nullptr, 0, nullptr, 0, 0, step_ptr, 0, M, p->z_dim, D,
+                    nullptr, 0, nullptr, 0, nullptr, p->stats, sparts, fo, fo + p->z_dim, fstep};
+        gf.max_wgs = p->gemm_wgs; LAUNCH(LDT_PROF_GEMM_IO, ldt_gemm_lnfold_launch(LDT_EPI_F32, &gf, s));
+    } else {
         const float* m = p->mod + (long)p->blocks * 6 * D;
         LnArgs nf{p->X, D, BFM(p->Hb), D, nullptr, nullptr, m, m + D, sstr, T, step_ptr, tstr, M, D};
         LAUNCH(LDT_PROF_LN, ldt_ln_launch(&nf, s));
@@ -460,7 +478,7 @@
 
 static int enqueue_step(const ldt_score_plan* p, float* x, float* x_mean, float* eps_tmp, const float* coef, int mode,
                         const float* noise, long noise_step_stride, long elem_offset, uint64_t seed, int* step_counter,
-                        const ldt_cond_args* cond, float* x_traj, hipStream_t s) {
+                        const ldt_cond_args* cond, float* x_traj, int seam, hipStream_t s) {
     if (cond) {
         TRY(ldt_cond_rows_launch(cond->temb, cond->extra, cond->c_buf, cond->c_buf_bf16, step_counter, p->batch, cond->t_dim, 1, s));
         if (cond->w_ada_bf16 && (cond->t_dim % 64 == 0 || !cond->w_ada)) {
@@ -477,10 +495,11 @@
             TRY(ldt_sgemm_launch(&g, s));
         }
     }
-    TRY(score_forward_impl(p, x, eps_tmp, cond ? nullptr : step_counter, s, nullptr));
+    TRY(score_forward_impl(p, x, eps_tmp, cond ? nullptr : step_counter, s, nullptr, (seam & SEAM_XIN) != 0));
     const long n = (long)p->batch * p->tokens * p->z_dim;
     StepArgs st{x, eps_tmp, noise, x, x_mean, coef, step_counter, 0, mode, n, elem_offset, noise_step_stride,
                 (uint32_t)seed, (uint32_t)(seed >> 32), 1, 0, x_traj};
+    if (seam & SEAM_XIN) { st.xin = BFM(p->xin); st.z_dim = p->z_dim; st.z_pad = p->z_pad; }
     TRY(ldt_sampler_step_launch(&st, s));
     return ldt_advance_step_launch(step_counter, s);
 }
@@ -498,6 +517,9 @@
     hipStream_t s = ST(stream);
     hipError_t e = hipMemsetAsync(step_counter, 0, sizeof(int), s);
     if (e != hipSuccess) { ldt_set_error("sample_loop: memset: %s", hipGetErrorString(e)); return (int)e; }
+    const int seam = seam_bits();
+    if (seam & SEAM_XIN)
+        TRY(ldt_cast_pad_launch(x, p->z_dim, BFM(p->xin), p->z_pad, (long)p->batch * p->tokens, p->z_dim, p->z_pad, s));
     ldt_score_plan plain = *p;
     plain.fold_monitor = nullptr;
     const bool mon = p->fold_monitor != nullptr;
@@ -505,7 +527,7 @@
     auto monitored = [&](int i) { return mon && (i % every == 0 || i == n_steps - 1); };
     if (!use_graph) {
         for (int i = 0; i < n_steps; ++i)
-            TRY(enqueue_step(monitored(i) ? p : &plain, x, x_mean, eps_tmp, coef, mode, noise, noise_step_stride, elem_offset, seed, step_counter, cond, x_traj, s));
+            TRY(enqueue_step(monitored(i) ? p : &plain, x, x_mean, eps_tmp, coef, mode, noise, noise_step_stride, elem_offset, seed, step_counter, cond, x_traj, seam, s));
         return LDT_OK;
     }
     hipStream_t gs = nullptr;
@@ -532,7 +554,7 @@
         for (int pass = 0; pass < (mon ? 2 : 1) && status == LDT_OK; ++pass) {
             HIPTRY(hipStreamBeginCapture(gs, hipStreamCaptureModeThreadLocal), "begin capture");
             if (status == LDT_OK) {
-                const int rc = enqueue_step(pass ? p : &plain, x, x_mean, eps_tmp, coef, mode, noise, noise_step_stride, elem_offset, seed, step_counter, cond, x_traj, gs);
+                const int rc = enqueue_step(pass ? p : &plain, x, x_mean, eps_tmp, coef, mode, noise, noise_step_stride, elem_offset, seed, step_counter, cond, x_traj, seam, gs);
                 const hipError_t ee = hipStreamEndCapture(gs, pass ? &graph_m : &graph);
                 if (rc != LDT_OK) status = rc;
                 else if (ee != hipSuccess) { ldt_set_error("sample_loop: end capture: %s", hipGetErrorString(ee)); status = (int)ee; }
diff --git a/ldt_amd/csrc/elementwise.hip b/ldt_amd/csrc/elementwise.hip
--- a/ldt_amd/csrc/elementwise.hip
+++ b/ldt_amd/csrc/elementwise.hip
@@ -162,6 +162,12 @@
         *reinterpret_cast<f32x4*>(a.x_out + 4 * i) = xn;
         if (a.traj) *reinterpret_cast<f32x4*>(a.traj + (long)step * a.n + 4 * i) = xn;
         if (a.x_mean_out) *reinterpret_cast<f32x4*>(a.x_mean_out + 4 * i) = xm;
+        if (a.xin) {
+            const long r = (4 * i) / a.z_dim;
+            const int c = (int)(4 * i - r * a.z_dim);
+            const bf16x4 pk = {(bf16_t)xn[0], (bf16_t)xn[1], (bf16_t)xn[2], (bf16_t)xn[3]};
+            *reinterpret_cast<bf16x4*>(a.xin + r * a.z_pad + c) = pk;
+        }
     }
 }
 
@@ -174,6 +180,8 @@
                 (!a->noise || ldt_aligned16(a->noise)) && (!a->x_mean_out || ldt_aligned16(a->x_mean_out)) && a->noise_step_stride % 4 == 0,
                 LDT_EALIGN, "sampler_step: buffers must be 16-byte aligned");
     LDT_REQUIRE(a->mode == 0 || a->mode == 1, LDT_EARG, "sampler_step: mode %d", a->mode);
+    LDT_REQUIRE(!a->xin || (a->z_dim > 0 && a->z_dim % 4 == 0 && a->z_pad >= a->z_dim && a->z_pad % 4 == 0 && a->n % a->z_dim == 0 &&
+                            (reinterpret_cast<uintptr_t>(a->xin) & 7) == 0), LDT_ESHAPE, "sampler_step: xin needs z_dim %% 4 == 0, z_pad %% 4 == 0, 8-byte aligned rows");
     long blocks = (a->n / 4 + 255) / 256;
     if (blocks > 2048) blocks = 2048;
     hipLaunchKernelGGL(sampler_step_kernel, dim3((unsigned)blocks), dim3(256), 0, s, *a);
diff --git a/ldt_amd/csrc/gemm256_tile.h b/ldt_amd/csrc/gemm256_tile.h
--- a/ldt_amd/csrc/gemm256_tile.h
+++ b/ldt_amd/csrc/gemm256_tile.h
@@ -148,7 +148,8 @@
         const bool shared_gate = has_gate && a.gate_sample_stride == 0;
         if (shared_gate) g4 = have_pre ? g4_pre : *reinterpret_cast<const f32x4*>(gate + nb + ch * 4);
         f32x4 sc4 = {1.f, 1.f, 1.f, 1.f};
-        constexpr int SP = (FOLD == FOLD_PRODUCER) ? 8 : 4;
+        static_assert(XRING != 2 || FOLD == FOLD_PRODUCER, "XRING = 2: the producer without its fp32 store");
+        constexpr int SP = (FOLD == FOLD_PRODUCER && XRING != 2) ? 8 : 4;
         const float* xsrc = XRING ? a.resid + ((long)mb + (lane >> 4)) * a.ldr + nb + ch * 4 : nullptr;
         const long xstep = (long)4 * a.ldr;
         auto request_pass = [&](int p) {
@@ -208,7 +209,7 @@
 #pragma unroll
                     for (int r = 0; r < 4; ++r) v[r] = x[r] + g4[r] * v[r];
                 }
-                if (XRING || !(a.dbg & 2)) *reinterpret_cast<f32x4*>(o) = v;
+                if (XRING != 2 && (XRING || !(a.dbg & 2))) *reinterpret_cast<f32x4*>(o) = v;
                 if (FOLD == FOLD_PRODUCER) {
                     const bf16x4 pk = {(bf16_t)(v[0] * sc4[0]), (bf16_t)(v[1] * sc4[1]), (bf16_t)(v[2] * sc4[2]), (bf16_t)(v[3] * sc4[3])};
                     if (XRING || !(a.dbg & 4)) *reinterpret_cast<bf16x4*>(a.xs + (mrow0 + row) * a.ldxs + nb + ch * 4) = pk;
diff --git a/ldt_amd/csrc/gemm_256.hip b/ldt_amd/csrc/gemm_256.hip
--- a/ldt_amd/csrc/gemm_256.hip
+++ b/ldt_amd/csrc/gemm_256.hip
@@ -9,7 +9,7 @@
 
 template <int EPI, int FOLD = FOLD_NONE, int XRING = 0, int WREG = 0, int KLONG = 0>
 __global__ __launch_bounds__(512) void gemm_bf16_nt_256f_kernel(const GemmArgs a) {
-    static_assert(!WREG || XRING == 1, "WREG: one tile per workgroup");
+    static_assert(!WREG || XRING != 0, "WREG: one tile per workgroup");
     extern __shared__ __attribute__((aligned(16))) char smem2[];
     const int tid = threadIdx.x;
     const int lane = tid & 63;
@@ -180,7 +180,7 @@
         if (XRING) {
             asm volatile("s_waitcnt vmcnt(0)" ::: "memory");
             G256_BARRIER();
-            g256_epilogue_staged<EPI, FOLD, 1>(a, acc, m0, n0, grp, wn, lane, lrow, lchk, gate, stage_reg, smem2 + G256_RING_BYTES, ln_scale,
+            g256_epilogue_staged<EPI, FOLD, XRING>(a, acc, m0, n0, grp, wn, lane, lrow, lchk, gate, stage_reg, smem2 + G256_RING_BYTES, ln_scale,
                                                true, g4_pre, sc4_pre, smem2 + wave * 16384);
             break;
         } else
@@ -462,14 +462,20 @@
             if (wreg_dbg == 1 && !a_copy.Wp) a_copy.Wp = dbg_wfrag_cached(a->W, a->ldw, a->N, a->K, stream);
             const bool wreg = a_copy.Wp && wreg_dbg != 0 && ldt_aligned16(a_copy.Wp);
             const bool klong = a->K >= 2048;
-#define LAUNCH_XR(W, KL)                                                                                                          \
+#define LAUNCH_XR(XR, W, KL)                                                                                                      \
     do {                                                                                                                          \
-        LDT_ENSURE_LDS((&gemm_bf16_nt_256f_kernel<EPI, FOLD, 1, W, KL>), G256_LDS_BYTES, "gemm256f");                              \
-        hipLaunchKernelGGL((gemm_bf16_nt_256f_kernel<EPI, FOLD, 1, W, KL>), dim3(grid), dim3(512), G256_LDS_BYTES, stream, *a);   \
+        LDT_ENSURE_LDS((&gemm_bf16_nt_256f_kernel<EPI, FOLD, XR, W, KL>), G256_LDS_BYTES, "gemm256f");                             \
+        hipLaunchKernelGGL((gemm_bf16_nt_256f_kernel<EPI, FOLD, XR, W, KL>), dim3(grid), dim3(512), G256_LDS_BYTES, stream, *a);  \
     } while (0)
-            if (wreg) { if (klong) LAUNCH_XR(1, 1); else LAUNCH_XR(1, 0); }
-            else if (klong) LAUNCH_XR(0, 1);
-            else LAUNCH_XR(0, 0);
+            if constexpr (FOLD == FOLD_PRODUCER) {
+                if (a->no_out && !wreg) {
+                    if (klong) LAUNCH_XR(2, 0, 1); else LAUNCH_XR(2, 0, 0);
+                    return ldt_check_launch("gemm_bf16_nt_256f");
+                }
+            }
+            if (wreg) { if (klong) LAUNCH_XR(1, 1, 1); else LAUNCH_XR(1, 1, 0); }
+            else if (klong) LAUNCH_XR(1, 0, 1);
+            else LAUNCH_XR(1, 0, 0);
 #undef LAUNCH_XR
             return ldt_check_launch("gemm_bf16_nt_256f");
         }
diff --git a/ldt_amd/csrc/gemm_bf16.hip b/ldt_amd/csrc/gemm_bf16.hip
--- a/ldt_amd/csrc/gemm_bf16.hip
+++ b/ldt_amd/csrc/gemm_bf16.hip
@@ -108,10 +108,24 @@
 
     const float* gate = a.gate;
     if (EPI == EPI_RESID_F32 && gate && a.step_ptr) gate += (long)(*a.step_ptr) * a.gate_step_stride;
+    const long fold_off = (EPI == EPI_F32_LNFOLD && a.step_ptr) ? (long)(*a.step_ptr) * a.fold_step_stride : 0;
 #pragma unroll
     for (int mi = 0; mi < MT; ++mi) {
         const int m = m0 + wm * (TBM / WGM) + mi * 16 + lrow;
         if (m >= a.M) continue;
+        float rr = 1.f, nm = 0.f;
+        if (EPI == EPI_F32_LNFOLD) {
+            float s1 = 0.f, s2 = 0.f;
+            for (int pp = 0; pp < a.stats_parts; ++pp) {
+                const f32x2 t = *reinterpret_cast<const f32x2*>(a.stats_in + ((long)pp * a.M + m) * 2);
+                s1 += t[0]; s2 += t[1];
+            }
+            const float invk = 1.0f / (float)a.K;
+            const float mean = s1 * invk;
+            const float var = fmaxf(s2 * invk - mean * mean, 0.f);
+            rr = rsqrtf(var + 1e-6f);
+            nm = -mean * rr;
+        }
         const float* grow = nullptr;
         if (EPI == EPI_RESID_F32 && gate) grow = gate + (long)(m / a.rows_per_sample) * a.gate_sample_stride;
 #pragma unroll
@@ -121,13 +135,26 @@
             f32x4 v = acc[ni][mi];
             const bool full = (n + 3 < a.N);
             float b[4] = {0.f, 0.f, 0.f, 0.f};
-            if (a.bias) {
-                if (full) { const f32x4 t = *reinterpret_cast<const f32x4*>(a.bias + n); b[0] = t[0]; b[1] = t[1]; b[2] = t[2]; b[3] = t[3]; }
-                else for (int r = 0; r < 4; ++r) if (n + r < a.N) b[r] = a.bias[n + r];
-            }
-#pragma unroll
-            for (int r = 0; r < 4; ++r) v[r] += b[r];
-            if (EPI == EPI_F32) {
+            if (EPI == EPI_F32_LNFOLD) {
+                const float* fs = a.fold_S + fold_off + n;
+                const float* fc = a.fold_C + fold_off + n;
+                float sv[4] = {0.f, 0.f, 0.f, 0.f};
+                if (full) {
+                    const f32x4 t = *reinterpret_cast<const f32x4*>(fs); const f32x4 u = *reinterpret_cast<const f32x4*>(fc);
+#pragma unroll
+                    for (int r = 0; r < 4; ++r) { sv[r] = t[r]; b[r] = u[r]; }
+                } else for (int r = 0; r < 4; ++r) if (n + r < a.N) { sv[r] = fs[r]; b[r] = fc[r]; }
+#pragma unroll
+                for (int r = 0; r < 4; ++r) v[r] = v[r] * rr + (nm * sv[r] + b[r]);
+            } else {
+                if (a.bias) {
+                    if (full) { const f32x4 t = *reinterpret_cast<const f32x4*>(a.bias + n); b[0] = t[0]; b[1] = t[1]; b[2] = t[2]; b[3] = t[3]; }
+                    else for (int r = 0; r < 4; ++r) if (n + r < a.N) b[r] = a.bias[n + r];
+                }
+#pragma unroll
+                for (int r = 0; r < 4; ++r) v[r] += b[r];
+            }
+            if (EPI == EPI_F32 || EPI == EPI_F32_LNFOLD) {
                 float* o = reinterpret_cast<float*>(a.out) + (long)m * a.ldo + n;
                 if (full) *reinterpret_cast<f32x4*>(o) = v;
                 else for (int r = 0; r < 4; ++r) if (n + r < a.N) o[r] = v[r];
@@ -199,6 +226,12 @@
         r.family = r.tiles_per_wg == 1 ? GEMM_ROUTE_256_ONE : GEMM_ROUTE_256_MULTI;
     };
     if (granule) {
+        if (epi == EPI_F32 && granule == 256) {
+            if (a->K < 256 || a->K % 256 != 0 || a->K > 1024) return r;
+            r.family = GEMM_ROUTE_V1; r.v1_shape = 2; r.v1_stages = 3; r.bm = r.bn = 64; r.tiles_per_wg = 1;
+            r.grid = (int)((long)((a->M + 63) / 64) * ((a->N + 63) / 64));
+            return r;
+        }
         const bool producer = epi == EPI_RESID_F32;
         if (!producer && epi != EPI_BF16 && epi != EPI_GELU_BF16) return r;
         if (granule == 32) {
@@ -241,6 +274,21 @@
 }
 
 int ldt_gemm_lnfold_launch(int epi, const GemmArgs* a, hipStream_t stream) {
+    if (epi == EPI_F32) {
+        LDT_REQUIRE(a->M > 0 && a->N > 0 && a->stats_parts >= 1 && a->stats_parts <= 4 && a->stats_parts * 256 == a->K, LDT_ESHAPE,
+                    "gemm_lnfold: the fp32 consumer needs stats_in[K/256 <= 4][M][2]; K=%d parts=%d", a->K, a->stats_parts);
+        LDT_REQUIRE(a->ldx % 8 == 0 && a->ldw % 8 == 0 && a->ldx >= a->K && a->ldw >= a->K && a->ldo % 4 == 0 && ldt_aligned16(a->X) &&
+                    ldt_aligned16(a->W) && ldt_aligned16(a->out), LDT_EALIGN, "gemm_lnfold: operands must be 16-byte aligned (ldx=%ld ldw=%ld ldo=%ld)",
+                    a->ldx, a->ldw, a->ldo);
+        LDT_REQUIRE(a->stats_in && a->fold_S && a->fold_C && ldt_aligned16(a->stats_in) && ldt_aligned16(a->fold_S) && ldt_aligned16(a->fold_C) &&
+                    a->fold_step_stride % 4 == 0 && !a->bias, LDT_EARG, "gemm_lnfold: consumer needs stats_in, fold_S, fold_C (16-byte aligned) and takes no bias (it is part of fold_C)");
+        const GemmRoute r = ldt_gemm_decide(epi, a, 256);
+        LDT_REQUIRE(r.family == GEMM_ROUTE_V1, LDT_ESHAPE, "gemm_lnfold: no fp32 consumer for M=%d N=%d K=%d", a->M, a->N, a->K);
+        GemmArgs c = *a;
+        c.col_major = 0;
+        hipLaunchKernelGGL((gemm_bf16_nt_kernel<EPI_F32_LNFOLD, 64, 64, 3>), dim3((unsigned)r.grid), dim3(256), 0, stream, c);
+        return ldt_check_launch("gemm_bf16_nt(lnfold)");
+    }
     const int width = epi == EPI_RESID_F32 ? a->N : a->K;
     const bool v1 = a->stats_parts > 0 && a->stats_parts * 32 == width && a->stats_parts * 256 != width;
     if (v1) LDT_REQUIRE(a->M > 0 && a->M % 128 == 0 && a->N % 64 == 0 && a->K >= 128 && a->K % BK == 0, LDT_ESHAPE,
diff --git a/ldt_amd/csrc/kernels.h b/ldt_amd/csrc/kernels.h
--- a/ldt_amd/csrc/kernels.h
+++ b/ldt_amd/csrc/kernels.h
@@ -2,6 +2,7 @@
 #include "common.h"
 
 enum { EPI_F32 = 0, EPI_BF16 = 1, EPI_GELU_BF16 = 2, EPI_RELU_BF16 = 3, EPI_RESID_F32 = 4 };
+enum { EPI_F32_LNFOLD = 5 };
 #define LDT_NUM_CUS 256
 static inline int ldt_wg_limit(int max_wgs) { return (max_wgs > 0 && max_wgs < LDT_NUM_CUS) ? max_wgs : LDT_NUM_CUS; }
 enum { ACT_NONE = 0, ACT_SILU = 1, ACT_RELU = 2, ACT_GELU = 3 };
@@ -27,6 +28,7 @@
     bf16_t* attn_o; float attn_scale_log2e;
     const bf16_t* attn_k; const bf16_t* attn_v; long attn_ldkv; long attn_kv_batch_stride;
     const bf16_t* Wp;
+    int no_out;
 };
 
 struct LnArgs {
@@ -57,6 +59,7 @@
     uint32_t seed_lo, seed_hi;
     int philox_mul, philox_add;
     float* traj;
+    bf16_t* xin; int z_dim, z_pad;
 };
 
 struct SgemmArgs {
diff --git a/ldt_amd/score.py b/ldt_amd/score.py
--- a/ldt_amd/score.py
+++ b/ldt_amd/score.py
@@ -305,7 +305,8 @@
         D, F = self.hidden_size, self.Transformer[0].mlp.out.in_channels
         n = mod.shape[0]
         fb = 6 * D + 2 * F
-        fold = torch.empty((n, self.num_blocks * fb), dtype=torch.float32, device=mod.device)
+        z = self.z_dim
+        fold = torch.empty((n, self.num_blocks * fb + 2 * z), dtype=torch.float32, device=mod.device)
         ones = torch.ones((1, D), dtype=torch.float32, device=mod.device)
         for l in range(self.num_blocks):
             m0, f0 = l * 6 * D, l * fb
@@ -315,6 +316,10 @@
                 N = wf.shape[0]
                 ops.sgemm(mod[:, sc:sc + D], wf, ops.sgemm(ones, wf).view(-1), out=fold[:, off:off + N])
                 ops.sgemm(mod[:, sh:sh + D], wf, b, out=fold[:, off + N:off + 2 * N])
+        m0, f0 = self.num_blocks * 6 * D, self.num_blocks * fb
+        wf = ops.widen_bf16(P["w_out"])[:z].contiguous()
+        ops.sgemm(mod[:, m0 + D:m0 + 2 * D], wf, ops.sgemm(ones, wf).view(-1), out=fold[:, f0:f0 + z])
+        ops.sgemm(mod[:, m0:m0 + D], wf, P["b_out"][:z].contiguous(), out=fold[:, f0 + z:f0 + 2 * z])
         return fold
 
     def label_embedding(self, label):
```

Measured after the change: 6.170 shapes/sec (median of 6 runs). No clear change (+0.5%).
